# marionmari/pyGPs

Hardware: AMD Instinct MI355X
Metric: GP fits/sec (nlZ+grad, RBF, N=8192 d=16) (higher is better)
Workload: dtype f64; 1 GPU; GPR+RBF, N=8192 d=16 fp64 synthetic (SURVEY 8d recipe, seed 0), infExact nlZ + dnlZ (BASELINE configs[1]); x,y resident in HBM, hyp changes every step; outputs nlZ, dnlZ(4), alpha(N) to host per step; fits_per_rank=313, fit_streams_per_gpu=2, sched=1

## Files before the change

pygps_amd/_lib.py:

```python
import ctypes as C
import os
import threading

import numpy as np

_HERE = os.path.dirname(os.path.abspath(__file__))
LIB_PATH = os.environ.get("PYGPS_AMD_LIB") or os.path.join(_HERE, "libpygps_amd.so")

COV_RBF, COV_RBFARD, COV_MATERN, COV_RBFUNIT, COV_RQ, COV_PIECEPOLY = 0, 1, 2, 3, 4, 5
COV_RQARD, COV_GABOR, COV_PERIODIC, COV_NOISE, COV_CONST, COV_SM = 6, 7, 8, 9, 10, 11
COV_PRE = 12
COV_COMPOSITE = 100
PROG_LEAF, PROG_SUM, PROG_PRODUCT, PROG_SCALE = 1, 2, 3, 4
PROG_MAX_ARD_DIM = 64
PROG_MAX = 8
MODE_TRAIN, MODE_CROSS, MODE_SELF_TEST = 0, 1, 2
LIK_ERF, LIK_GAUSS, LIK_LAPLACE = 0, 1, 2
ERR_LAPLACE_WNEG = -90
FLAG_MATERN_REFERENCE_DER = 1
STAGES = ("assemble", "potrf", "solve", "trtri", "lauum", "grad", "total")

_dp = C.POINTER(C.c_double)
_vp = C.c_void_p
_i64 = C.c_int64

SIGNATURES = {
    "pgp_init": (C.c_int, [C.c_int, C.POINTER(_vp)]),
    "pgp_destroy": (None, [_vp]),
    "pgp_strerror": (C.c_char_p, [C.c_int]),
    "pgp_version": (C.c_char_p, []),
    "pgp_device_count": (C.c_int, []),
    "pgp_device_info": (C.c_int, [_vp, C.POINTER(C.c_int), C.POINTER(C.c_int), _dp, C.c_char_p, C.c_int]),
    "pgp_cov": (C.c_int, [_vp, C.c_int, C.c_int, C.c_int, _dp, _i64, _dp, _i64, _i64, _dp, C.c_int, C.c_int,
                          C.c_int, _dp]),
    "pgp_set_composite": (C.c_int, [_vp, C.POINTER(C.c_int32), C.c_int]),
    "pgp_set_pre": (C.c_int, [_vp, _dp, _i64, _dp, _i64]),
    "pgp_node_kernel": (C.c_int, [_vp, C.c_int, _dp, _i64, C.c_double, C.c_double, _dp]),
    "pgp_knn_graph": (C.c_int, [_vp, _dp, _i64, _i64, C.c_int, _dp]),
    "pgp_set_data": (C.c_int, [_vp, _dp, _i64, _i64, _dp]),
    "pgp_exact_fit": (C.c_int, [_vp, C.c_int, _dp, C.c_int, C.c_int, C.c_int, C.c_double, _dp, _dp, C.c_int,
                                C.c_int, _dp, _dp, _dp, C.POINTER(_vp)]),
    "pgp_factor_to_host": (C.c_int, [_vp, _vp, _dp]),
    "pgp_factor_n": (_i64, [_vp]),
    "pgp_factor_free": (None, [_vp, _vp]),
    "pgp_predict": (C.c_int, [_vp, _vp, _dp, _i64, _dp, _dp, _dp]),
    "pgp_exact_fit_dense": (C.c_int, [_vp, _dp, _i64, _dp, C.c_double, C.c_int, _dp, _dp, _dp, C.POINTER(_vp)]),
    "pgp_dense_grad_term": (C.c_int, [_vp, _dp, _i64, C.c_double, _dp]),
    "pgp_predict_dense": (C.c_int, [_vp, _vp, _dp, _i64, _dp, _dp, _dp, _dp]),
    "pgp_ep_fit": (C.c_int, [_vp, C.c_int, _dp, C.c_int, C.c_int, C.c_int, _dp, _dp, C.c_int, C.c_int, C.c_int,
                             _dp, _dp, _dp, _dp, _dp, _dp, C.POINTER(C.c_int), C.POINTER(_vp)]),
    "pgp_ep_fit_dense": (C.c_int, [_vp, _dp, _dp, _dp, C.c_int, C.c_int, C.c_int, _dp, _dp, _dp, _dp, _dp, _dp,
                                   C.POINTER(C.c_int), C.POINTER(_vp)]),
    "pgp_ep_fit_lik": (C.c_int, [_vp, C.c_int, _dp, C.c_int, C.c_int, C.c_int, C.c_int, _dp, C.c_int, C.c_int, _dp, _dp,
                                 C.c_int, C.c_int, C.c_int, _dp, _dp, _dp, _dp, _dp, _dp, C.POINTER(C.c_int), C.POINTER(_vp)]),
    "pgp_ep_fit_dense_lik": (C.c_int, [_vp, _dp, C.c_int, _dp, C.c_int, C.c_int, _dp, _dp, C.c_int, C.c_int, C.c_int, _dp, _dp,
                                       _dp, _dp, _dp, _dp, C.POINTER(C.c_int), C.POINTER(_vp)]),
    "pgp_laplace_fit": (C.c_int, [_vp, C.c_int, _dp, C.c_int, C.c_int, C.c_int, C.c_int, _dp, C.c_int, _dp, _dp, C.c_int,
                                  C.c_int, C.c_int, _dp, _dp, _dp, _dp, C.POINTER(C.c_int), _dp, C.POINTER(_vp)]),
    "pgp_laplace_fit_dense": (C.c_int, [_vp, _dp, C.c_int, _dp, C.c_int, _dp, _dp, C.c_int, C.c_int, C.c_int, _dp, _dp,
                                        _dp, _dp, C.POINTER(C.c_int), _dp, C.POINTER(_vp)]),
    "pgp_gpmc_fit_predict": (C.c_int, [_vp, C.c_int, _dp, C.c_int, C.c_int, C.c_int, C.c_int, C.POINTER(C.c_int32), C.c_int, _dp, _dp,
                                       _i64, _dp, _dp, _dp, C.POINTER(C.c_int32), C.POINTER(C.c_int32)]),
    "pgp_fitc_fit": (C.c_int, [_vp, C.c_int, _dp, C.c_int, C.c_int, C.c_int, C.c_double, _dp, _i64, _dp, _dp, C.c_int,
                               C.c_int, _dp, _dp, _dp, _dp, C.POINTER(_vp)]),
    "pgp_fitc_predict": (C.c_int, [_vp, _vp, _dp, _i64, _dp, _dp, _dp]),
    "pgp_fitc_free": (None, [_vp, _vp]),
    "pgp_fitc_ep_fit": (C.c_int, [_vp, C.c_int, _dp, C.c_int, C.c_int, C.c_int, _dp, _i64, _dp, _dp, C.c_int, C.c_int,
                                  C.c_int, _dp, _dp, _dp, _dp, _dp, _dp, C.POINTER(C.c_int), C.POINTER(_vp)]),
    "pgp_fitc_ep_fit_lik": (C.c_int, [_vp, C.c_int, _dp, C.c_int, C.c_int, C.c_int, C.c_int, _dp, C.c_int, C.c_int, _dp, _i64,
                                      _dp, _dp, C.c_int, C.c_int, C.c_int, _dp, _dp, _dp, _dp, _dp, _dp, C.POINTER(C.c_int),
                                      C.POINTER(_vp)]),
    "pgp_potrf": (C.c_int, [_vp, _dp, _i64, _dp]),
    "pgp_potrs": (C.c_int, [_vp, _dp, _i64, _dp, _i64, _dp]),
    "pgp_last_timings": (C.c_int, [_vp, _dp]),
    "pgp_set_profiling": (C.c_int, [_vp, C.c_int]),
    "pgp_profile_classes": (C.c_int, []),
    "pgp_profile_class_name": (C.c_char_p, [C.c_int]),
    "pgp_profile_read": (C.c_int, [_vp, C.c_int, C.POINTER(_i64), _dp, _dp, _dp]),
    "pgp_profile_reset": (C.c_int, [_vp]),
    "pgp_set_option": (C.c_int, [_vp, C.c_char_p, C.c_int]),
    "pgp_comm_unique_id": (C.c_int, [C.c_char_p, C.c_char_p]),
    "pgp_comm_init_rccl": (C.c_int, [_vp, C.c_int, C.c_int, C.c_char_p, C.c_char_p, C.POINTER(_vp)]),
    "pgp_comm_init_host": (C.c_int, [_vp, C.c_int, C.c_int, _vp, _vp, _vp, C.POINTER(_vp)]),
    "pgp_comm_free": (None, [_vp]),
    "pgp_comm_world": (C.c_int, [_vp]),
    "pgp_comm_rank": (C.c_int, [_vp]),
    "pgp_comm_bcast_host": (C.c_int, [_vp, _dp, _i64, C.c_int]),
    "pgp_comm_allreduce_host": (C.c_int, [_vp, _dp, _i64, C.c_int]),
    "pgp_comm_allgather_host": (C.c_int, [_vp, _dp, _i64, _dp]),
    "pgp_sharded_exact_fit": (C.c_int, [_vp, _vp, C.c_int, _dp, C.c_int, C.c_int, C.c_int, C.c_double, _dp, _dp, C.c_int,
                                        C.c_int, _dp, _dp, _dp, _dp, _dp, C.POINTER(_vp)]),
    "pgp_sharded_predict": (C.c_int, [_vp, _vp, _vp, _dp, _i64, _dp, _dp, _dp]),
    "pgp_sfactor_free": (None, [_vp, _vp]),
    "pgp_sfactor_bytes": (_i64, [_vp]),
}

TEST_SIGNATURES = {
    "pgp_test_gemm": (C.c_int, [_vp, C.c_int, C.c_int, C.c_int, C.c_int, C.c_int, C.c_int, C.c_int, C.c_double,
                                C.c_double, _dp, _i64, _dp, _i64, _dp, _i64, C.c_int, C.c_int, C.c_int, C.c_int,
                                _dp]),
    "pgp_test_gemm_shrink": (C.c_int, [_vp, _dp, _i64, C.c_int, C.c_int, C.c_int, C.c_int, C.c_int, C.c_int, _dp, _i64,
                                       _i64]),
    "pgp_test_gemm_zskip": (C.c_int, [_vp] + [C.c_int] * 5 + [C.c_double, C.c_double, _dp, _i64, _dp, _i64, _dp, _dp, _i64,
                                      C.c_int, C.c_int, C.c_int]),
    "pgp_test_gemm_skip_wait": (C.c_int, [_vp, C.c_int, _dp, _dp, _dp, C.c_int, C.c_int, C.c_int, C.c_int, C.c_int,
                                          C.POINTER(C.c_int)]),
    "pgp_test_probit_hazard": (C.c_int, [_vp, _dp, _dp, C.c_int]),
    "pgp_test_laplace_lik": (C.c_int, [_vp, C.c_int, C.c_double, _dp, _dp, C.c_int, _dp]),
    "pgp_test_laplace_ep_lik": (C.c_int, [_vp, _dp, _dp, _dp, _dp, C.c_int, _dp]),
    "pgp_test_valu_peak": (C.c_int, [_vp, C.c_int, C.c_int, _dp]),
    "pgp_test_mfma_peak": (C.c_int, [_vp, C.c_int, _dp]),
    "pgp_test_mfma_cycles": (C.c_int, [_vp, C.c_int, C.c_int, C.c_int, _dp]),
    "pgp_test_leaf_ticks": (C.c_int, [_vp, _dp]),
    "pgp_test_assemble": (C.c_int, [_vp, C.c_int, C.c_int, _i64, _i64, C.c_int, _dp]),
    "pgp_test_gemm_trace": (C.c_int, [_vp, C.c_int, C.c_int, C.c_int, C.c_int, C.c_int, C.POINTER(C.c_longlong), _i64, C.POINTER(_i64)]),
    "pgp_test_read_gemm_trace": (C.c_int, [_vp, C.POINTER(C.c_longlong), _i64, C.POINTER(_i64)]),
    "pgp_test_store_roof": (C.c_int, [_vp, _i64, C.c_int, C.c_int, _dp]),
    "pgp_test_cumask_gemm": (C.c_int, [_vp, C.c_int, C.c_int, C.c_int, C.c_int, C.c_int, _dp]),
    "pgp_test_wave_costs": (C.c_int, [_vp, _dp]),
    "pgp_test_stream_concurrency": (C.c_int, [_vp, C.c_int, _dp]),
    "pgp_test_slot_probe": (C.c_int, [_vp, C.c_int, C.c_int, C.c_int, C.c_int, C.c_int, C.c_int, _dp]),
    "pgp_test_hadamard": (C.c_int, [_vp, C.c_int, _dp, C.c_int, C.c_int, C.c_int, _dp, _dp, _dp, C.c_double, _dp]),
    "pgp_test_gather_sym": (C.c_int, [_vp, _dp, _i64, C.POINTER(C.c_int32), _i64, _i64, _dp, _dp, _dp, _dp]),
    "pgp_test_vote": (C.c_int, [_vp, _dp, _dp, _i64, C.c_int, C.c_int, C.c_int, _dp, _dp]),
    "pgp_test_yield_table": (C.c_int, [_vp, C.POINTER(C.c_uint32)]),
}

_lock = threading.RLock()
_dll = None
_ctx = {}


def _torch_first():
    import sys
    if os.environ.get("PYGPS_AMD_NO_TORCH"):
        return
    if "torch" in sys.modules or os.environ.get("PYGPS_AMD_TORCH_FIRST") == "1":
        try:
            import torch
        except Exception:
            pass


def want_torch():
    import sys
    if "torch" not in sys.modules and _dll is not None:
        import logging
        logging.getLogger(__name__).warning(
            "pygps_amd: torch is imported AFTER libpygps_amd.so (HIP runtime in use: %s); on some nodes one of the two then "
            "sees no GPU -- import torch first or set PYGPS_AMD_TORCH_FIRST=1", hip_runtime_path())
    import torch
    return torch


def hip_runtime_path():
    try:
        with open("/proc/self/maps") as f:
            for line in f:
                if "libamdhip64" in line:
                    return line.split()[-1]
    except OSError:
        pass
    return None


def load():
    global _dll
    if _dll is not None:
        return _dll
    with _lock:
        if _dll is None:
            _torch_first()
            if not os.path.exists(LIB_PATH):
                raise RuntimeError(
                    "pygps_amd: %s not found -- build it with `python -c 'import __graft_entry__ as g; g.build()'` "
                    "(hipcc --offload-arch=gfx950).  There is no CPU fallback." % LIB_PATH)
            dll = C.CDLL(LIB_PATH)
            for table in (SIGNATURES, TEST_SIGNATURES):
                for name, (res, args) in table.items():
                    fn = getattr(dll, name)
                    fn.restype = res
                    fn.argtypes = args
            _dll = dll
    return _dll


def strerror(rc):
    return load().pgp_strerror(rc).decode()


def check(rc, what="pygps_amd", arg_messages=None):
    if rc == 0:
        return
    if rc > 0:
        raise np.linalg.LinAlgError("kernel matrix not positive definite, even with jitter. (first bad pivot %d)" % rc)
    if rc <= -100:
        raise RuntimeError("%s: %s" % (what, strerror(rc)))
    if arg_messages and rc in arg_messages:
        raise Exception(arg_messages[rc])
    raise Exception("%s: bad argument (code %d)" % (what, rc))


def ptr(a):
    return None if a is None else a.ctypes.data_as(_dp)


def f64(a):
    return np.ascontiguousarray(a, dtype=np.float64)


def default_device():
    return int(os.environ.get("LOCAL_RANK", os.environ.get("PYGPS_AMD_DEVICE", "0")))


_tls = threading.local()


def current_slot():
    return getattr(_tls, "slot", 0)


class fit_stream(object):

    def __init__(self, k):
        self.k = int(k)

    def __enter__(self):
        self.prev = current_slot()
        _tls.slot = self.k
        return self

    def __exit__(self, *exc):
        _tls.slot = self.prev
        return False


class concurrent_fit_streams(object):

    def __enter__(self):
        self.prev = getattr(_tls, "concurrent", None)
        self.used = {}
        _tls.concurrent = self
        return self

    def _use(self, key, h):
        if key not in self.used:
            load().pgp_set_option(h, b"concurrent_streams", 1)
            self.used[key] = h

    def __exit__(self, *exc):
        _tls.concurrent = self.prev
        for key, h in self.used.items():
            if self.prev is not None and key in self.prev.used:
                continue
            load().pgp_set_option(h, b"concurrent_streams", 0)
        self.used = {}
        return False


def ctx(device=None, slot=None):
    if device is None:
        device = default_device()
    if slot is None:
        slot = current_slot()
    h = _ctx.get((device, slot))
    scope = getattr(_tls, "concurrent", None)
    if h is not None:
        if scope is not None:
            scope._use((device, slot), h)
        return h
    dll = load()
    with _lock:
        h = _ctx.get((device, slot))
        if h is None:
            out = _vp()
            rc = dll.pgp_init(device, C.byref(out))
            if rc != 0:
                raise RuntimeError("pygps_amd: cannot initialise HIP device %d: %s (no CPU fallback)"
                                   % (device, dll.pgp_strerror(rc).decode()))
            h = out
            _ctx[(device, slot)] = h
    if scope is not None:
        scope._use((device, slot), h)
    return h


def device_info(device=None):
    dll = load()
    ncu, clk, gib = C.c_int(), C.c_int(), C.c_double()
    name = C.create_string_buffer(256)
    check(dll.pgp_device_info(ctx(device), C.byref(ncu), C.byref(clk), C.byref(gib), name, 256))
    return dict(name=name.value.decode(), n_cu=ncu.value, sclk_mhz=clk.value, hbm_gib=gib.value)


_devmem = {}


def device_memory_bytes(device=None):
    if device is None:
        device = default_device()
    if device not in _devmem:
        _devmem[device] = device_info(device)["hbm_gib"] * 2.0 ** 30
    return _devmem[device]


def last_timings(device=None):
    out = np.zeros(len(STAGES))
    check(load().pgp_last_timings(ctx(device), ptr(out)))
    return dict(zip(STAGES, out.tolist()))


def profile(device=None):
    dll = load()
    res = {}
    for i in range(dll.pgp_profile_classes()):
        n, ms, fl, by = _i64(), C.c_double(), C.c_double(), C.c_double()
        check(dll.pgp_profile_read(ctx(device), i, C.byref(n), C.byref(ms), C.byref(fl), C.byref(by)))
        res[dll.pgp_profile_class_name(i).decode()] = dict(launches=n.value, ms=ms.value, flops=fl.value,
                                                           bytes=by.value)
    return res
```

pygps_amd/csrc/capi.hip:

```cpp
#include <algorithm>
#include <atomic>
#include <cmath>
#include <cstdio>
#include <cstdlib>
#include <cstring>
#include <map>
#include <string>
#include <mutex>
#include <vector>

#include "ctx.h"

static thread_local char g_err[512] = "";
void pgp_set_last_hip_error(hipError_t e, const char* what, const char* file, int line) {
    snprintf(g_err, sizeof(g_err), "HIP error %d (%s) in %s at %s:%d", (int)e, hipGetErrorString(e), what, file, line);
    (void)hipGetLastError();
}

static void ctx_register(pgp_ctx* c);
static void ctx_unregister(pgp_ctx* c);

void prof_collect(pgp_ctx* c) {
    if (c->recs.empty()) return;
    (void)hipStreamSynchronize(c->st);
    for (auto& r : c->recs) {
        float ms = 0.f;
        (void)hipEventElapsedTime(&ms, r.e0, r.e1);
        c->pc_ms[r.cls] += ms; c->pc_flops[r.cls] += r.flops; c->pc_bytes[r.cls] += r.bytes; c->pc_launch[r.cls]++;
        if (r.shadow >= 0) { c->pc_ms[r.shadow] += ms; c->pc_flops[r.shadow] += r.flops; c->pc_launch[r.shadow]++; }
        if (getenv("PGP_PROF_DUMP"))
            fprintf(stderr, "prof %-34s %8.4f ms %10.3f GF %7.2f TF\n", kProfNames[r.cls], ms, r.flops * 1e-9,
                    ms > 0 ? r.flops / (ms * 1e-3) * 1e-12 : 0.0);
        c->ev_pool.push_back(r.e0); c->ev_pool.push_back(r.e1);
    }
    c->recs.clear();
}

DeviceGate& device_gate(int device) {
    static DeviceGate gates[64];
    return gates[(unsigned)device % 64u];
}
int& device_gate_depth(int device) {
    static thread_local int depth[64] = {0};
    return depth[(unsigned)device % 64u];
}

extern "C" {

const char* pgp_version(void) { return "pygps_amd 0.1 (gfx950)"; }
int pgp_device_count(void) {
    int n = 0;
    if (hipGetDeviceCount(&n) != hipSuccess) { (void)hipGetLastError(); return 0; }
    return n;
}

const char* pgp_strerror(int status) {
    if (status == 0) return "ok";
    if (status > 0) return "kernel matrix not positive definite";
    if (status <= PGP_ERR_HIP) return g_err[0] ? g_err : "HIP runtime failure";
    return "bad argument";
}

__global__ void pgp_noop_kernel() {}
static int alloc_result_buffer(pgp_ctx* c, long np);

static unsigned* yield_table(int device) {
    static std::mutex mu;
    static unsigned* tab[64] = {nullptr};
    std::lock_guard<std::mutex> lk(mu);
    if (device < 0 || device >= 64) return nullptr;
    if (!tab[device]) {
        if (hipMalloc((void**)&tab[device], 4096 * sizeof(unsigned)) != hipSuccess) { (void)hipGetLastError(); tab[device] = nullptr; return nullptr; }
        (void)hipMemset(tab[device], 0, 4096 * sizeof(unsigned));
    }
    return tab[device];
}

int pgp_init(int device, pgp_ctx** ctx_out) { GateShared device_gate_hold(device);
    if (!ctx_out) return -2;
    HIP_TRY(hipSetDevice(device));
    {
        static std::mutex mu;
        static bool primed[64] = {false};
        std::lock_guard<std::mutex> lk(mu);
        if (device >= 0 && device < 64 && !primed[device]) {
            hipLaunchKernelGGL(pgp_noop_kernel, dim3(1), dim3(64), 0, 0);
            HIP_TRY(hipDeviceSynchronize());
            primed[device] = true;
        }
    }
    pgp_ctx* c = new pgp_ctx();
    c->device = device;
    if (const char* e = getenv("PYGPS_AMD_PREDICT_INVERSE")) { const int v = atoi(e); if (v >= 0 && v <= 2) c->predict_inverse = v; }
    if (const char* e = getenv("PYGPS_AMD_KEEP_INVERSE")) c->keep_inverse = atoi(e) != 0;
    HIP_TRY(hipGetDeviceProperties(&c->prop, device));
    HIP_TRY(hipStreamCreateWithFlags(&c->st, hipStreamNonBlocking));
    {
        int lo = 0, hi = 0;
        (void)hipDeviceGetStreamPriorityRange(&lo, &hi);
        HIP_TRY(hipStreamCreateWithPriority(&c->st2, hipStreamNonBlocking, hi));
        if (lo == hi) c->ep_block = 0;
    }
    for (auto& e : c->ev) HIP_TRY(hipEventCreate(&e));
    memset(c->last_ms, 0, sizeof(c->last_ms));
    memset(c->pc_ms, 0, sizeof(c->pc_ms)); memset(c->pc_flops, 0, sizeof(c->pc_flops));
    memset(c->pc_bytes, 0, sizeof(c->pc_bytes)); memset(c->pc_launch, 0, sizeof(c->pc_launch));
    CHK(alloc_result_buffer(c, 0));
    c->yield_flags = yield_table(device);
    HIP_TRY(hipMalloc((void**)&c->Dk, (size_t)2048 * 1024 * sizeof(double)));
    HIP_TRY(hipMalloc((void**)&c->dpack, (size_t)8 * PACK_DOUBLES * sizeof(double)));
    HIP_TRY(hipMemset(c->Dk, 0, (size_t)2048 * 1024 * sizeof(double)));
    ctx_register(c);
    *ctx_out = c;
    return PGP_OK;
}

constexpr long RES_HEAD = 272, RES_INFO = 264;
static int alloc_result_buffer(pgp_ctx* c, long np) {
    const size_t bytes = (size_t)(RES_HEAD + np) * sizeof(double);
    if (c->res_dev) (void)hipFree(c->res_dev);
    if (c->res_host) (void)hipHostFree(c->res_host);
    c->res_dev = c->res_host = c->res_host_dev = nullptr; c->scal = c->alpha_dev = nullptr; c->info_dev = nullptr; c->res_cap = 0;
    HIP_TRY(hipMalloc((void**)&c->res_dev, bytes));
    HIP_TRY(hipMemset(c->res_dev, 0, bytes));
    HIP_TRY(hipHostMalloc((void**)&c->res_host, bytes, hipHostMallocMapped | hipHostMallocCoherent));
    c->res_host_dev = nullptr;
    if (hipHostGetDevicePointer((void**)&c->res_host_dev, c->res_host, 0) != hipSuccess) { (void)hipGetLastError(); c->res_host_dev = nullptr; }
    c->scal = c->res_dev; c->info_dev = (int*)(c->res_dev + RES_INFO); c->alpha_dev = c->res_dev + RES_HEAD;
    c->res_cap = bytes;
    return PGP_OK;
}

void pgp_destroy(pgp_ctx* c) { if (!c) return; GateShared device_gate_hold(c);
    if (!c) return;
    ctx_unregister(c);
    (void)hipSetDevice(c->device);
    (void)hipStreamSynchronize(c->st);
    if (c->st2) (void)hipStreamSynchronize(c->st2);
    for (auto& kv : c->pool) (void)hipFree(kv.second);
    for (auto& kv : c->spool) (void)hipFree(kv.second);
    for (auto& kv : c->orders) (void)hipFree(kv.second.first);
    void* bufs[] = {c->x_dev, c->y_dev, c->XsT, c->scale_dev, c->W, c->T, c->Binv, c->inv16, c->m_dev,
                    c->rvec, c->zvec, c->partial, c->Dk, c->dpack, c->Xs, c->res_dev, c->prep, c->pre2, c->pre1t, c->pre1s};
    for (void* b : bufs) if (b) (void)hipFree(b);
    if (c->res_host) (void)hipHostFree(c->res_host);
    if (c->in_host) (void)hipHostFree(c->in_host);
    if (c->pred_host) (void)hipHostFree(c->pred_host);
    if (c->gemm_trace) (void)hipFree(c->gemm_trace);
    for (auto& e : c->ev) (void)hipEventDestroy(e);
    for (auto& e : c->ev_pool) (void)hipEventDestroy(e);
    for (auto& r : c->recs) { (void)hipEventDestroy(r.e0); (void)hipEventDestroy(r.e1); }
    for (auto& e : c->la_ev) (void)hipEventDestroy(e);
    for (auto& e : c->tm_ev) (void)hipEventDestroy(e);
    for (auto& e : c->fill_ev) (void)hipEventDestroy(e);
    for (auto& e : c->ep_ev) (void)hipEventDestroy(e);
    (void)hipStreamDestroy(c->st);
    if (c->st2) (void)hipStreamDestroy(c->st2);
    delete c;
}

int pgp_device_info(pgp_ctx* c, int* n_cu, int* sclk_mhz, double* hbm_gib, char* name, int name_len) {
    if (!c) return -1;
    if (n_cu) *n_cu = c->prop.multiProcessorCount;
    if (sclk_mhz) *sclk_mhz = c->prop.clockRate / 1000;
    if (hbm_gib) *hbm_gib = (double)c->prop.totalGlobalMem / (1024.0 * 1024.0 * 1024.0);
    if (name && name_len > 0) { strncpy(name, c->prop.name, name_len - 1); name[name_len - 1] = 0; }
    return PGP_OK;
}

int pgp_set_option(pgp_ctx* c, const char* name, int value) {
    if (!c || !name) return -1;
    if (!strcmp(name, "nb_outer")) { if (value < 0) return -3; c->nb_outer = value; return PGP_OK; }
    if (!strcmp(name, "small_tile_below")) { c->small_tile_below = value; return PGP_OK; }
    if (!strcmp(name, "trtri_small_tile_below")) { c->trtri_small_tile_below = value; return PGP_OK; }
    if (!strcmp(name, "xcd_order")) { c->xcd_order = value; return PGP_OK; }
    if (!strcmp(name, "gemm_dbg")) { if (value & ~(64 | 256 | 512)) return -2; c->gemm_dbg = value; return PGP_OK; }
    if (!strcmp(name, "lookahead")) { c->lookahead = value; return PGP_OK; }
    if (!strcmp(name, "leaf_first")) { c->leaf_first = value; return PGP_OK; }
    if (!strcmp(name, "leaf_pivot")) { if (value < 0 || value > 2) return -2; c->leaf_pivot = value; return PGP_OK; }
    if (!strcmp(name, "sched")) { if (value < -1 || value > 2) return -2; c->sched = value < 0 ? PGP_SCHED_DEFAULT : value; c->sched_explicit = value >= 0; return PGP_OK; }
    if (!strcmp(name, "concurrent_streams")) { c->concurrent_streams = value != 0; return PGP_OK; }
    if (!strcmp(name, "tud_tile")) { if (value != 64 && value != 128) return -2; c->tud_tile = value; return PGP_OK; }
    if (!strcmp(name, "tur_tile")) { if (value != 0 && value != 64 && value != 128 && value != 1264) return -2; c->tur_tile = value; return PGP_OK; }
    if (!strcmp(name, "s_pan")) { if (value < -1 || value > 2) return -2; c->s_pan = value; return PGP_OK; }
    if (!strcmp(name, "s_pan_direct")) { c->s_pan_direct = value != 0; return PGP_OK; }
    if (!strcmp(name, "s_pan_out")) { c->s_pan_out = value != 0; return PGP_OK; }
    if (!strcmp(name, "skip_zeros")) { c->skip_zeros = value != 0; return PGP_OK; }
    if (!strcmp(name, "tud_mark")) { c->tud_mark = value != 0; return PGP_OK; }
    if (!strcmp(name, "sched2_wide")) { c->sched2_wide = value != 0; return PGP_OK; }
    if (!strcmp(name, "gram_assembly")) { if (value < 0 || value > 2) return -2; c->gram_assembly = value; return PGP_OK; }
    if (!strcmp(name, "yield")) { c->yield = value; return PGP_OK; }
    if (!strcmp(name, "ep_fused")) { c->ep_fused = value; return PGP_OK; }
    if (!strcmp(name, "ep_tol_exp")) { if (value < 1 || value > 16) return -3; c->ep_tol_exp = value; return PGP_OK; }
    if (!strcmp(name, "ep_max_sweep")) { if (value < 2 || value > 1000) return -3; c->ep_max_sweep = value; return PGP_OK; }
    if (!strcmp(name, "laplace_tol_exp")) { if (value < 1 || value > 16) return -3; c->laplace_tol_exp = value; return PGP_OK; }
    if (!strcmp(name, "ep_r_direct")) { c->ep_r_direct = value; return PGP_OK; }
    if (!strcmp(name, "ep_alpha_direct")) { c->ep_alpha_direct = value; return PGP_OK; }
    if (!strcmp(name, "ep_sym")) { c->ep_sym = value; return PGP_OK; }
    if (!strcmp(name, "ep_wait_kernel")) { c->ep_wait_kernel = value; return PGP_OK; }
    if (!strcmp(name, "ep_sigma_under")) { c->ep_sigma_under = value; return PGP_OK; }
    if (!strcmp(name, "ep_recompute")) { c->ep_recompute = value; return PGP_OK; }
    if (!strcmp(name, "ep_final_rebuild")) { c->ep_final_rebuild = value; return PGP_OK; }
    if (!strcmp(name, "ep_block")) { c->ep_block = value; return PGP_OK; }
    if (!strcmp(name, "xcd_max_k")) { c->xcd_max_k = value; return PGP_OK; }
    if (!strcmp(name, "xcd_min_tiles")) { c->xcd_min_tiles = value; return PGP_OK; }
    if (!strcmp(name, "xcd_super")) { c->xcd_super = value; return PGP_OK; }
    if (!strcmp(name, "solve_outer")) { if (value < 1) return -2; c->solve_outer = value; return PGP_OK; }
    if (!strcmp(name, "keep_inverse")) { c->keep_inverse = value != 0; return PGP_OK; }
    if (!strcmp(name, "predict_inverse")) { if (value < 0 || value > 2) return -2; c->predict_inverse = value; return PGP_OK; }
    if (!strcmp(name, "predict_batch")) { if (value < 128 || value % 128) return -2; c->predict_batch = value; return PGP_OK; }
    if (!strcmp(name, "s_tile")) { if (value != 0 && value != 64 && value != 128) return -2; c->s_tile = value; return PGP_OK; }
    if (!strcmp(name, "eet_overlap")) { if (value != 0 && value != 2 && value != 3) return -2; c->eet_overlap = value; return PGP_OK; }
    if (!strcmp(name, "eet_max_panels")) { c->eet_max_panels = value; return PGP_OK; }
    if (!strcmp(name, "eet_first")) { if (value < -1) return -2; c->eet_first = value; return PGP_OK; }
    if (!strcmp(name, "eet_tile")) { if (value != 64 && value != 128) return -2; c->eet_tile = value; return PGP_OK; }
    if (!strcmp(name, "fused_inverse")) { c->fused_inverse = value; return PGP_OK; }
    if (!strcmp(name, "trsm_lean")) { if (value < 0 || value > 2) return -2; c->trsm_lean = value; return PGP_OK; }
    if (!strcmp(name, "ep_merge12")) { c->ep_merge12 = value != 0; return PGP_OK; }
    if (!strcmp(name, "publish")) { c->publish = value != 0; return PGP_OK; }
    if (!strcmp(name, "fused_value_max_np")) { c->fused_value_max_np = value; return PGP_OK; }
    if (!strcmp(name, "asm_grid")) { c->asm_grid = value; return PGP_OK; }
    if (!strcmp(name, "gram_fast")) { if (value < 0 || value > 2) return -2; c->gram_fast = value; return PGP_OK; }
    if (!strcmp(name, "gram_grid")) { if (value < 0) return -2; c->gram_grid = value; return PGP_OK; }
    if (!strcmp(name, "asm_nt")) { c->asm_nt = value; return PGP_OK; }
    if (!strcmp(name, "pair_launch")) { c->pair_launch = value != 0; return PGP_OK; }
    if (!strcmp(name, "gemm_trace")) {
        GateShared device_gate_hold(c);
        HIP_TRY(hipSetDevice(c->device));
        HIP_TRY(hipDeviceSynchronize());
        if (c->gemm_trace) { (void)hipFree(c->gemm_trace); c->gemm_trace = nullptr; }
        c->gemm_trace_cap = 0; c->gemm_trace_pos = 0;
        if (value > 0) {
            const long cap = (long)value * 1024;
            HIP_TRY(hipMalloc((void**)&c->gemm_trace, (size_t)cap * 64));
            HIP_TRY(hipMemset(c->gemm_trace, 0, (size_t)cap * 64));
            c->gemm_trace_cap = cap;
        }
        return PGP_OK;
    }
    if (!strcmp(name, "ard_grad_form")) { if (value < 0 || value > 2) return -3; c->ard_grad_form = value; return PGP_OK; }
    return -2;
}

int pgp_last_timings(pgp_ctx* c, double* ms_out) {
    if (!c || !ms_out) return -1;
    memcpy(ms_out, c->last_ms, sizeof(c->last_ms));
    return PGP_OK;
}
int pgp_set_profiling(pgp_ctx* c, int on) { if (!c) return -1; c->prof = on != 0; return PGP_OK; }
int pgp_profile_classes(void) { return PC_COUNT; }
const char* pgp_profile_class_name(int cls) { return (cls >= 0 && cls < PC_COUNT) ? kProfNames[cls] : "?"; }
int pgp_profile_read(pgp_ctx* c, int cls, int64_t* launches, double* ms, double* flops, double* bytes) {
    if (!c || cls < 0 || cls >= PC_COUNT) return -1;
    prof_collect(c);
    if (launches) *launches = c->pc_launch[cls];
    if (ms) *ms = c->pc_ms[cls];
    if (flops) *flops = c->pc_flops[cls];
    if (bytes) *bytes = c->pc_bytes[cls];
    return PGP_OK;
}
int pgp_profile_reset(pgp_ctx* c) {
    if (!c) return -1;
    prof_collect(c);
    memset(c->pc_ms, 0, sizeof(c->pc_ms)); memset(c->pc_flops, 0, sizeof(c->pc_flops));
    memset(c->pc_bytes, 0, sizeof(c->pc_bytes)); memset(c->pc_launch, 0, sizeof(c->pc_launch));
    return PGP_OK;
}

}


static int matern_d(int para) { return (para == 1 || para == 3 || para == 5 || para == 7) ? para : 3; }

static int leaf_nhyp(int kind, long d) {
    switch (kind) {
        case PGP_COV_RBF: case PGP_COV_MATERN: case PGP_COV_PIECEPOLY: case PGP_COV_GABOR: return 2;
        case PGP_COV_RBFARD: return (int)d + 1;
        case PGP_COV_RQARD: return (int)d + 2;
        case PGP_COV_RBFUNIT: case PGP_COV_NOISE: case PGP_COV_CONST: return 1;
        case PGP_COV_RQ: case PGP_COV_PERIODIC: return 3;
        case PGP_COV_PRE: return 0;
        default: return -1;
    }
}

static int make_leaf(int kind, const double* hyp, int nhyp, int para, int flags, long d, CovParams& cp, double& iso) {
    const int want = leaf_nhyp(kind, d);
    if (want < 0) return -2;
    if (nhyp != want) return -11;
    cp = CovParams{};
    cp.kind = kind; cp.der = -1; cp.md = matern_d(para); cp.D = (int)d; cp.train = 1;
    cp.ref_der = (flags & PGP_FLAG_MATERN_REFERENCE_DER) ? 1 : 0;
    cp.sf2 = 1.0; cp.alpha = 1.0; cp.ppv = 0; cp.ppj = 1.0; cp.ga = 0.0; cp.gb = 0.0;
    iso = 1.0;
    switch (kind) {
        case PGP_COV_RBF: iso = 1.0 / exp(hyp[0]); cp.sf2 = exp(2.0 * hyp[1]); break;
        case PGP_COV_RBFARD: cp.sf2 = exp(2.0 * hyp[d]); break;
        case PGP_COV_MATERN: iso = sqrt((double)cp.md) / exp(hyp[0]); cp.sf2 = exp(2.0 * hyp[1]); break;
        case PGP_COV_RBFUNIT: iso = 1.0 / exp(hyp[0]); break;
        case PGP_COV_RQ: iso = 1.0 / exp(hyp[0]); cp.sf2 = exp(2.0 * hyp[1]); cp.alpha = exp(hyp[2]); break;
        case PGP_COV_PIECEPOLY:
            if (para < 0 || para > 3) return -12;
            iso = 1.0 / exp(hyp[0]); cp.sf2 = exp(2.0 * hyp[1]);
            cp.ppv = para; cp.ppj = floor(0.5 * (double)d) + para + 1.0;
            break;
        case PGP_COV_RQARD: cp.sf2 = exp(2.0 * hyp[d]); cp.alpha = exp(hyp[d + 1]); cp.gb = 1.0; break;
        case PGP_COV_GABOR: {
            const double ell = exp(hyp[0]), p = exp(2.0 * hyp[1]);
            iso = 1.0 / ell; cp.ga = 2.0 * M_PI * ell / p;
            break;
        }
        case PGP_COV_PERIODIC:
            if (d != 1) return -12;
            cp.gb = 1.0 / exp(hyp[0]); cp.ga = M_PI / exp(hyp[1]); cp.sf2 = exp(2.0 * hyp[2]);
            break;
        case PGP_COV_NOISE: cp.sf2 = exp(2.0 * hyp[0]); break;
        case PGP_COV_CONST: cp.sf2 = exp(hyp[0]); break;
    }
    return PGP_OK;
}

static int bind_pre(pgp_ctx* c, CovSpec& cs) {
    if (cs.pg.pre_leaf < 0) return PGP_OK;
    if (!c || !c->pre2 || c->pre_n != c->n || c->n <= 0) return -14;
    cs.pre_train = c->pre2; cs.pre_ld = c->pre_ld; cs.pre_rows = c->pre_ld;
    return PGP_OK;
}

int make_spec(pgp_ctx* c, int kind, const double* hyp, int nhyp, int para, int flags, int der, long d, CovSpec& cs) {
    cs = CovSpec{};
    if (c) { cs.asm_grid = c->asm_grid; cs.asm_nt = c->asm_nt; cs.gram_fast = c->gram_fast; cs.gram_grid = c->gram_grid; }
    if (!hyp && nhyp > 0) return -10;
    if (kind == PGP_COV_SM) {
        const long Q = para;
        if (Q < 1) return -12;
        if (d > SM_MAXD || Q * (1 + 2 * d) > SM_MAXHYP) return -13;
        if ((long)nhyp != Q * (1 + 2 * d)) return -11;
        if (der >= nhyp) return -4;
        CovSM& P = cs.smp;
        P = CovSM{};
        P.Q = (int)Q; P.D = (int)d; P.dt = -1; P.dj = -1; P.dq = 0;
        const long double pi = 3.14159265358979323846264338327950288L;
        long double sw = 0.0L;
        for (long q = 0; q < Q; ++q) { P.h[q] = (double)expl((long double)hyp[q]); sw += expl((long double)hyp[q]); }
        for (long i = 0; i < d * Q; ++i) {
            P.h[Q + i] = (double)(2.0L * pi * expl((long double)hyp[Q + i]));
            P.h[Q + d * Q + i] = (double)(2.0L * pi * pi * expl(2.0L * (long double)hyp[Q + d * Q + i]));
        }
        cs.sm = true; cs.scale.assign(d, 1.0); cs.ncov = nhyp; cs.nder = nhyp;
        cs.cp = CovParams{};
        cs.cp.kind = kind; cs.cp.der = der; cs.cp.D = (int)d; cs.cp.train = 1; cs.cp.sf2 = (double)sw;
        return PGP_OK;
    }
    if (kind >= PGP_COV_GABOR && kind < PGP_COV_NKIND) {
        CovProgram& P = cs.pg;
        P = CovProgram{};
        double iso;
        CHK(make_leaf(kind, hyp, nhyp, para, flags, d, P.leaf[0], iso));
        if (der >= nhyp) return -4;
        P.nleaf = 1; P.nterm = 1; P.nscale = 0; P.is2[0] = iso * iso; P.hyp0[0] = 0; P.nh[0] = nhyp; P.ard_leaf = -1; P.ard_leaf2 = -1;
        P.pre_leaf = kind == PGP_COV_PRE ? 0 : -1;
        P.coef[0] = 1.0; P.tl[0] = 1u; P.ts[0] = 0u;
        P.der = der; P.der_leaf = der >= 0 ? 0 : -1; P.der_j = der; P.der_scale = -1;
        cs.prog = true; cs.scale.assign(d, 1.0); cs.ncov = nhyp; cs.nder = nhyp;
        return bind_pre(c, cs);
    }
    if (kind != PGP_COV_COMPOSITE) {
        double iso;
        CHK(make_leaf(kind, hyp, nhyp, para, flags, d, cs.cp, iso));
        cs.scale.assign(d, iso);
        if (kind == PGP_COV_RBFARD || kind == PGP_COV_RQARD) {
            for (long k = 0; k < d; ++k) cs.scale[k] = 1.0 / exp(hyp[k]);
            double bound = 0.0;
            if (c && (long)c->xdev2.size() == d)
                for (long k = 0; k < d; ++k) bound += cs.scale[k] * cs.scale[k] * c->xdev2[k];
            cs.ard_grad_diff = !(bound <= ARD_GRAM_GRAD_BOUND) || (c && c->ard_grad_form == 2);
            if (c && c->ard_grad_form == 1) cs.ard_grad_diff = false;
        }
        cs.ncov = nhyp;
        cs.nder = (kind == PGP_COV_MATERN || kind == PGP_COV_PIECEPOLY) ? 3 : nhyp;
        if (der >= cs.nder) return -4;
        cs.cp.der = der;
        cs.ell4 = (kind == PGP_COV_RQARD && cs.cp.ref_der && der >= 0 && der < d) ? exp(4.0 * hyp[der]) : 1.0;
        return PGP_OK;
    }
    const std::vector<int>& tok = c->composite;
    if (tok.empty()) return -2;
    struct Term { unsigned leaves, scales; };
    std::vector<std::vector<Term>> stack;
    CovProgram& P = cs.pg;
    P = CovProgram{};
    P.der = der; P.der_leaf = P.der_j = P.der_scale = -1;
    P.ard_leaf = -1; P.ard_leaf2 = -1; P.pre_leaf = -1;
    int used = 0;
    for (size_t i = 0; i < tok.size();) {
        const int op = tok[i];
        if (op == PGP_PROG_LEAF) {
            if (i + 5 > tok.size()) return -2;
            const int lk = tok[i + 1], lpara = tok[i + 2], lflags = tok[i + 3], h0 = tok[i + 4];
            i += 5;
            const bool ard = lk == PGP_COV_RBFARD || lk == PGP_COV_RQARD;
            if (ard && (P.ard_leaf2 >= 0 || d > CP_MAXARD)) return -13;
            const int nh = leaf_nhyp(lk, d);
            if (nh < 0) return -2;
            if (h0 < 0 || h0 + nh > nhyp) return -11;
            if (P.nleaf >= CP_MAXLEAF) return -13;
            if (lk == PGP_COV_PRE) {
                if (P.pre_leaf >= 0) return -13;
                P.pre_leaf = P.nleaf;
            }
            double iso;
            CHK(make_leaf(lk, hyp + h0, nh, lpara, lflags, d, P.leaf[P.nleaf], iso));
            P.is2[P.nleaf] = iso * iso; P.hyp0[P.nleaf] = h0; P.nh[P.nleaf] = nh;
            if (ard) {
                double* aw = P.ard_leaf < 0 ? P.ardw : P.ardw2;
                (P.ard_leaf < 0 ? P.ard_leaf : P.ard_leaf2) = P.nleaf;
                for (long k = 0; k < d; ++k) aw[k] = exp(-2.0 * hyp[h0 + k]);
                if (lk == PGP_COV_RQARD && P.leaf[P.nleaf].ref_der && der >= h0 && der < h0 + d) cs.ell4 = exp(4.0 * hyp[der]);
            }
            if (der >= h0 && der < h0 + nh) { P.der_leaf = P.nleaf; P.der_j = der - h0; }
            stack.push_back({Term{1u << P.nleaf, 0u}});
            ++P.nleaf; used += nh;
        } else if (op == PGP_PROG_SUM || op == PGP_PROG_PRODUCT) {
            ++i;
            if (stack.size() < 2) return -2;
            std::vector<Term> b = stack.back(); stack.pop_back();
            std::vector<Term> a = stack.back(); stack.pop_back();
            std::vector<Term> r;
            if (op == PGP_PROG_SUM) { r = a; r.insert(r.end(), b.begin(), b.end()); }
            else for (const Term& x : a) for (const Term& y : b) r.push_back(Term{x.leaves | y.leaves, x.scales | y.scales});
            if (r.size() > (size_t)CP_MAXTERM) return -13;
            stack.push_back(r);
        } else if (op == PGP_PROG_SCALE) {
            if (i + 1 >= tok.size()) return -2;
            const int h = tok[i + 1];
            i += 2;
            if (stack.empty()) return -2;
            if (h < 0 || h >= nhyp) return -11;
            if (P.nscale >= CP_MAXSCALE) return -13;
            for (Term& t : stack.back()) t.scales |= 1u << P.nscale;
            P.shyp[P.nscale] = h;
            if (der == h) P.der_scale = P.nscale;
            ++P.nscale; ++used;
        } else {
            return -2;
        }
    }
    if (stack.size() != 1 || used != nhyp) return -11;
    P.nterm = (int)stack[0].size();
    for (int t = 0; t < P.nterm; ++t) {
        P.tl[t] = stack[0][t].leaves; P.ts[t] = stack[0][t].scales;
        double cf = 1.0;
        for (int k = 0; k < P.nscale; ++k)
            if ((P.ts[t] >> k) & 1u) cf *= exp(hyp[P.shyp[k]]);
        P.coef[t] = cf;
    }
    if (der >= nhyp) return -4;
    cs.prog = true;
    cs.scale.assign(d, 1.0);
    cs.ncov = nhyp; cs.nder = nhyp;
    cs.cp = CovParams{};
    if (P.ard_leaf >= 0 && c && (long)c->xdev2.size() == d) {
        double b1 = 0.0, b2 = 0.0;
        for (long k = 0; k < d && k < CP_MAXARD; ++k) { b1 += P.ardw[k] * c->xdev2[k]; if (P.ard_leaf2 >= 0) b2 += P.ardw2[k] * c->xdev2[k]; }
        cs.ard_grad_diff = !(std::max(b1, b2) <= ARD_GRAM_GRAD_BOUND);
    }
    if (c && P.ard_leaf >= 0 && c->ard_grad_form) cs.ard_grad_diff = c->ard_grad_form == 2;
    return bind_pre(c, cs);
}

int cov_point_value(pgp_ctx* c, const CovSpec& cs, int train, double* out) {
    if (cs.has_pre()) { *out = 0.0; return PGP_OK; }
    if (!cs.prog && cs.cp.der < 0) {
        (void)train;
        *out = cs.cp.sf2;
        return PGP_OK;
    }
    double* dv = c->scal + 6;
    CHK(cov_self_launch(cs, train, dv, c->st));
    HIP_TRY(hipMemcpyAsync(out, dv, sizeof(double), hipMemcpyDeviceToHost, c->st));
    HIP_TRY(hipStreamSynchronize(c->st));
    return PGP_OK;
}

int upload_scaled(pgp_ctx* c, const double* x_dev, long n, long d, const std::vector<double>& sc, double* XsT,
                         long ldp, int dpad, double* scale_dev) {
    HIP_TRY(hipMemcpyAsync(scale_dev, sc.data(), d * sizeof(double), hipMemcpyHostToDevice, c->st));
    return scale_transpose_launch(x_dev, n, (int)d, scale_dev, XsT, ldp, dpad, c->st);
}

static int tile_order(pgp_ctx* c, int mt, int nt, int tri, int off_tiles, const int** out, int* n) {
    std::vector<int> key = {mt, nt, tri ? 1 : 0, off_tiles, c->xcd_super};
    auto it = c->orders.find(key);
    if (it != c->orders.end()) { *out = it->second.first; *n = it->second.second; return PGP_OK; }
    const int S = c->xcd_super > 0 ? c->xcd_super : 8;
    std::vector<std::vector<int>> sts;
    for (int SI = 0; SI * S < mt; ++SI)
        for (int SJ = 0; SJ * S < nt; ++SJ) {
            std::vector<int> st;
            for (int ti = SI * S; ti < std::min(mt, SI * S + S); ++ti)
                for (int tj = SJ * S; tj < std::min(nt, SJ * S + S); ++tj)
                    if (!tri || ti + off_tiles >= tj) { st.push_back(ti); st.push_back(tj); }
            if (!st.empty()) sts.push_back(std::move(st));
        }
    std::stable_sort(sts.begin(), sts.end(), [](const std::vector<int>& a, const std::vector<int>& b) { return a.size() > b.size(); });
    std::vector<std::vector<int>> seq(8);
    for (auto& st : sts) {
        int best = 0;
        for (int x = 1; x < 8; ++x) if (seq[x].size() < seq[best].size()) best = x;
        seq[best].insert(seq[best].end(), st.begin(), st.end());
    }
    for (;;) {
        int lo = 0, hi = 0;
        for (int x = 1; x < 8; ++x) { if (seq[x].size() < seq[lo].size()) lo = x; if (seq[x].size() > seq[hi].size()) hi = x; }
        if (seq[hi].size() < seq[lo].size() + 4) break;
        const int tj = seq[hi].back(); seq[hi].pop_back();
        const int ti = seq[hi].back(); seq[hi].pop_back();
        seq[lo].push_back(ti); seq[lo].push_back(tj);
    }
    size_t maxlen = 0;
    for (auto& q : seq) maxlen = std::max(maxlen, q.size() / 2);
    const int nb = (int)maxlen * 8;
    std::vector<int> ord(2 * (size_t)nb, -1);
    for (int b = 0; b < nb; ++b) {
        const int x = b % 8, idx = b / 8;
        if ((size_t)idx < seq[x].size() / 2) { ord[2 * b] = seq[x][2 * idx]; ord[2 * b + 1] = seq[x][2 * idx + 1]; }
    }
    int* dev = nullptr;
    HIP_TRY(hipMalloc((void**)&dev, ord.size() * sizeof(int)));
    HIP_TRY(hipMemcpyAsync(dev, ord.data(), ord.size() * sizeof(int), hipMemcpyHostToDevice, c->st));
    HIP_TRY(hipStreamSynchronize(c->st));
    c->orders[key] = {dev, nb};
    *out = dev; *n = nb;
    return PGP_OK;
}

static int tri_tile_list(pgp_ctx* c, int mt, int nt, int off_tiles, const int** out, int* n) {
    std::vector<int> key = {mt, nt, 2, off_tiles};
    auto it = c->orders.find(key);
    if (it != c->orders.end()) { *out = it->second.first; *n = it->second.second; return PGP_OK; }
    std::vector<int> ord;
    for (int tj = 0; tj < nt; ++tj)
        for (int ti = 0; ti < mt; ++ti)
            if (ti + off_tiles >= tj) { ord.push_back(ti); ord.push_back(tj); }
    int* dev = nullptr;
    HIP_TRY(hipMalloc((void**)&dev, ord.size() * sizeof(int)));
    HIP_TRY(hipMemcpyAsync(dev, ord.data(), ord.size() * sizeof(int), hipMemcpyHostToDevice, c->st));
    HIP_TRY(hipStreamSynchronize(c->st));
    c->orders[key] = {dev, (int)ord.size() / 2};
    *out = dev; *n = (int)ord.size() / 2;
    return PGP_OK;
}

int batch_tile_list(pgp_ctx* c, int mt0, int nt, int nb, int dmt, const int** out, int* n) {
    std::vector<int> key = {mt0, nt, nb, dmt, 7777};
    auto it = c->orders.find(key);
    if (it != c->orders.end()) { *out = it->second.first; *n = it->second.second; return PGP_OK; }
    std::vector<int> ord;
    for (int z = 0; z < nb; ++z)
        for (int tj = 0; tj < nt; ++tj)
            for (int ti = tj; ti < mt0 - z * dmt; ++ti) { ord.push_back(ti | (z << 16)); ord.push_back(tj); }
    if (ord.empty()) { ord.push_back(-1); ord.push_back(-1); }
    int* dev = nullptr;
    HIP_TRY(hipMalloc((void**)&dev, ord.size() * sizeof(int)));
    HIP_TRY(hipMemcpyAsync(dev, ord.data(), ord.size() * sizeof(int), hipMemcpyHostToDevice, c->st));
    HIP_TRY(hipStreamSynchronize(c->st));
    c->orders[key] = {dev, (int)ord.size() / 2};
    *out = dev; *n = (int)ord.size() / 2;
    return PGP_OK;
}

bool gram_assembly_applies(pgp_ctx* c, const CovSpec& cs) {
    if (!c->gram_assembly || !cov_gram_applies(cs, c->dpad) || (long)c->xdev2.size() != c->d || (long)cs.scale.size() < c->d) return false;
    if (c->gram_assembly == 2) return true;
    double bound = 0.0;
    for (long k = 0; k < c->d; ++k) bound += cs.scale[k] * cs.scale[k] * c->xdev2[k];
    return bound <= 64.0;
}

static int gemm_prepare(pgp_ctx* c, GemmArgs& g) {
    if (g.batch < 1) g.batch = 1;
    g.dbg |= c->gemm_dbg;
    bool xcd = false;
    if (c->xcd_order && !g.order && g.tile != 64 && g.tile != 1264 && g.batch == 1 && g.K <= c->xcd_max_k) {
        const long mt = g.M / 128, nt = g.N / 128;
        const long tiles = g.tri == 2 ? mt * (mt + 1) / 2 : (g.tri == 1 ? mt * nt - nt * (nt - 1) / 2 : mt * nt);
        xcd = tiles >= c->xcd_min_tiles;
    }
    if (g.tri == 1 && !g.order && !xcd) {
        const int T = g.tile == 64 ? 64 : 128;
        CHK(tri_tile_list(c, g.M / T, g.N / T, g.tri_off / T, &g.order, &g.norder));
    }
    if (xcd) CHK(tile_order(c, g.M / 128, g.N / 128, g.tri, g.tri ? g.tri_off / 128 : 0, &g.order, &g.norder));
    if (c->yield && c->yield_flags) {
        g.yield_flags = c->yield_flags;
        if (g.yield_role != 2) g.yield_role = gemm_f64_uses_dma(g) ? 1 : 0;
    } else g.yield_role = 0;
    if (c->gemm_trace && gemm_f64_uses_dma128(g) && g.batch == 1) {
        const long mt = g.M / 128, nt = g.N / 128;
        const long nb = g.order ? g.norder : (g.tri == 2 ? mt * (mt + 1) / 2 : mt * nt);
        if (c->gemm_trace_pos + nb <= c->gemm_trace_cap) { g.trace = c->gemm_trace + 8 * c->gemm_trace_pos; c->gemm_trace_pos += nb; }
    }
    return PGP_OK;
}

int gemm_prof(pgp_ctx* c, int cls, GemmArgs g, hipStream_t st) {
    if (!st) st = c->st;
    CHK(gemm_prepare(c, g));
    ProfScope ps(c, cls, g.flops, 0.0, st, gemm_f64_uses_dma128(g) ? PC_KERNEL_DMA128 : -1);
    return gemm_f64_launch(g, st);
}

int gemm_prof_pair(pgp_ctx* c, int cls_a, GemmArgs a, int cls_b, GemmArgs b, hipStream_t st) {
    if (!st) st = c->st;
    CHK(gemm_prepare(c, a));
    CHK(gemm_prepare(c, b));
    if (c->pair_launch && gemm_f64_pair_ok(a, b)) {
        ProfScope ps(c, cls_a, a.flops + b.flops, 0.0, st, PC_KERNEL_DMA128);
        return gemm_f64_launch_pair(a, b, st);
    }
    { ProfScope ps(c, cls_a, a.flops, 0.0, st, gemm_f64_uses_dma128(a) ? PC_KERNEL_DMA128 : -1);
      CHK(gemm_f64_launch(a, st)); }
    ProfScope ps(c, cls_b, b.flops, 0.0, st, gemm_f64_uses_dma128(b) ? PC_KERNEL_DMA128 : -1);
    return gemm_f64_launch(b, st);
}

struct TriNode { int lo, mid, hi, depth; };
static void tri_nodes(int lo, int hi, int depth, std::vector<TriNode>& out) {
    if (hi - lo <= 1) return;
    int half = 1;
    while (half * 2 < hi - lo) half *= 2;
    const int mid = lo + half;
    out.push_back({lo, mid, hi, depth});
    tri_nodes(lo, mid, depth + 1, out);
    tri_nodes(mid, hi, depth + 1, out);
}

int trtri_lower(pgp_ctx* c, const double* L, long ldl, double* W, long ldw, double* T, long np) {
    const int nblk = (int)(np / 128);
    {
        ProfScope ps(c, PC_LEAFINV, (double)nblk * 128.0 * 128.0 * 128.0 / 3.0, 0.0);
        CHK(leaf_inv_launch(L, ldl, W, ldw, 128L * (1 + ldw), nblk, c->st));
    }
    std::vector<TriNode> nodes;
    tri_nodes(0, nblk, 0, nodes);
    int maxd = -1;
    for (auto& nd : nodes) maxd = std::max(maxd, nd.depth);
    for (int dep = maxd; dep >= 0; --dep) {
        std::vector<TriNode> lv;
        for (auto& nd : nodes) if (nd.depth == dep) lv.push_back(nd);
        if (lv.empty()) continue;
        std::sort(lv.begin(), lv.end(), [](const TriNode& a, const TriNode& b) { return a.lo < b.lo; });
        bool uniform = true;
        const int h1 = lv[0].mid - lv[0].lo, h2 = lv[0].hi - lv[0].mid;
        const int step = lv.size() > 1 ? lv[1].lo - lv[0].lo : 0;
        for (size_t i = 0; i < lv.size(); ++i)
            if (lv[i].mid - lv[i].lo != h1 || lv[i].hi - lv[i].mid != h2 || lv[i].lo != lv[0].lo + (int)i * step)
                uniform = false;
        const size_t ngroups = uniform ? 1 : lv.size();
        for (size_t gi = 0; gi < ngroups; ++gi) {
            const TriNode& nd = lv[gi];
            const int a1 = (nd.mid - nd.lo) * 128, a2 = (nd.hi - nd.mid) * 128;
            const long o1 = (long)nd.lo * 128, o2 = (long)nd.mid * 128;
            const int batch = uniform ? (int)lv.size() : 1;
            const long bstep = (long)step * 128;
            const long t128 = (long)(a2 / 128) * (a1 / 128) * batch;
            GemmArgs g{};
            g.A = L + o2 + o1 * ldl; g.lda = ldl; g.a_kc = 0;
            g.B = W + o1 + o1 * ldw; g.ldb = ldw; g.b_kc = 1;
            g.C = T; g.ldc = a2;
            g.M = a2; g.N = a1; g.K = a1; g.alpha = 1.0; g.beta = 0.0;
            g.kmode = KM_GE_J; g.koff = 0;
            g.batch = batch; g.sA = bstep * (1 + ldl); g.sB = bstep * (1 + ldw); g.sC = (long)a1 * a2;
            g.tile = t128 < c->trtri_small_tile_below ? 64 : 128;
            g.flops = (double)batch * (double)a2 * a1 * a1;
            CHK(gemm_prof(c, PC_GEMM_TRTRI, g));
            GemmArgs h{};
            h.A = W + o2 + o2 * ldw; h.lda = ldw; h.a_kc = 0;
            h.B = T; h.ldb = a2; h.b_kc = 1;
            h.C = W + o2 + o1 * ldw; h.ldc = ldw;
            h.M = a2; h.N = a1; h.K = a2; h.alpha = -1.0; h.beta = 0.0;
            h.kmode = KM_LT_I; h.koff = 0;
            h.batch = batch; h.sA = bstep * (1 + ldw); h.sB = (long)a1 * a2; h.sC = bstep * (1 + ldw);
            h.tile = g.tile;
            h.flops = (double)batch * (double)a2 * a2 * a1;
            CHK(gemm_prof(c, PC_GEMM_TRTRI, h));
        }
    }
    return PGP_OK;
}

int lauum_lower(pgp_ctx* c, const double* W, long ldw, double* Binv, long ldb, long np) {
    GemmArgs g{};
    g.A = W; g.lda = ldw; g.a_kc = 1;
    g.B = W; g.ldb = ldw; g.b_kc = 1;
    g.C = Binv; g.ldc = ldb;
    g.M = (int)np; g.N = (int)np; g.K = (int)np; g.alpha = 1.0; g.beta = 0.0;
    g.tri = 2; g.mask_diag = 1; g.kmode = KM_GE_I; g.koff = 0;
    const long t128 = (np / 128) * (np / 128 + 1) / 2;
    g.tile = t128 < c->small_tile_below ? 64 : 128;
    g.flops = (double)np * np * np / 3.0;
    return gemm_prof(c, PC_GEMM_LAUUM, g);
}

int eet_lower(pgp_ctx* c, const double* E, long lde, double* Binv, long ldb, long np) {
    GemmArgs g{};
    g.A = E; g.lda = lde; g.a_kc = 0;
    g.B = E; g.ldb = lde; g.b_kc = 0;
    g.C = Binv; g.ldc = ldb;
    g.M = (int)np; g.N = (int)np; g.K = (int)np; g.alpha = 1.0; g.beta = 0.0;
    g.tri = 2; g.mask_diag = 1; g.kmode = KM_GE_I; g.koff = 0;
    const long t128 = (np / 128) * (np / 128 + 1) / 2;
    g.tile = t128 < c->small_tile_below ? 64 : 128;
    g.flops = (double)np * np * np / 3.0;
    return gemm_prof(c, PC_GEMM_LAUUM, g);
}

int ensure_workspace(pgp_ctx* c, long np) {
    if (c->ws_np == np) return PGP_OK;
    (void)hipStreamSynchronize(c->st);
    void* olds[] = {c->W, c->T, c->Binv, c->inv16, c->m_dev, c->rvec, c->zvec, c->prep};
    for (void* b : olds) if (b) (void)hipFree(b);
    c->W = c->T = c->Binv = c->inv16 = c->m_dev = c->rvec = c->zvec = c->prep = nullptr;
    if (c->in_host) { (void)hipHostFree(c->in_host); c->in_host = nullptr; c->in_cap = 0; }
    c->ws_np = 0;
    c->dense_ready = false;
    const size_t nn = (size_t)np * np * sizeof(double);
    HIP_TRY(hipMalloc((void**)&c->W, nn));
    HIP_TRY(hipMemsetAsync(c->W, 0, nn, c->st));
    HIP_TRY(hipMalloc((void**)&c->Binv, nn));
    HIP_TRY(hipMemsetAsync(c->Binv, 0, nn, c->st));
    HIP_TRY(hipMalloc((void**)&c->T, std::max<size_t>(nn / 4, 128 * 128 * sizeof(double))));
    HIP_TRY(hipMalloc((void**)&c->inv16, (size_t)(np / 128) * PACK_DOUBLES * sizeof(double)));
    CHK(alloc_result_buffer(c, np));
    HIP_TRY(hipMalloc((void**)&c->m_dev, np * sizeof(double)));
    HIP_TRY(hipMalloc((void**)&c->rvec, np * sizeof(double)));
    HIP_TRY(hipMalloc((void**)&c->zvec, np * sizeof(double)));
    HIP_TRY(hipMalloc((void**)&c->prep, (size_t)hadamard_prep_count(np) * sizeof(double)));
    HIP_TRY(hipMemsetAsync(c->rvec, 0, np * sizeof(double), c->st));
    c->in_cap = (size_t)(np + 1024) * sizeof(double);
    HIP_TRY(hipHostMalloc((void**)&c->in_host, c->in_cap, hipHostMallocDefault));
    c->ws_np = np;
    return PGP_OK;
}

int alloc_factor_buffer(pgp_ctx* c, long np, long ldf, double** F) {
    const size_t bytes = (size_t)ldf * np * sizeof(double);
    bool fresh = false;
    CHK(pool_alloc(c, bytes, (void**)F, &fresh));
    if (fresh) HIP_TRY(hipMemsetAsync(*F, 0, bytes, c->st));
    return PGP_OK;
}

static std::mutex g_ctx_mu;
static std::vector<pgp_ctx*> g_ctxs;
int pgp_ctx_count_on_device(int device) {
    std::lock_guard<std::mutex> lk(g_ctx_mu);
    int n = 0;
    for (pgp_ctx* c : g_ctxs) n += c->device == device;
    return n;
}
void pgp_drop_idle_pools(int device) { GateShared device_gate_hold(device);
    std::lock_guard<std::mutex> lk(g_ctx_mu);
    for (pgp_ctx* c : g_ctxs) {
        if (c->device != device) continue;
        std::lock_guard<std::mutex> lp(c->pool_mu);
        for (auto& kv : c->pool) (void)hipFree(kv.second);
        for (auto& kv : c->spool) (void)hipFree(kv.second);
        c->pool.clear(); c->pool_bytes = 0;
        c->spool.clear(); c->spool_bytes = 0;
    }
}
static void ctx_register(pgp_ctx* c) { std::lock_guard<std::mutex> lk(g_ctx_mu); g_ctxs.push_back(c); }
static void ctx_unregister(pgp_ctx* c) {
    std::lock_guard<std::mutex> lk(g_ctx_mu);
    g_ctxs.erase(std::remove(g_ctxs.begin(), g_ctxs.end(), c), g_ctxs.end());
}

extern "C" {

int pgp_set_composite(pgp_ctx* c, const int32_t* prog, int nprog) { if (!c) return -1; GateShared device_gate_hold(c);
    if (!c) return -1;
    if (nprog < 0 || (nprog > 0 && !prog)) return -2;
    c->composite.assign(prog, prog + nprog);
    return PGP_OK;
}

int pgp_set_pre(pgp_ctx* c, const double* M2, int64_t n, const double* M1, int64_t ns) { if (!c) return -1; GateShared device_gate_hold(c);
    if (!c) return -1;
    if (n <= 0) return -3;
    if (M1 && ns <= 0) return -5;
    HIP_TRY(hipSetDevice(c->device));
    (void)hipStreamSynchronize(c->st);
    const long np = round_up(n, 128);
    if (M2) {
        if (c->pre2) (void)hipFree(c->pre2);
        c->pre2 = nullptr; c->pre_n = 0;
        if (c->pre1t) (void)hipFree(c->pre1t);
        if (c->pre1s) (void)hipFree(c->pre1s);
        c->pre1t = c->pre1s = nullptr; c->pre_ns = 0;
        HIP_TRY(hipMalloc((void**)&c->pre2, (size_t)np * np * sizeof(double)));
        HIP_TRY(hipMemsetAsync(c->pre2, 0, (size_t)np * np * sizeof(double), c->st));
        HIP_TRY(hipMemcpy2DAsync(c->pre2, np * sizeof(double), M2, n * sizeof(double), n * sizeof(double), n, hipMemcpyHostToDevice, c->st));
        HIP_TRY(hipStreamSynchronize(c->st));
        c->pre_n = n; c->pre_ld = np;
    }
    if (M1) {
        if (!c->pre2 || c->pre_n != n) return -2;
        if (c->pre1t) (void)hipFree(c->pre1t);
        if (c->pre1s) (void)hipFree(c->pre1s);
        c->pre1t = c->pre1s = nullptr; c->pre_ns = 0;
        const long nsp = round_up(ns, 128);
        HIP_TRY(hipMalloc((void**)&c->pre1t, (size_t)nsp * np * sizeof(double)));
        HIP_TRY(hipMalloc((void**)&c->pre1s, (size_t)nsp * sizeof(double)));
        HIP_TRY(hipMemsetAsync(c->pre1t, 0, (size_t)nsp * np * sizeof(double), c->st));
        HIP_TRY(hipMemsetAsync(c->pre1s, 0, (size_t)nsp * sizeof(double), c->st));
        std::vector<double> blk;
        for (int64_t a = 0; a < ns; a += 1024) {
            const int64_t nb = std::min<int64_t>(1024, ns - a);
            blk.resize((size_t)nb * n);
            for (int64_t i = 0; i < n; ++i)
                for (int64_t j = 0; j < nb; ++j) blk[(size_t)j * n + i] = M1[(size_t)i * ns + a + j];
            HIP_TRY(hipMemcpy2DAsync(c->pre1t + a * np, np * sizeof(double), blk.data(), n * sizeof(double), n * sizeof(double), nb,
                                     hipMemcpyHostToDevice, c->st));
            HIP_TRY(hipStreamSynchronize(c->st));
        }
        HIP_TRY(hipMemcpyAsync(c->pre1s, M1 + (size_t)n * ns, ns * sizeof(double), hipMemcpyHostToDevice, c->st));
        HIP_TRY(hipStreamSynchronize(c->st));
        c->pre_ns = ns; c->pre_nsp = nsp;
    }
    return PGP_OK;
}

int pgp_set_data(pgp_ctx* c, const double* x, int64_t n, int64_t d, const double* y) { if (!c) return -1; GateShared device_gate_hold(c);
    if (!c) return -1;
    if (!x) return -2;
    if (n <= 0) return -3;
    if (d <= 0) return -4;
    HIP_TRY(hipSetDevice(c->device));
    (void)hipStreamSynchronize(c->st);
    void* olds[] = {c->x_dev, c->y_dev, c->XsT, c->scale_dev};
    for (void* b : olds) if (b) (void)hipFree(b);
    c->x_dev = c->y_dev = c->XsT = c->scale_dev = nullptr;
    c->n = 0;
    const long np = round_up(n, 128);
    const int dpad = (int)round_up(d, SKC);
    HIP_TRY(hipMalloc((void**)&c->x_dev, n * d * sizeof(double)));
    HIP_TRY(hipMalloc((void**)&c->y_dev, np * sizeof(double)));
    HIP_TRY(hipMalloc((void**)&c->XsT, (size_t)dpad * np * sizeof(double)));
    HIP_TRY(hipMalloc((void**)&c->scale_dev, dpad * sizeof(double)));
    HIP_TRY(hipMemcpyAsync(c->x_dev, x, n * d * sizeof(double), hipMemcpyHostToDevice, c->st));
    HIP_TRY(hipMemsetAsync(c->y_dev, 0, np * sizeof(double), c->st));
    if (y) HIP_TRY(hipMemcpyAsync(c->y_dev, y, n * sizeof(double), hipMemcpyHostToDevice, c->st));
    HIP_TRY(hipStreamSynchronize(c->st));
    {
        std::vector<double> mean((size_t)d, 0.0);
        for (int64_t p = 0; p < n; ++p) for (int64_t k = 0; k < d; ++k) mean[k] += x[p * d + k];
        for (int64_t k = 0; k < d; ++k) mean[k] /= (double)n;
        c->xdev2.assign((size_t)d, 0.0);
        for (int64_t p = 0; p < n; ++p)
            for (int64_t k = 0; k < d; ++k) { const double v = x[p * d + k] - mean[k]; if (v * v > c->xdev2[k]) c->xdev2[k] = v * v; }
    }
    c->n = n; c->d = d; c->np = np; c->ldf = np + 128;
    c->dpad = dpad;
    return PGP_OK;
}

int pgp_exact_fit(pgp_ctx* c, int kind, const double* covhyp, int ncov, int para, int flags, double log_sn,
                  const double* mvec, const double* dm, int nmean, int want, double* alpha_out, double* nlZ_out,
                  double* dnlZ_out, pgp_factor** factor_out) {
    if (!c) return -1;
    GateShared device_gate_hold(c);
    if (!c) return -1;
    if (c->n <= 0) return -1;
    if (!covhyp) return -3;
    if (want < 1 || want > 3) return -11;
    if (ncov < 0 || 8 + ncov + 1 > RES_INFO) return -4;
    HIP_TRY(hipSetDevice(c->device));
    c->dense_ready = false;
    const long n = c->n, d = c->d, np = c->np;
    bool fused = c->fused_inverse != 0;
    if (want < 3 && fused && c->fused_value_max_np >= 0 && np > c->fused_value_max_np) fused = false;
    const long ldf = c->ldf;
    CovSpec cp;
    { const int rc = make_spec(c, kind, covhyp, ncov, para, flags, -1, d, cp); if (rc != PGP_OK) return rc == -11 ? -10 : rc; }
    const std::vector<double>& sc = cp.scale;
    CHK(ensure_workspace(c, np));
    double kss = 0.0;
    if (factor_out) CHK(cov_point_value(c, cp, 2, &kss));
    const long need = std::max(hadamard_partial_count(np, ncov), 32L * np);
    if ((want >= 3 || fused) && c->partial_cap < need) {
        if (c->partial) (void)hipFree(c->partial);
        c->partial = nullptr; c->partial_cap = 0;
        HIP_TRY(hipMalloc((void**)&c->partial, need * sizeof(double)));
        c->partial_cap = need;
    }
    const double sn2 = exp(2.0 * log_sn);
    double* F = nullptr;
    CHK(alloc_factor_buffer(c, np, ldf, &F));
    FactorGuard fguard(c, F, (size_t)ldf * np * sizeof(double), true);
// ... 258 lines not shown
```

pygps_amd/csrc/common.h:

```cpp
#pragma once
#include <hip/hip_runtime.h>
#include <cstdint>
#include <cstdio>

#define PGP_OK 0
#define PGP_ERR_HIP (-100)
#define PGP_ERR_ARG (-1)

#define HIP_TRY(expr)                                                                       \
    do {                                                                                    \
        hipError_t e__ = (expr);                                                            \
        if (e__ != hipSuccess) {                                                            \
            pgp_set_last_hip_error(e__, #expr, __FILE__, __LINE__);                         \
            return PGP_ERR_HIP;                                                             \
        }                                                                                   \
    } while (0)

void pgp_set_last_hip_error(hipError_t e, const char* what, const char* file, int line);

enum GemmKMode {
    KM_FULL = 0,
    KM_GE_I = 1,
    KM_GE_J = 2,
    KM_LT_I = 3,
    KM_LT_J = 4,
};

struct GemmArgs {
    const double* A; long lda; int a_kc;
    const double* B; long ldb; int b_kc;
    double* C; long ldc;
    int M, N, K;
    double alpha, beta;
    int tri;
    int tri_off;
    int mask_diag;
    int kmode; int koff;
    int batch; long sA, sB, sC;
    int tile;
    const int* order;
    int norder;
    int order_z;
    int dbg;
    double flops;
    const double* A2; long lda2; int a_split;
    double* C2; long ldc2; int c_split;
    const double* Cin; long ldcin; const double* Cin2; long ldcin2;
    int rev_cols;
    int rev_rows;
    int fold_rows;
    int zero_from;
    int zf_upper;
    int batch_dm;
    int batch_dk;
    int batch_dldc; long batch_sC2;
    unsigned* yield_flags; int yield_role;
    int skip_lo, skip_hi;
    unsigned* wait_flag; unsigned wait_target; unsigned* wait_err;
    long long* trace;
};

__device__ __forceinline__ unsigned pgp_cu_key() {
    const unsigned hw = __builtin_amdgcn_s_getreg((4 << 0) | (0 << 6) | (31 << 11));
    const unsigned xcc = __builtin_amdgcn_s_getreg((20 << 0) | (0 << 6) | (3 << 11)) & 15u;
    return (xcc << 8) | ((hw >> 8) & 0xffu);
}
__device__ __forceinline__ void pgp_yield_mark(unsigned* flags, int delta) {
    if (flags && threadIdx.x == 0) {
        if (delta > 0) __hip_atomic_fetch_add(flags + pgp_cu_key(), 1u, __ATOMIC_RELAXED, __HIP_MEMORY_SCOPE_AGENT);
        else __hip_atomic_fetch_sub(flags + pgp_cu_key(), 1u, __ATOMIC_RELAXED, __HIP_MEMORY_SCOPE_AGENT);
    }
}

int gemm_f64_launch(const GemmArgs& g, hipStream_t st);
bool gemm_f64_pair_ok(const GemmArgs& a, const GemmArgs& b);
int gemm_f64_launch_pair(const GemmArgs& a, const GemmArgs& b, hipStream_t st);
bool gemm_f64_uses_dma(const GemmArgs& g);
bool gemm_f64_uses_dma128(const GemmArgs& g);

void func_max_dynamic_lds(const void* fn, size_t bytes);
```

pygps_amd/csrc/ctx.h:

```cpp
#pragma once
#include <algorithm>
#include <chrono>
#include <condition_variable>
#include <cstdio>
#include <cstdlib>
#include <map>
#include <mutex>
#include <vector>

#include "../../include/pygps_amd.h"
#include "kernels.h"
#include "sqdist_tile.h"

enum ProfClass { PC_ASSEMBLE = 0, PC_GEMM_TRAIL, PC_GEMM_INNER, PC_LEAF, PC_TRSM, PC_LEAFINV, PC_GEMM_TRTRI,
                 PC_GEMM_LAUUM, PC_HADAMARD, PC_SMALL, PC_GEMM_SOLVE, PC_DIAG, PC_KERNEL_DMA128, PC_COUNT };
static const char* const kProfNames[PC_COUNT] = {
    "cov_tile_kernel(assemble)", "gemm_f64(potrf trailing syrk)", "gemm_f64(potrf inner update)",
    "leaf_potrf_kernel", "trsm_rows_kernel", "leaf_inv_kernel", "gemm_f64(trtri)", "gemm_f64(lauum W^T W)",
    "hadamard_reduce_kernel", "small/O(N) kernels", "gemm_f64(panel solve X E_D)", "diag_in/out staging",
    "kernel gemm_f64_kernel<128,128,false,false,true,*> + gemm_f64_pair_kernel (LDS-DMA 128-tile)"};

struct ProfRec { int cls; hipEvent_t e0, e1; double flops, bytes; int shadow; };

struct pgp_factor {
    long n, np, ldf;
    double* F;
    double* alpha;
    double* XsT;
    double* Wd;
    double* Linv = nullptr;
    double* Eraw = nullptr;
    size_t Eraw_bytes = 0;
    int dpad, d;
    CovSpec cs;
    double kss = 0.0;
    double sn2;
    double sw;
    double* sWv = nullptr;
};

constexpr int PGP_SCHED_DEFAULT = 2;

struct pgp_ctx {
    int device = 0;
    std::vector<int> composite;
    hipStream_t st = nullptr;
    hipStream_t st2 = nullptr;
    std::vector<hipEvent_t> fill_ev;
    std::vector<hipEvent_t> ep_ev;
    int eet_tile = 128;
    int eet_first = -1;
    int eet_overlap = 3;
    int eet_max_panels = 32;
    std::vector<hipEvent_t> la_ev;
    std::vector<hipEvent_t> tm_ev;
    int lookahead = 1;
    bool sched_explicit = false;
    bool concurrent_streams = false;
    int sched = PGP_SCHED_DEFAULT;
    int tur_tile = 0;
    int tud_tile = 64;
    int sched2_wide = 0;
    int s_pan = -1;
    int s_pan_direct = 1;
    int s_pan_out = 1;
    int skip_zeros = 1;
    int tud_mark = 1;
    int leaf_pivot = 2;
    int leaf_first = 0;
    int yield = 1;
    long long* gemm_trace = nullptr;
    long gemm_trace_cap = 0;
    long gemm_trace_pos = 0;
    unsigned* yield_flags = nullptr;
    int ep_fused = 2;
    int ep_r_direct = 1;
    int ep_alpha_direct = 1;
    int ep_recompute = 0;
    int ep_final_rebuild = 0;
    int ep_tol_exp = 4;
    int ep_max_sweep = 10;
    int laplace_tol_exp = 6;
    int ep_sigma_under = 1;
    int ep_wait_kernel = 1;
    int ep_sym = 1;
    int ep_block = 1;
    int fused_value_max_np = 12288;
    int fused_inverse = 1;
    hipDeviceProp_t prop;
    std::mutex pool_mu;
    std::multimap<size_t, void*> pool;
    size_t pool_bytes = 0;
    std::multimap<size_t, void*> spool;
    size_t spool_bytes = 0;
    long n = 0, d = 0, np = 0, ldf = 0;
    int dpad = 0;
    double *x_dev = nullptr, *y_dev = nullptr, *XsT = nullptr, *scale_dev = nullptr;
    double *pre2 = nullptr, *pre1t = nullptr, *pre1s = nullptr;
    long pre_n = 0, pre_ld = 0, pre_ns = 0, pre_nsp = 0;
    long ws_np = 0;
    double *W = nullptr, *T = nullptr, *Binv = nullptr, *inv16 = nullptr, *alpha_dev = nullptr, *m_dev = nullptr,
           *rvec = nullptr, *zvec = nullptr, *partial = nullptr, *scal = nullptr;
    long partial_cap = 0;
    double* prep = nullptr;
    int pair_launch = 1;
    int ard_grad_form = 0;
    std::vector<double> xdev2;
    int gram_assembly = 1;
    bool dense_ready = false;
    long dense_n = 0;
    int* info_dev = nullptr;
    double* res_dev = nullptr;
    double* res_host = nullptr;
    double* res_host_dev = nullptr;
    int ep_merge12 = 1;
    int trsm_lean = 0;
    int publish = 1;
    double* in_host = nullptr;
    double* pred_host = nullptr;
    size_t pred_cap = 0;
    size_t res_cap = 0, in_cap = 0;
    double *Dk = nullptr, *dpack = nullptr, *Xs = nullptr;
    int xcd_max_k = 512;
    int xcd_min_tiles = 256;
    int xcd_super = 8;
    int solve_outer = 8;
    int keep_inverse = 1;
    int predict_inverse = 1;
    int predict_batch = 65536;
    int s_tile = 0;
    int gram_fast = 2, gram_grid = 32768;
    int asm_grid = 4096, asm_nt = 0;
    size_t Xs_bytes = 0;
    hipEvent_t ev[PGP_NSTAGE + 2];
    double last_ms[PGP_NSTAGE];
    bool prof = false;
    std::vector<ProfRec> recs;
    std::vector<hipEvent_t> ev_pool;
    double pc_ms[PC_COUNT], pc_flops[PC_COUNT], pc_bytes[PC_COUNT];
    int64_t pc_launch[PC_COUNT];
    std::map<std::vector<int>, std::pair<int*, int>> orders;
    int gemm_dbg = 64 | 256 | 512;
    int xcd_order = 0;
    int nb_outer = 0;
    int trtri_small_tile_below = 2049;
    int small_tile_below = 200;
};

#define CHK(x)                      \
    do {                            \
        int rc__ = (x);             \
        if (rc__ != PGP_OK) return rc__; \
    } while (0)

int pgp_ctx_count_on_device(int device);
void pgp_drop_idle_pools(int device);

static inline bool pool_trace_on() { static const bool on = getenv("PGP_POOL_TRACE") != nullptr; return on; }
static inline hipError_t pool_hip_malloc(void** out, size_t bytes, const char* who) {
    if (!pool_trace_on()) return hipMalloc(out, bytes);
    const auto t0 = std::chrono::steady_clock::now();
    const hipError_t e = hipMalloc(out, bytes);
    fprintf(stderr, "[pool] hipMalloc %8.1f MiB  %8.3f ms  (%s)%s\n", bytes / 1048576.0,
            std::chrono::duration<double, std::milli>(std::chrono::steady_clock::now() - t0).count(), who, e == hipSuccess ? "" : " FAILED");
    return e;
}
static inline void pool_hip_free(void* p, size_t bytes, const char* who) {
    if (!pool_trace_on()) { (void)hipFree(p); return; }
    const auto t0 = std::chrono::steady_clock::now();
    (void)hipFree(p);
    fprintf(stderr, "[pool] hipFree   %8.1f MiB  %8.3f ms  (%s)\n", bytes / 1048576.0,
            std::chrono::duration<double, std::milli>(std::chrono::steady_clock::now() - t0).count(), who);
}

static inline size_t pool_idle_cap(pgp_ctx* c) {
    return (size_t)c->prop.totalGlobalMem / 3 / (size_t)std::max(1, pgp_ctx_count_on_device(c->device));
}

static inline int pool_alloc(pgp_ctx* c, size_t bytes, void** out, bool* fresh = nullptr) {
    if (fresh) *fresh = false;
    {
        std::lock_guard<std::mutex> lk(c->pool_mu);
        auto it = c->pool.find(bytes);
        if (it != c->pool.end()) {
            *out = it->second;
            c->pool.erase(it);
            c->pool_bytes -= bytes;
            return PGP_OK;
        }
    }
    if (fresh) *fresh = true;
    if (pool_hip_malloc(out, bytes, "factor pool") != hipSuccess) {
        (void)hipGetLastError();
        pgp_drop_idle_pools(c->device);
        HIP_TRY(pool_hip_malloc(out, bytes, "factor pool, retry"));
    }
    return PGP_OK;
}
static inline void pool_free(pgp_ctx* c, size_t bytes, void* p) {
    if (!p) return;
    const size_t cap = pool_idle_cap(c);
    std::lock_guard<std::mutex> lk(c->pool_mu);
    if (c->pool_bytes + bytes > cap) { pool_hip_free(p, bytes, "factor pool over its cap"); return; }
    c->pool.insert({bytes, p});
    c->pool_bytes += bytes;
}

static inline int spool_take(pgp_ctx* c, size_t bytes, void** out) {
    {
        std::lock_guard<std::mutex> lk(c->pool_mu);
        auto it = c->spool.find(bytes);
        if (it != c->spool.end()) {
            *out = it->second;
            c->spool.erase(it);
            c->spool_bytes -= bytes;
            return PGP_OK;
        }
    }
    hipError_t e = pool_hip_malloc(out, bytes ? bytes : 8, "handle buffer");
    if (e != hipSuccess) { pgp_set_last_hip_error(e, "hipMalloc(handle buffer)", __FILE__, __LINE__); return PGP_ERR_HIP; }
    return PGP_OK;
}
static inline void spool_give(pgp_ctx* c, size_t bytes, void* p) {
    if (!p) return;
    if (!c) { (void)hipFree(p); return; }
    const size_t cap = pool_idle_cap(c);
    std::lock_guard<std::mutex> lk(c->pool_mu);
    if (c->spool_bytes + bytes > cap) { pool_hip_free(p, bytes, "scratch pool over its cap (handle buffer)"); return; }
    c->spool.insert({bytes, p});
    c->spool_bytes += bytes;
}

struct ProfScope {
    pgp_ctx* c; int cls; double flops, bytes; hipEvent_t e0 = nullptr, e1 = nullptr; hipStream_t s; int shadow;
    ProfScope(pgp_ctx* c_, int cls_, double f, double b, hipStream_t s_ = nullptr, int shadow_ = -1)
        : c(c_), cls(cls_), flops(f), bytes(b), s(s_ ? s_ : c_->st), shadow(shadow_) {
        if (!c->prof) return;
        auto get = [&]() {
            hipEvent_t e;
            if (!c->ev_pool.empty()) { e = c->ev_pool.back(); c->ev_pool.pop_back(); }
            else (void)hipEventCreate(&e);
            return e;
        };
        e0 = get(); e1 = get();
        (void)hipEventRecord(e0, s);
    }
    ~ProfScope() {
        if (!c->prof) return;
        (void)hipEventRecord(e1, s);
        c->recs.push_back({cls, e0, e1, flops, bytes, shadow});
    }
};


struct DevScratch {
    std::vector<void*> ptrs;
    ~DevScratch() { for (void* p : ptrs) if (p) (void)hipFree(p); }
    template <typename T>
    int alloc(T** out, size_t bytes) {
        void* p = nullptr;
        hipError_t e = hipMalloc(&p, bytes ? bytes : 8);
        if (e != hipSuccess) { pgp_set_last_hip_error(e, "hipMalloc(scratch)", __FILE__, __LINE__); return PGP_ERR_HIP; }
        ptrs.push_back(p);
        *out = (T*)p;
        return PGP_OK;
    }
};

struct PoolScratch {
    pgp_ctx* c;
    std::vector<std::pair<size_t, void*>> held;
    explicit PoolScratch(pgp_ctx* c_) : c(c_) {}
    ~PoolScratch() {
        const size_t cap = pool_idle_cap(c);
        std::lock_guard<std::mutex> lk(c->pool_mu);
        for (auto& h : held) {
            if (c->spool_bytes + h.first > cap) { pool_hip_free(h.second, h.first, "scratch pool over its cap"); continue; }
            c->spool.insert({h.first, h.second});
            c->spool_bytes += h.first;
        }
    }
    template <typename T>
    int alloc(T** out, size_t bytes) {
        void* p = nullptr;
        if (!bytes) bytes = 8;
        {
            std::lock_guard<std::mutex> lk(c->pool_mu);
            auto it = c->spool.find(bytes);
            if (it != c->spool.end()) { p = it->second; c->spool.erase(it); c->spool_bytes -= bytes; }
        }
        if (!p && pool_hip_malloc(&p, bytes, "scratch pool") != hipSuccess) {
            (void)hipGetLastError();
            pgp_drop_idle_pools(c->device);
            hipError_t e = pool_hip_malloc(&p, bytes, "scratch pool, retry");
            if (e != hipSuccess) { pgp_set_last_hip_error(e, "hipMalloc(pool scratch)", __FILE__, __LINE__); return PGP_ERR_HIP; }
        }
        held.push_back({bytes, p});
        *out = (T*)p;
        return PGP_OK;
    }
    size_t release(void* p) {
        for (size_t i = 0; i < held.size(); ++i)
            if (held[i].second == p) { const size_t b = held[i].first; held.erase(held.begin() + (long)i); return b; }
        return 0;
    }
};

struct FactorGuard {
    pgp_ctx* c; double* F; size_t bytes; bool scrub;
    FactorGuard(pgp_ctx* c_, double* F_, size_t b, bool scrub_ = false) : c(c_), F(F_), bytes(b), scrub(scrub_) {}
    ~FactorGuard() {
        if (!F) return;
        if (scrub) { (void)hipMemsetAsync(F, 0, bytes, c->st); (void)hipStreamSynchronize(c->st); }
        pool_free(c, bytes, F);
    }
    double* release() { double* p = F; F = nullptr; return p; }
};

struct FactorHandleGuard {
    pgp_ctx* c; pgp_factor* f;
    FactorHandleGuard(pgp_ctx* c_, pgp_factor* f_) : c(c_), f(f_) {}
    ~FactorHandleGuard() { if (f) pgp_factor_free(c, f); }
    pgp_factor* release() { pgp_factor* p = f; f = nullptr; return p; }
};

void prof_collect(pgp_ctx* c);
static inline long round_up(long v, long m) { return (v + m - 1) / m * m; }
int make_spec(pgp_ctx* c, int kind, const double* hyp, int nhyp, int para, int flags, int der, long d, CovSpec& cs);
int cov_point_value(pgp_ctx* c, const CovSpec& cs, int train, double* out);
struct SweepJob {
    double* F; long ldf, np, mrows;
    bool inverse = false;
    double* E = nullptr; long lde = 0;
    double* R = nullptr; long ldr = 0, nrhs2 = 0;
    double* eet_out = nullptr; long eet_ld = 0;
    double* rhs_C = nullptr;  long rhs_ld = 0;
    hipEvent_t join = nullptr;
};
int potrf_blocked(pgp_ctx* c, SweepJob& job);
static inline int ensure_events(std::vector<hipEvent_t>& ev, size_t n) {
    for (hipEvent_t e; ev.size() < n; ev.push_back(e)) HIP_TRY(hipEventCreateWithFlags(&e, hipEventDisableTiming));
    return PGP_OK;
}
int gemm_prof(pgp_ctx* c, int cls, GemmArgs g, hipStream_t st = nullptr);
int gemm_prof_pair(pgp_ctx* c, int cls_a, GemmArgs a, int cls_b, GemmArgs b, hipStream_t st = nullptr);
int batch_tile_list(pgp_ctx* c, int mt0, int nt, int nb, int dmt, const int** out, int* n);
inline long predict_batch_points(int option, long ns, long np) {
    const long cap = std::max<long>(16384, ((long)1 << 34) / (8 * std::max<long>(np, 1)) / 128 * 128);
    const long want = std::min<long>(option, (ns + 127) / 128 * 128);
    return std::max<long>(128, std::min<long>(want, cap));
}
struct DeviceGate {
    std::mutex m;
    std::condition_variable cv;
    int readers = 0, writers_waiting = 0;
    bool writer = false;
    void lock_shared() { std::unique_lock<std::mutex> l(m); cv.wait(l, [&] { return !writer && writers_waiting == 0; }); ++readers; }
    void unlock_shared() { std::lock_guard<std::mutex> l(m); if (--readers == 0) cv.notify_all(); }
    void lock() { std::unique_lock<std::mutex> l(m); ++writers_waiting; cv.wait(l, [&] { return !writer && readers == 0; }); --writers_waiting; writer = true; }
    void unlock() { std::lock_guard<std::mutex> l(m); writer = false; cv.notify_all(); }
};
DeviceGate& device_gate(int device);
int& device_gate_depth(int device);
struct GateShared {
    DeviceGate& g; int& depth; int state = 1;
    explicit GateShared(pgp_ctx* c) : GateShared(c ? c->device : 0) {}
    explicit GateShared(int device) : g(device_gate(device)), depth(device_gate_depth(device)) {
        if (depth++ > 0) state = 0; else g.lock_shared();
    }
    void exclusive() { if (state == 1) { g.unlock_shared(); g.lock(); state = 2; } }
    void shared_again() { if (state == 2) { g.unlock(); g.lock_shared(); state = 1; } }
    ~GateShared() { --depth; if (state == 1) g.unlock_shared(); else if (state == 2) g.unlock(); }
    GateShared(const GateShared&) = delete;
    GateShared& operator=(const GateShared&) = delete;
};
constexpr double ARD_GRAM_GRAD_BOUND = 1.0e6;
bool gram_assembly_applies(pgp_ctx* c, const CovSpec& cs);
int diag_block_factor(pgp_ctx* c, const double* src, long lds, int w, double* Fd, long ldf, double* Ed, long lde,
                      int info_base, hipStream_t st, hipEvent_t staged = nullptr);
int trtri_lower(pgp_ctx* c, const double* L, long ldl, double* W, long ldw, double* T, long np);
int lauum_lower(pgp_ctx* c, const double* W, long ldw, double* Binv, long ldb, long np);
int upload_scaled(pgp_ctx* c, const double* x_dev, long n, long d, const std::vector<double>& sc, double* XsT, long ldp,
                  int dpad, double* scale_dev);
int alloc_factor_buffer(pgp_ctx* c, long np, long ldf, double** F);
int ensure_workspace(pgp_ctx* c, long np);
int solve_lower_multi(pgp_ctx* c, const double* L, long ldl, const double* Wd, double* Y, long ldy, long np, int nrhs,
                      bool trans);
int eet_lower(pgp_ctx* c, const double* E, long lde, double* Binv, long ldb, long np);

struct GatherSrc {
    long n = 0;
    long n_pos = 0;
    const double* K_all = nullptr;
    long ld = 0;
    const int* idx = nullptr;
    const double* m_all = nullptr;
    double* y = nullptr;
    double* m = nullptr;
};
int gather_sym_launch(const GatherSrc& g, double* Kd, long np, hipStream_t st);
int ep_fit_gathered(pgp_ctx* c, const GatherSrc& g, double* nlZ_out, int* sweeps_out, pgp_factor** factor_out);
int laplace_fit_gathered(pgp_ctx* c, const GatherSrc& g, double* nlZ_out, int* steps_out, pgp_factor** factor_out);
int predict_dense_block(pgp_ctx* c, pgp_factor* f, double* Ks, long nb, int nrhs, const double* msd, double* o1, double* o2);
```

pygps_amd/csrc/gemm_f64.hip:

```cpp
#include <algorithm>
#include <atomic>

#include "gemm_tile.h"

void func_max_dynamic_lds(const void* fn, size_t bytes) {
    constexpr int MAXF = 64, MAXD = 16;
    static std::atomic<const void*> fns[MAXF];
    static std::atomic<size_t> done[MAXF][MAXD];
    int dev = 0;
    if (hipGetDevice(&dev) != hipSuccess || dev < 0 || dev >= MAXD) { (void)hipFuncSetAttribute(fn, hipFuncAttributeMaxDynamicSharedMemorySize, (int)bytes); return; }
    int slot = -1;
    for (int i = 0; i < MAXF; ++i) {
        const void* cur = fns[i].load(std::memory_order_acquire);
        if (cur == fn) { slot = i; break; }
        if (cur == nullptr) {
            const void* expect = nullptr;
            if (fns[i].compare_exchange_strong(expect, fn, std::memory_order_acq_rel) || expect == fn) { slot = i; break; }
        }
    }
    if (slot < 0) { (void)hipFuncSetAttribute(fn, hipFuncAttributeMaxDynamicSharedMemorySize, (int)bytes); return; }
    if (done[slot][dev].load(std::memory_order_acquire) >= bytes) return;
    (void)hipFuncSetAttribute(fn, hipFuncAttributeMaxDynamicSharedMemorySize, (int)bytes);
    size_t prev = done[slot][dev].load(std::memory_order_relaxed);
    while (prev < bytes && !done[slot][dev].compare_exchange_weak(prev, bytes, std::memory_order_release)) {}
}


namespace {

using gemm_tile_ns::BK;

__device__ __forceinline__ bool decode_tile(const GemmArgs& g, int b, int T, int TNc, int& ti, int& tj) {
    if (g.order) {
        ti = g.order[2 * b];
        tj = g.order[2 * b + 1];
        return ti >= 0;
    }
    if (g.tri == 2) {
        int r = (int)((sqrt(8.0 * (double)b + 1.0) - 1.0) * 0.5);
        while ((long)(r + 1) * (r + 2) / 2 <= b) ++r;
        while ((long)r * (r + 1) / 2 > b) --r;
        ti = r;
        tj = b - r * (r + 1) / 2;
        return true;
    }
    const int mt = g.M / T;
    ti = b % mt;
    tj = b / mt;
    if (g.rev_cols) tj = g.N / TNc - 1 - tj;
    if (g.rev_rows) ti = mt - 1 - ti;
    return true;
}

template <int TM, int TN, bool AKC, bool BKC, bool DMA = false, bool YIELD = false>
__global__ __launch_bounds__(256, 2) void gemm_f64_kernel(GemmArgs g) {
    extern __shared__ __attribute__((aligned(16))) double smem[];
    if (g.trace) {
        long long* tr0 = g.trace + 8L * (blockIdx.x + (long)gridDim.x * blockIdx.z);
        tr0[0] = (long long)wall_clock64();
        tr0[6] = (long long)__builtin_readcyclecounter();
    }
    int ti, tj;
    if (!decode_tile(g, (int)blockIdx.x, TM, TN, ti, tj)) return;
    long bz = blockIdx.z;
    if (g.order_z) { bz = ti >> 16; ti &= 0xffff; }
    if (g.wait_flag) {
        if (threadIdx.x == 0) {
            for (unsigned it = 0; (int)(__hip_atomic_load(g.wait_flag, __ATOMIC_ACQUIRE, __HIP_MEMORY_SCOPE_AGENT) - g.wait_target) < 0; ++it) {
                if (it > (1u << 22) || ((it & 1023u) == 1023u && __hip_atomic_load(g.wait_err, __ATOMIC_RELAXED, __HIP_MEMORY_SCOPE_AGENT))) {
                    __hip_atomic_store(g.wait_err, 1u, __ATOMIC_RELAXED, __HIP_MEMORY_SCOPE_AGENT);
                    break;
                }
                __builtin_amdgcn_s_sleep(8);
            }
        }
        __syncthreads();
    }
    if (!YIELD && g.yield_role == 2) {
        pgp_yield_mark(g.yield_flags, +1);
        gemm_tile_ns::gemm_tile<TM, TN, AKC, BKC, DMA, false>(g, ti, tj, bz, smem, (int)(blockIdx.x + gridDim.x * blockIdx.z));
        __syncthreads();
        pgp_yield_mark(g.yield_flags, -1);
        return;
    }
    gemm_tile_ns::gemm_tile<TM, TN, AKC, BKC, DMA, YIELD>(g, ti, tj, bz, smem, (int)(blockIdx.x + gridDim.x * blockIdx.z));
}

template <bool YIELD>
__global__ __launch_bounds__(256, 2) void gemm_f64_pair_kernel(GemmArgs a, GemmArgs b, int na) {
    extern __shared__ __attribute__((aligned(16))) double smem[];
    auto run = [&](const GemmArgs& g, int bid) {
        if (g.trace) {
            long long* tr0 = g.trace + 8L * bid;
            tr0[0] = (long long)wall_clock64();
            tr0[6] = (long long)__builtin_readcyclecounter();
        }
        int ti, tj;
        if (!decode_tile(g, bid, 128, 128, ti, tj)) return;
        gemm_tile_ns::gemm_tile<128, 128, false, false, true, YIELD>(g, ti, tj, 0, smem, bid);
    };
    if ((int)blockIdx.x < na) run(a, (int)blockIdx.x);
    else run(b, (int)blockIdx.x - na);
}

template <bool YIELD>
__global__ __launch_bounds__(256, 2) void gemm_f64_fold_kernel(GemmArgs g) {
    extern __shared__ __attribute__((aligned(16))) double smem[];
    const int mt = g.M / 128, half = (mt + 1) / 2;
    const int r = (int)blockIdx.x % half, tj = (int)blockIdx.x / half;
    const int hi = mt - 1 - r;
    const long bz = blockIdx.z;
    gemm_tile_ns::gemm_tile<128, 128, false, false, true, YIELD>(g, hi, tj, bz, smem, 0);
    if (hi != r) {
        __syncthreads();
        gemm_tile_ns::gemm_tile<128, 128, false, false, true, YIELD>(g, r, tj, bz, smem, 0);
    }
}

template <int T, bool AKC, bool BKC, bool DMA = false, bool YIELD = false>
int launch_t(const GemmArgs& g, hipStream_t st) {
    constexpr int SK = BK + 2;
    constexpr int ASZ = AKC ? T * SK : BK * (T + 16);
    constexpr int BSZ = BKC ? T * SK : BK * (T + 16);
    const size_t shm = 2 * (ASZ + BSZ) * sizeof(double);
    const int mt = g.M / T, nt = g.N / T;
    unsigned nblk = (g.tri == 2) ? (unsigned)((long)mt * (mt + 1) / 2) : (unsigned)(mt * nt);
    if (g.order) nblk = (unsigned)g.norder;
    dim3 grid(nblk, 1, (g.batch > 0 && !g.order_z) ? g.batch : 1);
    func_max_dynamic_lds((const void*)gemm_f64_kernel<T, T, AKC, BKC, DMA, YIELD>, shm);
    hipLaunchKernelGGL((gemm_f64_kernel<T, T, AKC, BKC, DMA, YIELD>), grid, dim3(256), shm, st, g);
    return hipGetLastError() == hipSuccess ? PGP_OK : PGP_ERR_HIP;
}

static bool dma_ok(const GemmArgs& g);
static bool dma1264_ok(const GemmArgs& g) {
    return g.tile == 1264 && dma_ok(g) && !g.tri && !g.order && g.batch <= 1 && !g.order_z && (g.N % 64) == 0 && (g.M % 128) == 0 && g.kmode == KM_FULL;
}
template <bool YIELD>
int launch_1264(const GemmArgs& g, hipStream_t st) {
    constexpr int SA_ = 128 + 16;
    const size_t shm = 2 * (BK * SA_ + (BK / 2) * SA_) * sizeof(double);
    dim3 grid((unsigned)((g.M / 128) * (g.N / 64)), 1, 1);
    func_max_dynamic_lds((const void*)gemm_f64_kernel<128, 64, false, false, true, YIELD>, shm);
    hipLaunchKernelGGL((gemm_f64_kernel<128, 64, false, false, true, YIELD>), grid, dim3(256), shm, st, g);
    return hipGetLastError() == hipSuccess ? PGP_OK : PGP_ERR_HIP;
}

static bool dma_ok(const GemmArgs& g) {
    return g.tile != 64 && (g.dbg & 64) && !g.a_kc && !g.b_kc && (g.K % 16) == 0 && (g.koff % 16) == 0 && (g.batch_dk % 16) == 0;
}

template <int T>
int launch_l(const GemmArgs& g, hipStream_t st) {
    if (!g.a_kc && !g.b_kc) return launch_t<T, false, false>(g, st);
    if (!g.a_kc && g.b_kc) return launch_t<T, false, true>(g, st);
    if (g.a_kc && !g.b_kc) return launch_t<T, true, false>(g, st);
    return launch_t<T, true, true>(g, st);
}

}

bool gemm_f64_uses_dma128(const GemmArgs& g) { return dma_ok(g) && !dma1264_ok(g); }
bool gemm_f64_uses_dma(const GemmArgs& g) { return dma_ok(g); }

static unsigned launch_blocks(const GemmArgs& g) {
    const int mt = g.M / 128, nt = g.N / 128;
    if (g.order) return (unsigned)g.norder;
    return (g.tri == 2) ? (unsigned)((long)mt * (mt + 1) / 2) : (unsigned)(mt * nt);
}
bool gemm_f64_pair_ok(const GemmArgs& a, const GemmArgs& b) {
    auto plain = [](const GemmArgs& g) {
        return g.M > 0 && g.N > 0 && g.tile != 64 && dma_ok(g) && g.batch <= 1 && !g.order_z && !g.wait_flag && g.yield_role != 2;
    };
    return plain(a) && plain(b) && (a.yield_role == 1 && a.yield_flags) == (b.yield_role == 1 && b.yield_flags);
}
int gemm_f64_launch_pair(const GemmArgs& a, const GemmArgs& b, hipStream_t st) {
    if (!gemm_f64_pair_ok(a, b)) return -2;
    constexpr int SA_ = 128 + 16;
    const size_t shm = 2 * (2 * BK * SA_) * sizeof(double);
    const unsigned na = launch_blocks(a), nb = launch_blocks(b);
    const bool yield = a.yield_role == 1 && a.yield_flags;
    func_max_dynamic_lds((const void*)(yield ? gemm_f64_pair_kernel<true> : gemm_f64_pair_kernel<false>), shm);
    if (yield) hipLaunchKernelGGL(gemm_f64_pair_kernel<true>, dim3(na + nb), dim3(256), shm, st, a, b, (int)na);
    else hipLaunchKernelGGL(gemm_f64_pair_kernel<false>, dim3(na + nb), dim3(256), shm, st, a, b, (int)na);
    return hipGetLastError() == hipSuccess ? PGP_OK : PGP_ERR_HIP;
}

static int launch_fold(const GemmArgs& g, hipStream_t st) {
    constexpr int SA_ = 128 + 16;
    const size_t shm = 2 * (2 * BK * SA_) * sizeof(double);
    const int mt = g.M / 128, nt = g.N / 128;
    dim3 grid((unsigned)(((mt + 1) / 2) * nt), 1, g.batch > 0 ? g.batch : 1);
    const bool yield = g.yield_role == 1 && g.yield_flags;
    func_max_dynamic_lds((const void*)(yield ? gemm_f64_fold_kernel<true> : gemm_f64_fold_kernel<false>), shm);
    if (yield) hipLaunchKernelGGL(gemm_f64_fold_kernel<true>, grid, dim3(256), shm, st, g);
    else hipLaunchKernelGGL(gemm_f64_fold_kernel<false>, grid, dim3(256), shm, st, g);
    return hipGetLastError() == hipSuccess ? PGP_OK : PGP_ERR_HIP;
}

int gemm_f64_launch(const GemmArgs& g, hipStream_t st) {
    if (g.M <= 0 || g.N <= 0) return PGP_OK;
    if (g.tile == 64) return launch_l<64>(g, st);
    if (g.fold_rows && g.tile == 128 && dma_ok(g) && !g.tri && !g.order && !g.order_z && !g.wait_flag && g.yield_role != 2 && !g.trace)
        return launch_fold(g, st);
    if (dma1264_ok(g)) return (g.yield_role == 1 && g.yield_flags) ? launch_1264<true>(g, st) : launch_1264<false>(g, st);
    if (dma_ok(g)) return (g.yield_role == 1 && g.yield_flags) ? launch_t<128, false, false, true, true>(g, st)
                                                               : launch_t<128, false, false, true>(g, st);
    return launch_l<128>(g, st);
}
```

pygps_amd/csrc/gemm_tile.h:

```cpp
#pragma once
#include "common.h"

typedef double double4_t __attribute__((ext_vector_type(4)));
typedef double double2_t __attribute__((ext_vector_type(2)));

namespace gemm_tile_ns {

constexpr int BK = 16;

template <int LDS_OFF>
__device__ __forceinline__ void lds_dma_1k_s(unsigned voff, const double* sbase, unsigned lds_wave_base) {
    asm volatile("s_add_u32 m0, %2, %3\n\ts_nop 0\n\tglobal_load_lds_dwordx4 %0, %1"
                 :: "v"(voff), "s"(sbase), "s"(lds_wave_base), "n"(LDS_OFF) : "memory", "scc");
}
__device__ __forceinline__ const double* uniform_ptr(const double* p) {
    const unsigned long a = (unsigned long)p;
    const unsigned lo = __builtin_amdgcn_readfirstlane((unsigned)a), hi = __builtin_amdgcn_readfirstlane((unsigned)(a >> 32));
    return (const double*)(((unsigned long)hi << 32) | lo);
}
template <int V> struct IC { static constexpr int value = V; };

__device__ __forceinline__ double swap_adjacent(double v) {
    const int lo = __builtin_amdgcn_update_dpp(0, __double2loint(v), 0xB1, 0xF, 0xF, false);
    const int hi = __builtin_amdgcn_update_dpp(0, __double2hiint(v), 0xB1, 0xF, 0xF, false);
    return __hiloint2double(hi, lo);
}

__device__ __noinline__ void gemm_yield_wait(const unsigned* yf) {
    for (int i = 0; i < 400; ++i) {
        __builtin_amdgcn_s_sleep(32);
        if (__hip_atomic_load(yf, __ATOMIC_RELAXED, __HIP_MEMORY_SCOPE_AGENT) == 0u) break;
    }
}

template <int TM, int TN, bool AKC, bool BKC, bool DMA = false, bool YIELD = false>
__device__ __forceinline__ void gemm_tile(const GemmArgs& g, int ti, int tj, long bz, double* __restrict__ smem, int wg = 0) {
    static_assert(!DMA || (!AKC && !BKC && TM == 128 && (TN == 128 || TN == 64)), "LDS-DMA staging: M-contiguous operands, 128 x 128 or 128 x 64 tiles");
    constexpr bool BH = DMA && TN == 64;
    constexpr int SA = TM + 16, SB = BH ? TM + 16 : TN + 16, SK = BK + 2;
    constexpr int ASZ = AKC ? TM * SK : BK * SA;
    constexpr int BSZ = BKC ? TN * SK : (BH ? (BK / 2) * SB : BK * SB);
    constexpr int STAGE = ASZ + BSZ;
    constexpr int FM = TM / 32, FN = TN / 32;
    constexpr int AV = TM * BK / 2 / 256;
    constexpr int BV = TN * BK / 2 / 256;

    const int i0 = ti * TM, j0 = tj * TN;
    if (g.batch_dm && i0 >= g.M - (int)bz * g.batch_dm) return;
    const int zero_from = g.zero_from > 0 ? g.zero_from - (int)bz * g.batch_dm : 0;
    if (i0 < g.skip_hi && j0 < g.skip_hi && i0 >= g.skip_lo && j0 >= g.skip_lo) return;
    bool diag = false;
    if (g.tri) {
        if (i0 + g.tri_off < j0) return;
        diag = g.mask_diag && (i0 + g.tri_off == j0);
    }
    int k0 = 0, k1 = g.K;
    const int koff = g.koff + (int)bz * g.batch_dk;
    if (g.kmode == KM_GE_I) k0 = i0 + koff;
    else if (g.kmode == KM_GE_J) k0 = j0 + koff;
    else if (g.kmode == KM_LT_I) k1 = i0 + TM + koff;
    else if (g.kmode == KM_LT_J) k1 = j0 + TN + koff;
    if (g.zf_upper && zero_from > 0 && i0 >= zero_from && i0 - zero_from > k0) k0 = i0 - zero_from;
    if (k0 < 0) k0 = 0;
    if (k1 > g.K) k1 = g.K;
    k0 &= ~(BK - 1);

    const bool a_hi = g.a_split && i0 >= g.a_split;
    const bool c_hi = g.c_split && i0 >= g.c_split;
    const double* __restrict__ A = (a_hi ? g.A2 - g.a_split : g.A) + bz * g.sA;
    const long lda = a_hi ? g.lda2 : g.lda;
    const double* __restrict__ B = g.B + bz * g.sB;
    double* __restrict__ C = (c_hi ? g.C2 - g.c_split : g.C) + bz * g.sC - (bz * (bz - 1) / 2) * g.batch_sC2;
    const long ldc = (c_hi ? g.ldc2 : g.ldc) - bz * g.batch_dldc;
    const double* __restrict__ Cin = g.Cin ? (c_hi ? g.Cin2 - g.c_split : g.Cin) : C;
    const long ldcin = g.Cin ? (c_hi ? g.ldcin2 : g.ldcin) : ldc;

    const int t = threadIdx.x;
    const int lane = t & 63, wave = t >> 6;
    const int wm = (wave & 1) * (TM / 2), wn = (wave >> 1) * (TN / 2);
    const int l15 = lane & 15, l4 = lane >> 4;

    double4_t acc[FM][FN];
    const double ab = g.beta / g.alpha;
    const bool wantc = g.beta != 0.0 && !(zero_from > 0 && i0 >= zero_from);
    constexpr int LZ = 16;
    const bool lazyc = DMA && wantc && (g.dbg & 256) && (k1 - k0) >= (LZ + 2) * BK;
    const bool preload = wantc && !lazyc;
#pragma unroll
    for (int im = 0; im < FM; ++im)
#pragma unroll
        for (int in = 0; in < FN; ++in) {
            if (preload) {
                const double* cp = Cin + (long)(i0 + wm + im * 16 + l15) + (long)(j0 + wn + in * 16 + l4) * ldcin;
#pragma unroll
                for (int r = 0; r < 4; ++r) acc[im][in][r] = ab * cp[(long)(4 * r) * ldcin];
            } else {
#pragma unroll
                for (int r = 0; r < 4; ++r) acc[im][in][r] = 0.0;
            }
        }

    double2_t ra[AV], rb[BV];
    const double* pa[AV];
    const double* pb[BV];
    long astep, bstep;
    if (!AKC) {
        constexpr int VPR = TM / 2, RPP = 256 / VPR;
#pragma unroll
        for (int p = 0; p < AV; ++p) pa[p] = A + (long)(i0 + 2 * (t % VPR)) + (long)(k0 + t / VPR + p * RPP) * lda;
        astep = (long)BK * lda;
    } else {
#pragma unroll
        for (int p = 0; p < AV; ++p) pa[p] = A + (long)(k0 + 2 * (t & 7)) + (long)(i0 + (t >> 3) + p * 32) * lda;
        astep = BK;
    }
    if (!BKC) {
        constexpr int VPR = TN / 2, RPP = 256 / VPR;
#pragma unroll
        for (int p = 0; p < BV; ++p) pb[p] = B + (long)(j0 + 2 * (t % VPR)) + (long)(k0 + t / VPR + p * RPP) * g.ldb;
        bstep = (long)BK * g.ldb;
    } else {
#pragma unroll
        for (int p = 0; p < BV; ++p) pb[p] = B + (long)(k0 + 2 * (t & 7)) + (long)(j0 + (t >> 3) + p * 32) * g.ldb;
        bstep = BK;
    }
    const double* da[4];
    const double* db[4];
    unsigned lds_w = 0;
    const unsigned dvoff = (unsigned)lane * 16u;
    unsigned dvoff_b = dvoff;
    if constexpr (BH) dvoff_b = (unsigned)(lane & 31) * 16u + (unsigned)(lane >> 5) * (unsigned)(4L * g.ldb * 8L);
    const unsigned smem_lds = (unsigned)(unsigned long)(__attribute__((address_space(3))) void*)smem;
    if constexpr (DMA) {
        static_assert(SA == SB, "one LDS row stride for both operands");
#pragma unroll
        for (int p = 0; p < 4; ++p) {
            da[p] = uniform_ptr(A + (long)i0 + (long)(k0 + wave + 4 * p) * lda);
            db[p] = uniform_ptr(B + (long)j0 + (long)(k0 + wave + (BH ? 8 * (p & 1) : 4 * p)) * g.ldb);
        }
        lds_w = __builtin_amdgcn_readfirstlane(smem_lds + (unsigned)wave * (unsigned)(SA * 8));
    }
    const long dstep_a = (long)BK * lda, dstep_b = (long)BK * g.ldb;
    auto dma_stage = [&](auto bufc) {
        constexpr int O = decltype(bufc)::value * STAGE * 8;
        if constexpr (DMA && BH) {
            lds_dma_1k_s<O + 0 * SA * 8>(dvoff, da[0], lds_w);
            lds_dma_1k_s<O + ASZ * 8 + 0 * SB * 8>(dvoff_b, db[0], lds_w);
            lds_dma_1k_s<O + 4 * SA * 8>(dvoff, da[1], lds_w);
            lds_dma_1k_s<O + 8 * SA * 8>(dvoff, da[2], lds_w);
            lds_dma_1k_s<O + ASZ * 8 + 4 * SB * 8>(dvoff_b, db[1], lds_w);
            lds_dma_1k_s<O + 12 * SA * 8>(dvoff, da[3], lds_w);
#pragma unroll
            for (int p = 0; p < 4; ++p) da[p] += dstep_a;
            db[0] += dstep_b; db[1] += dstep_b;
        } else if constexpr (DMA) {
            lds_dma_1k_s<O + 0 * SA * 8>(dvoff, da[0], lds_w);
            lds_dma_1k_s<O + ASZ * 8 + 0 * SB * 8>(dvoff, db[0], lds_w);
            lds_dma_1k_s<O + 4 * SA * 8>(dvoff, da[1], lds_w);
            lds_dma_1k_s<O + ASZ * 8 + 4 * SB * 8>(dvoff, db[1], lds_w);
            lds_dma_1k_s<O + 8 * SA * 8>(dvoff, da[2], lds_w);
            lds_dma_1k_s<O + ASZ * 8 + 8 * SB * 8>(dvoff, db[2], lds_w);
            lds_dma_1k_s<O + 12 * SA * 8>(dvoff, da[3], lds_w);
            lds_dma_1k_s<O + ASZ * 8 + 12 * SB * 8>(dvoff, db[3], lds_w);
#pragma unroll
            for (int p = 0; p < 4; ++p) { da[p] += dstep_a; db[p] += dstep_b; }
        }
    };
    auto gload = [&](int) {
#pragma unroll
        for (int p = 0; p < AV; ++p) { ra[p] = *(const double2_t*)pa[p]; pa[p] += astep; }
#pragma unroll
        for (int p = 0; p < BV; ++p) { rb[p] = *(const double2_t*)pb[p]; pb[p] += bstep; }
    };
    auto sstore = [&](int buf) {
        double* sa = smem + buf * STAGE;
        double* sb = sa + ASZ;
        if (!AKC) {
            constexpr int VPR = TM / 2;
            constexpr int RPP = 256 / VPR;
#pragma unroll
            for (int p = 0; p < AV; ++p) {
                const int mv = t % VPR, kr = t / VPR + p * RPP;
                *(double2_t*)(sa + kr * SA + 2 * mv) = ra[p];
            }
        } else {
#pragma unroll
            for (int p = 0; p < AV; ++p) {
                const int kp = t & 7, m = (t >> 3) + p * 32;
                *(double2_t*)(sa + m * SK + 2 * kp) = ra[p];
            }
        }
        if (!BKC) {
            constexpr int VPR = TN / 2;
            constexpr int RPP = 256 / VPR;
#pragma unroll
            for (int p = 0; p < BV; ++p) {
                const int nv = t % VPR, kr = t / VPR + p * RPP;
                *(double2_t*)(sb + kr * SB + 2 * nv) = rb[p];
            }
        } else {
#pragma unroll
            for (int p = 0; p < BV; ++p) {
                const int kp = t & 7, n = (t >> 3) + p * 32;
                *(double2_t*)(sb + n * SK + 2 * kp) = rb[p];
            }
        }
    };

    if (k0 < k1) {
        if constexpr (DMA) {
            dma_stage(IC<0>{});
            asm volatile("s_waitcnt vmcnt(0)" ::: "memory");
        } else {
            gload(k0);
            sstore(0);
        }
        __syncthreads();
        double fa[2][FM], fb[2][FN];
        auto ldfrag = [&](int b, int ks, int slot) {
            const double* sa = smem + b * STAGE;
            const double* sb = sa + ASZ;
            const int k = ks * 4 + l4;
#pragma unroll
            for (int im = 0; im < FM; ++im) {
                const int m = wm + im * 16 + l15;
                fa[slot][im] = AKC ? sa[m * SK + k] : sa[k * SA + m];
            }
#pragma unroll
            for (int in = 0; in < FN; ++in) {
                const int n = wn + in * 16 + l15;
                if constexpr (BH) fb[slot][in] = sb[(l4 + 4 * (ks >> 1)) * SB + (ks & 1) * 64 + n];
                else fb[slot][in] = BKC ? sb[n * SK + k] : sb[k * SB + n];
            }
        };
        auto mfmas = [&](int slot) {
#pragma unroll
            for (int in = 0; in < FN; ++in)
#pragma unroll
                for (int im = 0; im < FM; ++im)
                    acc[im][in] = __builtin_amdgcn_mfma_f64_16x16x4f64(fb[slot][in], fa[slot][im], acc[im][in], 0, 0, 0);
        };
        constexpr int NS = BK / 4;
        ldfrag(0, 0, 0);
        const unsigned* yf = nullptr;
        if constexpr (YIELD) yf = g.yield_flags + pgp_cu_key();
        auto kstep = [&](int kt, auto bufc, auto pollc) {
            constexpr int buf = decltype(bufc)::value;
            constexpr bool POLL = YIELD && decltype(pollc)::value != 0;
            const bool more = kt + BK < k1;
            if constexpr (DMA) { if (more) dma_stage(IC<(buf ^ 1)>{}); }
            else if (more) gload(kt + BK);
            unsigned yv = 0u;
            if constexpr (POLL) yv = __hip_atomic_load(yf, __ATOMIC_RELAXED, __HIP_MEMORY_SCOPE_AGENT);
#pragma unroll
            for (int ks = 0; ks + 1 < NS; ++ks) {
                ldfrag(buf, ks + 1, (ks + 1) & 1);
                mfmas(ks & 1);
            }
            if constexpr (DMA) asm volatile("s_waitcnt vmcnt(0)" ::: "memory");
            else if (more) sstore(buf ^ 1);
            __syncthreads();
            if constexpr (POLL) { if (__builtin_amdgcn_readfirstlane(yv) != 0u) gemm_yield_wait(yf); }
            if (more) ldfrag(buf ^ 1, 0, NS & 1);
            __builtin_amdgcn_sched_barrier(0);
            mfmas((NS - 1) & 1);
        };
        int kt = k0;
        if constexpr (DMA) {
            if (lazyc) {
                double4_t creg[2];
                static_assert(FM == 4 && (FN == 4 || FN == 2), "lazy C: 64-row wave tiles, 64 or 32 columns");
                const int my_half = __builtin_amdgcn_readfirstlane(wave >> 1);
#pragma unroll
                for (int st = 0; st < LZ; ++st) {
                    const int chunk = (BH ? (st & 7) : st) >> 1, in = chunk / (FM / 2), hf = chunk % (FM / 2);
                    const bool act = !BH || my_half == (st >> 3);
                    if (!(st & 1)) {
                        if (act) {
#pragma unroll
                        for (int q = 0; q < 2; ++q) {
                            const double* cp = Cin + (long)(i0 + wm + (2 * hf + q) * 16 + l15) + (long)(j0 + wn + in * 16 + l4) * ldcin;
#pragma unroll
                            for (int r = 0; r < 4; ++r) creg[q][r] = cp[(long)(4 * r) * ldcin];
                        }
                        }
                    } else if (act) {
#pragma unroll
                        for (int q = 0; q < 2; ++q)
#pragma unroll
                            for (int r = 0; r < 4; ++r) acc[2 * hf + q][in][r] = fma(ab, creg[q][r], acc[2 * hf + q][in][r]);
                    }
                    if (st & 1) kstep(kt, IC<1>{}, IC<0>{});
                    else if ((st & 3) == 0) kstep(kt, IC<0>{}, IC<1>{});
                    else kstep(kt, IC<0>{}, IC<0>{});
                    kt += BK;
                }
            }
        }
        while (kt < k1) {
            kstep(kt, IC<0>{}, IC<1>{});
            kt += BK;
            if (kt >= k1) break;
            kstep(kt, IC<1>{}, IC<0>{});
            kt += BK;
            if constexpr (YIELD) {
                if (kt >= k1) break;
                kstep(kt, IC<0>{}, IC<0>{});
                kt += BK;
                if (kt >= k1) break;
                kstep(kt, IC<1>{}, IC<0>{});
                kt += BK;
            }
        }
    }

    long long* const trc = g.trace ? g.trace + 8L * wg : nullptr;
    if (trc) trc[2] = (long long)wall_clock64();
    if (!diag && (g.dbg & 512) && !(ldc & 1) && !((unsigned long)C & 15ul)) {
        const bool odd = l15 & 1;
#pragma unroll
        for (int im = 0; im < FM; ++im)
#pragma unroll
            for (int in = 0; in < FN; ++in) {
                const int m = wm + im * 16 + l15;
                const int nb = wn + in * 16 + l4;
#pragma unroll
                for (int r = 0; r < 4; r += 2) {
                    const double x = g.alpha * acc[im][in][r], yv = g.alpha * acc[im][in][r + 1];
                    const double nx = swap_adjacent(x), ny = swap_adjacent(yv);
                    const double2_t val = odd ? double2_t{ny, yv} : double2_t{x, nx};
                    double* cp = C + (long)(i0 + (odd ? m - 1 : m)) + (long)(j0 + nb + 4 * (odd ? r + 1 : r)) * ldc;
                    *(double2_t*)cp = val;
                }
            }
    } else {
#pragma unroll
    for (int im = 0; im < FM; ++im)
#pragma unroll
        for (int in = 0; in < FN; ++in) {
            const int m = wm + im * 16 + l15;
            const int nb = wn + in * 16 + l4;
            double* cp = C + (long)(i0 + m) + (long)(j0 + nb) * ldc;
#pragma unroll
            for (int r = 0; r < 4; ++r) {
                const int n = nb + 4 * r;
                if (!diag || m >= n) cp[(long)(4 * r) * ldc] = g.alpha * acc[im][in][r];
            }
        }
    }
    if (trc) {
        trc[3] = (long long)wall_clock64();
        asm volatile("s_waitcnt vmcnt(0)" ::: "memory");
        __syncthreads();
        trc[4] = (long long)wall_clock64(); trc[5] = (long long)pgp_cu_key(); trc[7] = (long long)__builtin_readcyclecounter();
    }
}

}
```

pygps_amd/csrc/testhooks.h:

```cpp
#pragma once
#include <stdint.h>

#include "../../include/pygps_amd.h"
#ifdef __cplusplus
extern "C" {
#endif
int pgp_test_gemm(pgp_ctx* ctx, int tile, int a_kc, int b_kc, int tri, int mask_diag, int kmode, int koff,
                  double alpha, double beta, const double* A, int64_t lda, const double* B, int64_t ldb,
                  double* C, int64_t ldc, int M, int N, int K, int iters, double* ms_out);
int pgp_test_gemm_shrink(pgp_ctx* ctx, const double* Y, int64_t ldy, int M, int K, int w, int nb, int dm, int zero_from,
                         double* C, int64_t ldc, int64_t sC);
int pgp_test_gemm_zskip(pgp_ctx* ctx, int tile, int tri, int mask_diag, int zero_from, int zf_upper, double alpha, double beta,
                        const double* A, int64_t lda, const double* B, int64_t ldb, const double* Cin, double* C, int64_t ldc,
                        int M, int N, int K);
int pgp_test_gemm_skip_wait(pgp_ctx* ctx, int tile, const double* A, const double* B, double* C, int n, int K, int skip_lo,
                            int skip_hi, int wait_ms, int* timed_out);
int pgp_test_probit_hazard(pgp_ctx* ctx, const double* z, double* out, int n);
int pgp_test_laplace_lik(pgp_ctx* ctx, int lik, double log_sn, const double* y, const double* f, int n, double* out);
int pgp_test_laplace_ep_lik(pgp_ctx* ctx, const double* y, const double* mu, const double* s2, const double* sn, int n, double* out);
int pgp_test_valu_peak(pgp_ctx* ctx, int iters, int waves_per_simd, double* out2);
int pgp_test_mfma_peak(pgp_ctx* ctx, int iters, double* tflops_out);
int pgp_test_mfma_cycles(pgp_ctx* ctx, int iters, int nacc, int waves_per_simd, double* out3);
int pgp_test_leaf_ticks(pgp_ctx* ctx, double* ticks_out );
int pgp_test_wave_costs(pgp_ctx* ctx, double* out16);
int pgp_test_slot_probe(pgp_ctx* ctx, int nwg, int lds_kb, int hold_us, int reserve, int probe_lds_kb, int delay_us, double* out4);
int pgp_test_cumask_gemm(pgp_ctx* ctx, int M, int K, int reserve_per_xcd, int stride, int iters, double* out2);
int pgp_test_assemble(pgp_ctx* ctx, int kind, int mode, int64_t n, int64_t d, int iters, double* ms_out);
int pgp_test_gemm_trace(pgp_ctx* ctx, int M, int K, int tri, int warm, int conc, long long* out, int64_t out_words, int64_t* nblk_out);
int pgp_test_read_gemm_trace(pgp_ctx* ctx, long long* out, int64_t words, int64_t* nwg);
int pgp_test_store_roof(pgp_ctx* ctx, int64_t n, int grid, int iters, double* out3);
int pgp_test_hadamard(pgp_ctx* ctx, int kind, const double* hyp, int ncov, int para, int flags, const double* Binv,
                      const double* alpha, const double* wv, double sn2, double* out);
int pgp_test_stream_concurrency(pgp_ctx* ctx, int wait_us, double* out2);
int pgp_test_gather_sym(pgp_ctx* ctx, const double* K, int64_t n, const int32_t* idx, int64_t n_idx, int64_t n_pos,
                        const double* m_all, double* Kd_out, double* y_out, double* m_out);
int pgp_test_vote(pgp_ctx* ctx, const double* fmu, const double* fs2, int64_t ns, int n_class, int ci, int cj, double* votes_out,
                  double* norm_out);
int pgp_test_yield_table(pgp_ctx* ctx, uint32_t* out4096);
#ifdef __cplusplus
}
#endif
```

pygps_amd/csrc/testhooks.hip:

```cpp
#include <time.h>
#include <cstdlib>
#include <cmath>
#include <vector>

#include "ctx.h"
#include <chrono>
#include <thread>

#include "testhooks.h"
#include "erf_lik.h"
#include "laplace_lik.h"

typedef double double4_t __attribute__((ext_vector_type(4)));

namespace {
__global__ __launch_bounds__(256) void mfma_peak_kernel(double* out, int iters, double a0, double b0) {
    double4_t acc[8];
#pragma unroll
    for (int i = 0; i < 8; ++i) acc[i] = double4_t{0.0, 0.0, 0.0, 0.0};
    double a = a0 + threadIdx.x * 1e-9, b = b0;
    for (int it = 0; it < iters; ++it) {
#pragma unroll
        for (int i = 0; i < 8; ++i) acc[i] = __builtin_amdgcn_mfma_f64_16x16x4f64(a, b, acc[i], 0, 0, 0);
    }
// ... 52 lines not shown
    long long h[2];
    HIP_TRY(hipMemcpy(h, d, 16, hipMemcpyDeviceToHost));
    out3[0] = (double)h[0]; out3[1] = (double)h[1]; out3[2] = ms;
    (void)hipEventDestroy(e0); (void)hipEventDestroy(e1); (void)hipFree(d);
    return PGP_OK;
}

__global__ __launch_bounds__(256) void valu_peak_kernel(double* out, int iters, double a0, double b0) {
    double s[16], a[4], b[4];
    for (int i = 0; i < 16; ++i) s[i] = 0.0;
    for (int i = 0; i < 4; ++i) { a[i] = a0 + threadIdx.x * 1e-3 + i; b[i] = b0 + i * 0.5; }
    for (int it = 0; it < iters; ++it) {
#pragma unroll
        for (int i = 0; i < 4; ++i)
#pragma unroll
            for (int j = 0; j < 4; ++j) {
                const double d = a[i] - b[j];
                s[4 * i + j] = fma(d, d, s[4 * i + j]);
            }
#pragma unroll
        for (int i = 0; i < 4; ++i) { a[i] += 1e-9; }
    }
    double t = 0.0;
    for (int i = 0; i < 16; ++i) t += s[i];
    if (t == 12345.678) out[0] = t;
}

int pgp_test_valu_peak(pgp_ctx* c, int iters, int waves_per_simd, double* out2) {
    if (!c || !out2) return -1;
    HIP_TRY(hipSetDevice(c->device));
    double* out = nullptr;
    HIP_TRY(hipMalloc((void**)&out, 8));
    hipEvent_t e0, e1;
    HIP_TRY(hipEventCreate(&e0)); HIP_TRY(hipEventCreate(&e1));
    const int blocks = c->prop.multiProcessorCount * waves_per_simd;
    hipLaunchKernelGGL(valu_peak_kernel, dim3(blocks), dim3(256), 0, c->st, out, 64, 1.0, 1.0);
    HIP_TRY(hipEventRecord(e0, c->st));
    hipLaunchKernelGGL(valu_peak_kernel, dim3(blocks), dim3(256), 0, c->st, out, iters, 1.0, 1.0);
    HIP_TRY(hipEventRecord(e1, c->st));
    HIP_TRY(hipStreamSynchronize(c->st));
    float ms = 0.f;
    HIP_TRY(hipEventElapsedTime(&ms, e0, e1));
    const double winstr = (double)blocks * 4.0 * (double)iters * 36.0;
    const double per_simd = (double)waves_per_simd * (double)iters * 36.0;
    out2[0] = winstr / (ms * 1e6);
    out2[1] = (ms * 1e-3) * 2.4e9 / per_simd;
    (void)hipEventDestroy(e0); (void)hipEventDestroy(e1); (void)hipFree(out);
    return PGP_OK;
}

int pgp_test_mfma_peak(pgp_ctx* ctx, int iters, double* tflops_out) {
    if (!ctx || !tflops_out) return -1;
    pgp_ctx* c = ctx;
    HIP_TRY(hipSetDevice(c->device));
    hipDeviceProp_t prop;
    HIP_TRY(hipGetDeviceProperties(&prop, c->device));
    double* out = nullptr;
    HIP_TRY(hipMalloc((void**)&out, 8));
    hipEvent_t e0, e1;
    HIP_TRY(hipEventCreate(&e0)); HIP_TRY(hipEventCreate(&e1));
    const int blocks = prop.multiProcessorCount * 2;
    hipLaunchKernelGGL(mfma_peak_kernel, dim3(blocks), dim3(256), 0, c->st, out, 16, 1.0, 1.0);
    HIP_TRY(hipEventRecord(e0, c->st));
    hipLaunchKernelGGL(mfma_peak_kernel, dim3(blocks), dim3(256), 0, c->st, out, iters, 1.0, 1.0);
    HIP_TRY(hipEventRecord(e1, c->st));
    HIP_TRY(hipStreamSynchronize(c->st));
    float ms = 0.f;
    HIP_TRY(hipEventElapsedTime(&ms, e0, e1));
    const double flops = (double)blocks * 4.0 * (double)iters * 8.0 * 2048.0;
    *tflops_out = flops / (ms * 1e-3) / 1e12;
    (void)hipEventDestroy(e0); (void)hipEventDestroy(e1); (void)hipFree(out);
    return PGP_OK;
}

int pgp_test_leaf_ticks(pgp_ctx* c, double* ticks_out) {
    if (!c || !ticks_out) return -1;
    HIP_TRY(hipSetDevice(c->device));
    std::vector<double> A(128 * 128, 0.0);
    for (int i = 0; i < 128; ++i)
        for (int j = 0; j < 128; ++j) A[i + j * 128] = (i == j ? 3.0 : 0.0) + 1.0 / (1.0 + (i > j ? i - j : j - i));
    double *Ad, *pk; int* info; long long* tk;
    HIP_TRY(hipMalloc((void**)&Ad, A.size() * 8)); HIP_TRY(hipMalloc((void**)&pk, PACK_DOUBLES * 8));
    HIP_TRY(hipMalloc((void**)&info, 4)); HIP_TRY(hipMalloc((void**)&tk, 24 * 8));
    HIP_TRY(hipMemset(info, 0, 4)); HIP_TRY(hipMemset(tk, 0, 24 * 8));
    for (int rep = 0; rep < 3; ++rep) {
        HIP_TRY(hipMemcpy(Ad, A.data(), A.size() * 8, hipMemcpyHostToDevice));
        int rc = leaf_potrf_launch(Ad, 128, pk, info, 0, c->st, tk, nullptr, c->leaf_pivot);
        if (rc) return rc;
        HIP_TRY(hipStreamSynchronize(c->st));
    }
    long long h[24];
    HIP_TRY(hipMemcpy(h, tk, sizeof(h), hipMemcpyDeviceToHost));
    for (int i = 0; i < 24; ++i) ticks_out[i] = (double)h[i];
    (void)hipFree(Ad); (void)hipFree(pk); (void)hipFree(info); (void)hipFree(tk);
    return PGP_OK;
}

namespace {
__global__ __launch_bounds__(256) void wave_costs_kernel(double* __restrict__ out, double seed) {
    __shared__ double lds[512];
    __shared__ int nxt[256];
    const int t = threadIdx.x;
    lds[t] = seed + t; lds[t + 256] = seed - t; nxt[t] = (t * 7 + 1) & 255;
    __syncthreads();
    long long a, b, ra, rb;
    double x = seed, acc = 0.0;
    a = __builtin_amdgcn_s_memtime(); ra = __builtin_amdgcn_s_memrealtime();
#pragma unroll 16
    for (int i = 0; i < 2048; ++i) x = fma(x, 0.999999, 1e-9);
    acc += x;
    asm volatile("" :: "v"(x));
    b = __builtin_amdgcn_s_memtime(); rb = __builtin_amdgcn_s_memrealtime();
    if (t == 0) { out[0] = (double)(b - a) / 2048.0; out[1] = (double)(rb - ra); out[9] = (double)(b - a); }
    double y[8];
#pragma unroll
    for (int q = 0; q < 8; ++q) y[q] = seed + q;
    a = __builtin_amdgcn_s_memtime();
    for (int i = 0; i < 256; ++i) {
#pragma unroll
        for (int q = 0; q < 8; ++q) y[q] = fma(y[q], 0.999999, 1e-9);
    }
#pragma unroll
    for (int q = 0; q < 8; ++q) acc += y[q];
    asm volatile("" :: "v"(acc));
    b = __builtin_amdgcn_s_memtime();
    if (t == 0) out[2] = (double)(b - a) / 2048.0;
    int idx = t;
    a = __builtin_amdgcn_s_memtime();
    for (int i = 0; i < 512; ++i) idx = nxt[idx];
    asm volatile("" :: "v"(idx));
    b = __builtin_amdgcn_s_memtime();
    if (t == 0) out[3] = (double)(b - a) / 512.0;
    acc += idx;
    a = __builtin_amdgcn_s_memtime();
    for (int i = 0; i < 512; ++i) {
        double sum = 0.0;
        const int o = (i & 1) * 256;
#pragma unroll
        for (int q = 0; q < 20; ++q) sum += lds[o + ((t >> 4) + 16 * q) % 256];
        acc = fma(sum, 1e-9, acc);
        asm volatile("" :: "v"(acc));
    }
    b = __builtin_amdgcn_s_memtime();
    if (t == 0) out[4] = (double)(b - a) / 512.0;
    a = __builtin_amdgcn_s_memtime();
    for (int i = 0; i < 512; ++i) __syncthreads();
    b = __builtin_amdgcn_s_memtime();
    if (t == 0) out[5] = (double)(b - a) / 512.0;
    a = __builtin_amdgcn_s_memtime();
    for (int i = 0; i < 512; ++i) {
        if ((t & 15) == (i & 15)) lds[(i & 1) * 256 + (t >> 4)] = acc + i;
        __syncthreads();
        acc += lds[(i & 1) * 256 + (i & 15)];
        asm volatile("" :: "v"(acc));
    }
    b = __builtin_amdgcn_s_memtime();
    if (t == 0) out[6] = (double)(b - a) / 512.0;
    x = seed + 2.0;
    a = __builtin_amdgcn_s_memtime();
#pragma unroll 16
    for (int i = 0; i < 512; ++i) x = __builtin_amdgcn_rcp(x) + 1.5;
    asm volatile("" :: "v"(x));
    b = __builtin_amdgcn_s_memtime();
    if (t == 0) out[7] = (double)(b - a) / 512.0;
    acc += x;
    x = seed + 2.0;
    a = __builtin_amdgcn_s_memtime();
#pragma unroll 16
    for (int i = 0; i < 512; ++i) x = __builtin_amdgcn_rsq(x) + 1.5;
    asm volatile("" :: "v"(x));
    b = __builtin_amdgcn_s_memtime();
    if (t == 0) out[8] = (double)(b - a) / 512.0;
    acc += x;
    if (acc == 12345.678 && t == 0) out[15] = acc;
}
}
int pgp_test_wave_costs(pgp_ctx* c, double* out16) {
    if (!c || !out16) return -1;
    HIP_TRY(hipSetDevice(c->device));
    double* od;
    HIP_TRY(hipMalloc((void**)&od, 16 * 8));
    HIP_TRY(hipMemset(od, 0, 16 * 8));
    for (int rep = 0; rep < 3; ++rep) hipLaunchKernelGGL(wave_costs_kernel, dim3(1), dim3(256), 0, c->st, od, 1.0 + 1e-3 * rep);
    HIP_TRY(hipStreamSynchronize(c->st));
    HIP_TRY(hipMemcpy(out16, od, 16 * 8, hipMemcpyDeviceToHost));
    (void)hipFree(od);
    return PGP_OK;
}

int pgp_test_assemble(pgp_ctx* c, int kind, int mode, int64_t n, int64_t d, int iters, double* ms_out) {
    if (!c || !ms_out) return -1;
    HIP_TRY(hipSetDevice(c->device));
    const long np = round_up(n, 128);
    const int dpad = (int)round_up(d, SKC);
    std::vector<double> x((size_t)n * d);
    unsigned long long s = 88172645463325252ULL;
    for (auto& v : x) { s ^= s << 13; s ^= s >> 7; s ^= s << 17; v = ((double)(s >> 11) / 9007199254740992.0 - 0.5) * 3.4; }
    std::vector<double> hyp(kind == PGP_COV_RBFARD ? d + 1 : 2, 0.0);
    for (size_t i = 0; i + 1 < hyp.size(); ++i) hyp[i] = 0.5 * log((double)d);
    CovSpec cp;
    CHK(make_spec(c, kind, hyp.data(), (int)hyp.size(), 3, 0, -1, d, cp));
    const std::vector<double>& sc = cp.scale;
    double *xd, *XT, *scd, *out;
    const long ldo = mode == 2 ? np + 128 : n;
    HIP_TRY(hipMalloc((void**)&xd, x.size() * 8)); HIP_TRY(hipMalloc((void**)&XT, (size_t)dpad * np * 8));
    HIP_TRY(hipMalloc((void**)&scd, dpad * 8)); HIP_TRY(hipMalloc((void**)&out, (size_t)ldo * np * 8));
    HIP_TRY(hipMemcpy(xd, x.data(), x.size() * 8, hipMemcpyHostToDevice));
    HIP_TRY(hipMemcpy(scd, sc.data(), d * 8, hipMemcpyHostToDevice));
    CHK(scale_transpose_launch(xd, n, (int)d, scd, XT, np, dpad, c->st));
    const bool gram = c->gram_assembly && cov_gram_applies(cp, dpad);
    double* prep = nullptr;
    if (gram) HIP_TRY(hipMalloc((void**)&prep, (size_t)hadamard_prep_count(np) * 8));
    hipEvent_t e0, e1;
    HIP_TRY(hipEventCreate(&e0)); HIP_TRY(hipEventCreate(&e1));
    int rc = PGP_OK;
    for (int it = -std::max(100, iters); it < iters && rc == PGP_OK; ++it) {
        if (it == 0) HIP_TRY(hipEventRecord(e0, c->st));
        if (gram) {
            rc = hadamard_prepare_launch(XT, np, n, np, dpad, cp, prep, c->st, true);
            if (rc == PGP_OK) rc = mode == 2 ? cov_factor_gram_launch(XT, np, n, np, dpad, cp, 100.0, out, ldo, prep, c->st)
                                             : cov_sym_gram_launch(XT, np, n, dpad, cp, out, 0, prep, c->st);
        } else
        rc = mode == 2 ? cov_factor_launch(XT, np, n, np, dpad, cp, 100.0, out, ldo, c->st)
                       : cov_sym_launch(XT, np, n, dpad, cp, out, c->st, 0);
    }
    HIP_TRY(hipEventRecord(e1, c->st));
    HIP_TRY(hipStreamSynchronize(c->st));
    float ms = 0.f;
    HIP_TRY(hipEventElapsedTime(&ms, e0, e1));
    *ms_out = ms / iters;
    (void)hipEventDestroy(e0); (void)hipEventDestroy(e1);
    (void)hipFree(xd); (void)hipFree(XT); (void)hipFree(scd); (void)hipFree(out);
    if (prep) (void)hipFree(prep);
    return rc;
}

namespace {
__global__ __launch_bounds__(256) void store_only_sym_kernel(double* out, long n, const int2* tab, long ntiles, double v) {
    const int t = threadIdx.x;
    for (long ti = blockIdx.x; ti < ntiles; ti += gridDim.x) {
        const int2 ij = tab[ti];
        double* base = out + (long)ij.x * 64 * n + (long)ij.y * 64;
        double* mir = out + (long)ij.y * 64 * n + (long)ij.x * 64;
#pragma unroll
        for (int p = 0; p < 8; ++p) {
            const int e = t + 256 * p, r = e >> 5, cpair = e & 31;
            *(double2_t*)(base + (long)r * n + 2 * cpair) = double2_t{v, v + 1.0};
        }
        if (ij.x != ij.y) {
#pragma unroll
            for (int p = 0; p < 8; ++p) {
                const int e = t + 256 * p, r = e >> 5, cpair = e & 31;
                *(double2_t*)(mir + (long)r * n + 2 * cpair) = double2_t{v, v + 1.0};
            }
        }
    }
}
__global__ __launch_bounds__(256) void store_only_linear_kernel(double* out, long n2, double v) {
    const long i = ((long)blockIdx.x * 256 + threadIdx.x) * 2;
    if (i + 1 < n2) *(double2_t*)(out + i) = double2_t{v, v + 1.0};
}
}

int pgp_test_store_roof(pgp_ctx* c, int64_t n, int grid, int iters, double* out3) {
    if (!c || !out3 || n <= 0 || n % 64 || iters <= 0) return -1;
    HIP_TRY(hipSetDevice(c->device));
    const long nt = n / 64, S = 8, nst = (nt + S - 1) / S;
    std::vector<int2> h;
    for (long SI = 0; SI < nst; ++SI)
        for (long SJ = SI; SJ < nst; ++SJ)
            for (long i = SI * S; i < std::min(nt, SI * S + S); ++i)
                for (long j = std::max(i, SJ * S); j < std::min(nt, SJ * S + S); ++j) h.push_back(make_int2((int)i, (int)j));
    int2* tab; double* out;
    HIP_TRY(hipMalloc((void**)&tab, h.size() * sizeof(int2)));
    HIP_TRY(hipMalloc((void**)&out, (size_t)n * n * 8));
    HIP_TRY(hipMemcpy(tab, h.data(), h.size() * sizeof(int2), hipMemcpyHostToDevice));
    hipEvent_t e0, e1;
    HIP_TRY(hipEventCreate(&e0)); HIP_TRY(hipEventCreate(&e1));
    const long ntl = (long)h.size(), n2 = (long)n * n;
    const unsigned g = (unsigned)std::min<long>(ntl, grid > 0 ? grid : 4096);
    for (int which = 0; which < 3; ++which) {
        for (int it = -std::max(50, iters / 2); it < iters; ++it) {
            if (it == 0) HIP_TRY(hipEventRecord(e0, c->st));
            if (which == 0) hipLaunchKernelGGL(store_only_sym_kernel, dim3(g), dim3(256), 0, c->st, out, (long)n, tab, ntl, 1.0);
            else if (which == 1) HIP_TRY(hipMemsetAsync(out, 0, (size_t)n2 * 8, c->st));
            else hipLaunchKernelGGL(store_only_linear_kernel, dim3((unsigned)((n2 / 2 + 255) / 256)), dim3(256), 0, c->st, out, n2, 1.0);
        }
        HIP_TRY(hipEventRecord(e1, c->st));
        HIP_TRY(hipStreamSynchronize(c->st));
        float ms = 0.f;
        HIP_TRY(hipEventElapsedTime(&ms, e0, e1));
        out3[which] = ms / iters;
    }
    (void)hipEventDestroy(e0); (void)hipEventDestroy(e1);
    (void)hipFree(tab); (void)hipFree(out);
    return hipGetLastError() == hipSuccess ? PGP_OK : PGP_ERR_HIP;
}

int pgp_test_gemm(pgp_ctx* ctx, int tile, int a_kc, int b_kc, int tri, int mask_diag, int kmode, int koff,
                  double alpha, double beta, const double* A, int64_t lda, const double* B, int64_t ldb, double* C,
                  int64_t ldc, int M, int N, int K, int iters, double* ms_out) {
    if (!ctx) return -1;
    pgp_ctx* c = ctx;
    HIP_TRY(hipSetDevice(c->device));
    const size_t an = (size_t)lda * (a_kc ? M : K), bn = (size_t)ldb * (b_kc ? N : K), cn = (size_t)ldc * N;
    double *Ad, *Bd, *Cd;
    HIP_TRY(hipMalloc((void**)&Ad, an * 8)); HIP_TRY(hipMalloc((void**)&Bd, bn * 8)); HIP_TRY(hipMalloc((void**)&Cd, cn * 8));
    HIP_TRY(hipMemcpy(Ad, A, an * 8, hipMemcpyHostToDevice));
    HIP_TRY(hipMemcpy(Bd, B, bn * 8, hipMemcpyHostToDevice));
    HIP_TRY(hipMemcpy(Cd, C, cn * 8, hipMemcpyHostToDevice));
    GemmArgs g{};
    g.A = Ad; g.lda = lda; g.a_kc = a_kc; g.B = Bd; g.ldb = ldb; g.b_kc = b_kc; g.C = Cd; g.ldc = ldc;
    g.M = M; g.N = N; g.K = K; g.alpha = alpha; g.beta = beta; g.tri = tri; g.tri_off = 0; g.mask_diag = mask_diag;
    g.kmode = kmode; g.koff = koff; g.batch = 1; g.tile = tile; g.dbg = c->gemm_dbg;
    if (getenv("PGP_TEST_GEMM_FOLD")) g.fold_rows = 1;
    hipStream_t ts = c->st;
    int rc = gemm_f64_launch(g, ts);
    HIP_TRY(hipStreamSynchronize(ts));
    if (rc == PGP_OK) HIP_TRY(hipMemcpy(C, Cd, cn * 8, hipMemcpyDeviceToHost));
    if (rc == PGP_OK && iters > 0 && ms_out) {
        hipEvent_t e0, e1;
        HIP_TRY(hipEventCreate(&e0)); HIP_TRY(hipEventCreate(&e1));
        {
            HIP_TRY(hipEventRecord(e0, ts));
            rc = gemm_f64_launch(g, ts);
            HIP_TRY(hipEventRecord(e1, ts));
            HIP_TRY(hipStreamSynchronize(ts));
            float m1 = 0.f;
            HIP_TRY(hipEventElapsedTime(&m1, e0, e1));
            const int nwarm = (int)std::min(4000.0, std::max(1.0, 80.0 / std::max(1e-3, (double)m1)));
            for (int i = 0; i < nwarm && rc == PGP_OK; ++i) rc = gemm_f64_launch(g, ts);
        }
        HIP_TRY(hipEventRecord(e0, ts));
        for (int i = 0; i < iters; ++i) rc = gemm_f64_launch(g, ts);
        HIP_TRY(hipEventRecord(e1, ts));
        HIP_TRY(hipStreamSynchronize(ts));
        float ms = 0.f;
        HIP_TRY(hipEventElapsedTime(&ms, e0, e1));
        *ms_out = ms / iters;
        (void)hipEventDestroy(e0); (void)hipEventDestroy(e1);
    }
    (void)hipFree(Ad); (void)hipFree(Bd); (void)hipFree(Cd);
    return rc;
}

int pgp_test_gemm_trace(pgp_ctx* c, int M, int K, int tri, int warm, int conc, long long* out, int64_t out_words, int64_t* nblk_out) {
    if (!c || !out || !nblk_out || M % 128 || K % 16) return -1;
    HIP_TRY(hipSetDevice(c->device));
    const long mt = M / 128;
    const long nblk = tri ? mt * (mt + 1) / 2 : mt * mt;
    if (out_words < 8 * nblk) return -2;
    double *A, *Cd, *C2; long long* tr;
    HIP_TRY(hipMalloc((void**)&A, (size_t)M * K * 8)); HIP_TRY(hipMalloc((void**)&Cd, (size_t)M * M * 8));
    HIP_TRY(hipMalloc((void**)&C2, (size_t)M * M * 8)); HIP_TRY(hipMalloc((void**)&tr, (size_t)nblk * 64));
    HIP_TRY(hipMemset(tr, 0, (size_t)nblk * 64));
    std::vector<double> h((size_t)M * K);
    unsigned long long s = 88172645463325252ULL;
    for (auto& v : h) { s ^= s << 13; s ^= s >> 7; s ^= s << 17; v = ((double)(s >> 11) / 9007199254740992.0 - 0.5) * 0.01; }
    HIP_TRY(hipMemcpy(A, h.data(), h.size() * 8, hipMemcpyHostToDevice));
    HIP_TRY(hipMemset(Cd, 0, (size_t)M * M * 8)); HIP_TRY(hipMemset(C2, 0, (size_t)M * M * 8));
    GemmArgs g{};
    g.A = A; g.lda = M; g.B = A; g.ldb = M; g.C = Cd; g.ldc = M; g.M = M; g.N = M; g.K = K; g.alpha = -1.0; g.beta = 1.0;
    g.tri = tri ? 2 : 0; g.mask_diag = tri ? 1 : 0; g.batch = 1; g.tile = 128; g.dbg = c->gemm_dbg;
    int rc = PGP_OK;
    for (int i = 0; i < warm && rc == PGP_OK; ++i) rc = gemm_f64_launch(g, c->st);
    HIP_TRY(hipStreamSynchronize(c->st));
    GemmArgs g2 = g; g2.C = C2;
    if (conc > 0 && rc == PGP_OK) rc = gemm_f64_launch(g2, c->st2);
    g.trace = tr;
    if (rc == PGP_OK) rc = gemm_f64_launch(g, c->st);
    HIP_TRY(hipStreamSynchronize(c->st)); HIP_TRY(hipStreamSynchronize(c->st2));
    HIP_TRY(hipMemcpy(out, tr, (size_t)nblk * 64, hipMemcpyDeviceToHost));
    *nblk_out = nblk;
    (void)hipFree(A); (void)hipFree(Cd); (void)hipFree(C2); (void)hipFree(tr);
    return rc;
}

int pgp_test_read_gemm_trace(pgp_ctx* c, long long* out, int64_t words, int64_t* nwg) {
    if (!c || !out || !nwg || !c->gemm_trace) return -1;
    HIP_TRY(hipSetDevice(c->device));
    HIP_TRY(hipDeviceSynchronize());
    const long n = std::min<long>(c->gemm_trace_pos, words / 8);
    HIP_TRY(hipMemcpy(out, c->gemm_trace, (size_t)n * 64, hipMemcpyDeviceToHost));
    HIP_TRY(hipMemset(c->gemm_trace, 0, (size_t)c->gemm_trace_cap * 64));
    c->gemm_trace_pos = 0;
    *nwg = n;
    return PGP_OK;
}

int pgp_test_gemm_skip_wait(pgp_ctx* ctx, int tile, const double* A, const double* B, double* C, int n, int K, int skip_lo,
                            int skip_hi, int wait_ms, int* timed_out) {
    if (!ctx) return -1;
    pgp_ctx* c = ctx;
    HIP_TRY(hipSetDevice(c->device));
    DevScratch scr;
    double *Ad = nullptr, *Bd = nullptr, *Cd = nullptr;
    unsigned* fl = nullptr;
    const size_t an = (size_t)n * K * 8, cn = (size_t)n * n * 8;
    CHK(scr.alloc(&Ad, an)); CHK(scr.alloc(&Bd, an)); CHK(scr.alloc(&Cd, cn));
    CHK(scr.alloc(&fl, 16));
    HIP_TRY(hipMemcpy(Ad, A, an, hipMemcpyHostToDevice));
    HIP_TRY(hipMemcpy(Bd, B, an, hipMemcpyHostToDevice));
    HIP_TRY(hipMemcpy(Cd, C, cn, hipMemcpyHostToDevice));
    HIP_TRY(hipMemset(fl, 0, 16));
    GemmArgs g{};
    g.A = Ad; g.lda = n; g.B = Bd; g.ldb = n; g.C = Cd; g.ldc = n; g.M = n; g.N = n; g.K = K; g.alpha = -1.0; g.beta = 1.0;
    g.tri = 2; g.mask_diag = 1; g.batch = 1; g.tile = tile; g.dbg = c->gemm_dbg; g.skip_lo = skip_lo; g.skip_hi = skip_hi;
    if (wait_ms > 0) { g.wait_flag = fl; g.wait_target = 7u; g.wait_err = fl + 1; }
    int rc = gemm_f64_launch(g, c->st);
    if (rc == PGP_OK && wait_ms > 0) {
        std::this_thread::sleep_for(std::chrono::milliseconds(wait_ms));
        const unsigned seven = 7u;
        HIP_TRY(hipMemcpyAsync(fl, &seven, sizeof(seven), hipMemcpyHostToDevice, c->st2));
        HIP_TRY(hipStreamSynchronize(c->st2));
    }
    HIP_TRY(hipStreamSynchronize(c->st));
    unsigned flh[2] = {0u, 0u};
    HIP_TRY(hipMemcpy(flh, fl, sizeof(flh), hipMemcpyDeviceToHost));
    if (timed_out) *timed_out = (int)flh[1];
    if (rc == PGP_OK) HIP_TRY(hipMemcpy(C, Cd, cn, hipMemcpyDeviceToHost));
    return rc;
}

int pgp_test_gemm_shrink(pgp_ctx* ctx, const double* Y, int64_t ldy, int M, int K, int w, int nb, int dm, int zero_from,
                         double* C, int64_t ldc, int64_t sC) {
    if (!ctx) return -1;
    pgp_ctx* c = ctx;
    if (!Y || !C || M <= 0 || M % 128 || w % 128 || K % 16 || dm % 128 || nb < 1) return -2;
    HIP_TRY(hipSetDevice(c->device));
    DevScratch scr;
    double *yd, *cd;
    const size_t cbytes = (size_t)((nb - 1) * sC + ldc * w) * 8;
    CHK(scr.alloc(&yd, (size_t)ldy * K * 8)); CHK(scr.alloc(&cd, cbytes));
    HIP_TRY(hipMemcpy(yd, Y, (size_t)ldy * K * 8, hipMemcpyHostToDevice));
    HIP_TRY(hipMemcpy(cd, C, cbytes, hipMemcpyHostToDevice));
    GemmArgs g{};
    g.A = yd; g.lda = ldy; g.B = yd; g.ldb = ldy; g.C = cd; g.ldc = ldc; g.M = M; g.N = w; g.K = K;
    g.alpha = -1.0; g.beta = 1.0; g.tri = 1; g.mask_diag = 1; g.kmode = KM_FULL; g.tile = 128;
    g.batch = nb; g.sA = dm; g.sB = dm; g.sC = sC; g.batch_dm = dm; g.zero_from = zero_from;
    CHK(gemm_prof(c, PC_GEMM_TRAIL, g, c->st));
    HIP_TRY(hipStreamSynchronize(c->st));
    HIP_TRY(hipMemcpy(C, cd, cbytes, hipMemcpyDeviceToHost));
    return PGP_OK;
}

int pgp_test_gemm_zskip(pgp_ctx* ctx, int tile, int tri, int mask_diag, int zero_from, int zf_upper, double alpha, double beta,
                        const double* A, int64_t lda, const double* B, int64_t ldb, const double* Cin, double* C, int64_t ldc,
                        int M, int N, int K) {
    if (!ctx) return -1;
    pgp_ctx* c = ctx;
    if (!A || !B || !C || M <= 0 || N <= 0 || M % 128 || N % 128 || K % 16 || lda < M || ldb < N || ldc < M) return -2;
    if ((tile != 64 && tile != 128) || zero_from < 0 || zero_from % 128) return -2;
    HIP_TRY(hipSetDevice(c->device));
    DevScratch scr;
    double *Ad = nullptr, *Bd = nullptr, *Cd = nullptr, *Ci = nullptr;
    const size_t an = (size_t)lda * K * 8, bn = (size_t)ldb * K * 8, cn = (size_t)ldc * N * 8;
    CHK(scr.alloc(&Ad, an)); CHK(scr.alloc(&Bd, bn)); CHK(scr.alloc(&Cd, cn));
    HIP_TRY(hipMemcpy(Ad, A, an, hipMemcpyHostToDevice));
    HIP_TRY(hipMemcpy(Bd, B, bn, hipMemcpyHostToDevice));
    HIP_TRY(hipMemcpy(Cd, C, cn, hipMemcpyHostToDevice));
    if (Cin) { CHK(scr.alloc(&Ci, cn)); HIP_TRY(hipMemcpy(Ci, Cin, cn, hipMemcpyHostToDevice)); }
    GemmArgs g{};
    g.A = Ad; g.lda = lda; g.B = Bd; g.ldb = ldb; g.C = Cd; g.ldc = ldc; g.M = M; g.N = N; g.K = K; g.alpha = alpha; g.beta = beta;
    if (Ci) { g.Cin = Ci; g.ldcin = ldc; }
    g.tri = tri; g.mask_diag = mask_diag; g.kmode = KM_FULL; g.batch = 1; g.tile = tile; g.dbg = c->gemm_dbg;
    g.zero_from = zero_from; g.zf_upper = zf_upper;
    const int rc = gemm_f64_launch(g, c->st);
    HIP_TRY(hipStreamSynchronize(c->st));
    if (rc == PGP_OK) HIP_TRY(hipMemcpy(C, Cd, cn, hipMemcpyDeviceToHost));
    return rc;
}

}

namespace {
__device__ unsigned g_probe_claim[16];
__device__ unsigned g_probe_cnt[4];
__device__ long long g_probe_t[4];
__device__ unsigned g_probe_log[4 * 2048];
__global__ void holder_kernel(long long hold_ticks, int reserve) {
    extern __shared__ double hs[];
    __shared__ int leave;
    if (threadIdx.x == 0) {
        int mine = 0;
        if (reserve > 0) {
            const unsigned hw = __builtin_amdgcn_s_getreg((4 << 0) | (0 << 6) | (31 << 11));
            const unsigned xcc = __builtin_amdgcn_s_getreg((20 << 0) | (0 << 6) | (3 << 11)) & 15u;
            const unsigned key = 1u + ((hw >> 8) & 0xffu);
            const unsigned prev = atomicCAS(&g_probe_claim[xcc], 0u, key);
            mine = prev == 0u || prev == key;
        }
        leave = mine;
        atomicAdd(&g_probe_cnt[mine ? 1 : 0], 1u);
        if (blockIdx.x < 2048) {
            const unsigned hw = __builtin_amdgcn_s_getreg((4 << 0) | (0 << 6) | (31 << 11));
            const unsigned xcc = __builtin_amdgcn_s_getreg((20 << 0) | (0 << 6) | (3 << 11));
            g_probe_log[4 * blockIdx.x] = hw; g_probe_log[4 * blockIdx.x + 1] = xcc; g_probe_log[4 * blockIdx.x + 2] = mine;
            g_probe_log[4 * blockIdx.x + 3] = (unsigned)(wall_clock64() & 0xffffffffu);
        }
        if (blockIdx.x == 0) g_probe_t[0] = wall_clock64();
    }
    __syncthreads();
    if (leave) return;
    hs[threadIdx.x] = 1.0;
    const long long t0 = wall_clock64();
    while (wall_clock64() - t0 < hold_ticks) __builtin_amdgcn_s_sleep(20);
}
__global__ void probe_kernel() {
    extern __shared__ double ps[];
    if (threadIdx.x == 0) { g_probe_t[1] = wall_clock64(); ps[0] = 1.0; }
}
__global__ void probe_mark_kernel() { if (threadIdx.x == 0) g_probe_t[2] = wall_clock64(); }
}

extern "C" int pgp_test_slot_probe(pgp_ctx* c, int nwg, int lds_kb, int hold_us, int reserve, int probe_lds_kb, int delay_us,
                                   double* out4) {
    if (!c || !out4) return -1;
    HIP_TRY(hipSetDevice(c->device));
    unsigned zero16[16] = {0}; unsigned zero4[4] = {0}; long long zt[4] = {0, 0, 0, 0};
    HIP_TRY(hipMemcpyToSymbol(HIP_SYMBOL(g_probe_claim), zero16, sizeof(zero16)));
    HIP_TRY(hipMemcpyToSymbol(HIP_SYMBOL(g_probe_cnt), zero4, sizeof(zero4)));
    HIP_TRY(hipMemcpyToSymbol(HIP_SYMBOL(g_probe_t), zt, sizeof(zt)));
    (void)hipFuncSetAttribute((const void*)holder_kernel, hipFuncAttributeMaxDynamicSharedMemorySize, 160 * 1024);
    (void)hipFuncSetAttribute((const void*)probe_kernel, hipFuncAttributeMaxDynamicSharedMemorySize, 160 * 1024);
    HIP_TRY(hipDeviceSynchronize());
    hipLaunchKernelGGL(holder_kernel, dim3(nwg), dim3(256), (size_t)lds_kb * 1024, c->st, (long long)hold_us * 100, reserve);
    struct timespec ts = {0, (long)delay_us * 1000};
    nanosleep(&ts, nullptr);
    hipLaunchKernelGGL(probe_mark_kernel, dim3(1), dim3(64), 0, c->st2);
    hipLaunchKernelGGL(probe_kernel, dim3(1), dim3(256), (size_t)probe_lds_kb * 1024, c->st2);
    HIP_TRY(hipDeviceSynchronize());
    unsigned cnt[4]; long long t[4];
    HIP_TRY(hipMemcpyFromSymbol(cnt, HIP_SYMBOL(g_probe_cnt), sizeof(cnt)));
    HIP_TRY(hipMemcpyFromSymbol(t, HIP_SYMBOL(g_probe_t), sizeof(t)));
    out4[0] = (double)(t[1] - t[2]) / 100.0; out4[1] = cnt[0]; out4[2] = cnt[1]; out4[3] = (double)(t[1] - t[0]) / 100.0;
    if (getenv("PGP_PROBE_DUMP")) {
        static unsigned lg[4 * 2048];
        HIP_TRY(hipMemcpyFromSymbol(lg, HIP_SYMBOL(g_probe_log), sizeof(lg)));
        for (int i = 0; i < nwg && i < 2048; ++i)
            fprintf(stderr, "wg %4d hw %08x cu %2u sh %u se %u xcc %08x leave %u t %u\n", i, lg[4 * i], (lg[4 * i] >> 8) & 15u, (lg[4 * i] >> 12) & 1u,
                    (lg[4 * i] >> 13) & 7u, lg[4 * i + 1], lg[4 * i + 2], lg[4 * i + 3] - lg[3]);
    }
    return PGP_OK;
}

extern "C" int pgp_test_cumask_gemm(pgp_ctx* c, int M, int K, int reserve_per_xcd, int stride, int iters, double* out2) {
    if (!c || !out2) return -1;
    HIP_TRY(hipSetDevice(c->device));
    const int ncu = c->prop.multiProcessorCount;
    std::vector<uint32_t> mask((ncu + 31) / 32, 0u);
    int kept = 0;
    for (int i = 0; i < ncu; ++i) {
        const int within = stride == 8 ? i / 8 : i % (ncu / 8);
        const bool keep = within >= reserve_per_xcd;
        if (keep) { mask[i / 32] |= 1u << (i % 32); ++kept; }
    }
    hipStream_t ms = nullptr;
    HIP_TRY(hipExtStreamCreateWithCUMask(&ms, (uint32_t)mask.size(), mask.data()));
    DevScratch scr;
    double *A, *Cm;
    CHK(scr.alloc(&A, (size_t)M * K * 8)); CHK(scr.alloc(&Cm, (size_t)M * M * 8));
    HIP_TRY(hipMemset(A, 0, (size_t)M * K * 8)); HIP_TRY(hipMemset(Cm, 0, (size_t)M * M * 8));
    GemmArgs g{};
    g.A = A; g.lda = M; g.B = A; g.ldb = M; g.C = Cm; g.ldc = M; g.M = M; g.N = M; g.K = K;
    g.alpha = -1.0; g.beta = 1.0; g.tile = 128; g.batch = 1; g.dbg = c->gemm_dbg;
    hipEvent_t e0, e1;
    HIP_TRY(hipEventCreate(&e0)); HIP_TRY(hipEventCreate(&e1));
    hipStream_t sts[2] = {ms, c->st};
    for (int s = 0; s < 2; ++s) {
        for (int i = 0; i < 3; ++i) CHK(gemm_f64_launch(g, sts[s]));
        HIP_TRY(hipStreamSynchronize(sts[s]));
        HIP_TRY(hipEventRecord(e0, sts[s]));
        for (int i = 0; i < iters; ++i) CHK(gemm_f64_launch(g, sts[s]));
        HIP_TRY(hipEventRecord(e1, sts[s]));
        HIP_TRY(hipStreamSynchronize(sts[s]));
        float t = 0.f;
        HIP_TRY(hipEventElapsedTime(&t, e0, e1));
        out2[s] = t / iters;
    }
    (void)hipEventDestroy(e0); (void)hipEventDestroy(e1);
    (void)hipStreamDestroy(ms);
    return kept;
}

__global__ void pgp_probe_spin_kernel(unsigned* flag, long long wait_ticks, long long* out) {
    const long long t0 = (long long)wall_clock64();
    long long t = t0;
    unsigned seen = 0u;
    while ((t = (long long)wall_clock64()) - t0 < wait_ticks) {
        if (__hip_atomic_load(flag, __ATOMIC_RELAXED, __HIP_MEMORY_SCOPE_AGENT)) { seen = 1u; break; }
        __builtin_amdgcn_s_sleep(16);
    }
    if (threadIdx.x == 0) { out[0] = (long long)seen; out[1] = t - t0; }
}
__global__ void pgp_probe_set_kernel(unsigned* flag) { __hip_atomic_store(flag, 1u, __ATOMIC_RELAXED, __HIP_MEMORY_SCOPE_AGENT); }
extern "C" int pgp_test_stream_concurrency(pgp_ctx* c, int wait_us, double* out2) {
    if (!c || !out2) return -1;
    HIP_TRY(hipSetDevice(c->device));
    DevScratch scr;
    double* buf;
    CHK(scr.alloc(&buf, 64));
    HIP_TRY(hipMemset(buf, 0, 64));
    unsigned* flag = (unsigned*)buf;
    long long* res = (long long*)(buf + 2);
    hipLaunchKernelGGL(pgp_probe_spin_kernel, dim3(1), dim3(64), 0, c->st2, flag, (long long)wait_us * 100LL, res);
    hipLaunchKernelGGL(pgp_probe_set_kernel, dim3(1), dim3(1), 0, c->st, flag);
    HIP_TRY(hipStreamSynchronize(c->st2));
    HIP_TRY(hipStreamSynchronize(c->st));
    long long h[2] = {0, 0};
    HIP_TRY(hipMemcpy(h, res, sizeof(h), hipMemcpyDeviceToHost));
    out2[0] = (double)h[0]; out2[1] = (double)h[1] / 100.0;
    return PGP_OK;
}

namespace {
__global__ void laplace_lik_test_kernel(int lik, double sn2, const double* __restrict__ y, const double* __restrict__ f,
                                        double* __restrict__ out, int n) {
    const int i = blockIdx.x * blockDim.x + threadIdx.x;
    if (i >= n) return;
    double lp, d1, d2, d3;
    if (lik == PGP_LIK_GAUSS) gauss_laplace_derivs(y[i], f[i], sn2, &lp, &d1, &d2, &d3);
    else erf_laplace_derivs(y[i], f[i], &lp, &d1, &d2, &d3);
    out[i] = lp; out[n + i] = d1; out[2L * n + i] = d2; out[3L * n + i] = d3;
}
}

extern "C" int pgp_test_laplace_lik(pgp_ctx* c, int lik, double log_sn, const double* y, const double* f, int n, double* out) {
    if (!c || !y || !f || !out || n <= 0) return -1;
    if (lik != PGP_LIK_ERF && lik != PGP_LIK_GAUSS) return -2;
    HIP_TRY(hipSetDevice(c->device));
    DevScratch scr;
    double *yd, *fd, *od;
    CHK(scr.alloc(&yd, (size_t)n * 8)); CHK(scr.alloc(&fd, (size_t)n * 8)); CHK(scr.alloc(&od, (size_t)4 * n * 8));
    HIP_TRY(hipMemcpy(yd, y, (size_t)n * 8, hipMemcpyHostToDevice));
    HIP_TRY(hipMemcpy(fd, f, (size_t)n * 8, hipMemcpyHostToDevice));
    hipLaunchKernelGGL(laplace_lik_test_kernel, dim3((unsigned)((n + 255) / 256)), dim3(256), 0, c->st, lik, exp(2.0 * log_sn), yd, fd, od, n);
    HIP_TRY(hipStreamSynchronize(c->st));
    HIP_TRY(hipMemcpy(out, od, (size_t)4 * n * 8, hipMemcpyDeviceToHost));
    return PGP_OK;
}

namespace {
__global__ void laplace_ep_lik_test_kernel(const double* __restrict__ in, double* __restrict__ out, int n) {
    const int i = blockIdx.x * blockDim.x + threadIdx.x;
    if (i >= n) return;
    const double y = in[i], mu = in[n + i], s2 = in[2L * n + i], sn = in[3L * n + i];
    double lZ, dlZ, d2lZ;
    laplace_ep_moments(y, mu, s2, sn, &lZ, &dlZ, &d2lZ);
    out[i] = lZ; out[n + i] = dlZ; out[2L * n + i] = d2lZ; out[3L * n + i] = laplace_ep_dlZhyp(y, mu, s2, sn);
}
}

extern "C" int pgp_test_laplace_ep_lik(pgp_ctx* c, const double* y, const double* mu, const double* s2, const double* sn, int n,
                                       double* out) {
    if (!c || !y || !mu || !s2 || !sn || !out || n <= 0) return -1;
    HIP_TRY(hipSetDevice(c->device));
    DevScratch scr;
    double *id, *od;
    CHK(scr.alloc(&id, (size_t)4 * n * 8)); CHK(scr.alloc(&od, (size_t)4 * n * 8));
    const double* src[4] = {y, mu, s2, sn};
    for (int q = 0; q < 4; ++q) HIP_TRY(hipMemcpy(id + (size_t)q * n, src[q], (size_t)n * 8, hipMemcpyHostToDevice));
    hipLaunchKernelGGL(laplace_ep_lik_test_kernel, dim3((unsigned)((n + 255) / 256)), dim3(256), 0, c->st, id, od, n);
    HIP_TRY(hipGetLastError());
    HIP_TRY(hipStreamSynchronize(c->st));
    HIP_TRY(hipMemcpy(out, od, (size_t)4 * n * 8, hipMemcpyDeviceToHost));
    return PGP_OK;
}

extern "C" int pgp_test_hadamard(pgp_ctx* c, int kind, const double* hyp, int ncov, int para, int flags, const double* Binv,
                                 const double* alpha, const double* wv, double sn2, double* out) {
    if (!c) return -1;
    GateShared device_gate_hold(c);
    if (c->n <= 0) return -1;
    if (!hyp || !Binv || !alpha || !out) return -2;
    HIP_TRY(hipSetDevice(c->device));
    const long n = c->n, d = c->d, np = c->np;
    CovSpec cp;
    CHK(make_spec(c, kind, hyp, ncov, para, flags, -1, d, cp));
    if (cp.ncov != ncov) return -11;
    hipStream_t st = c->st;
    const double nan = std::nan("");
    std::vector<double> hB((size_t)np * np, nan), ha(np, nan), hw(np, nan);
    for (long r = 0; r < n; ++r)
        for (long q = r; q < n; ++q) hB[(size_t)r * np + q] = Binv[(size_t)r * n + q];
    for (long r = 0; r < n; ++r) { ha[r] = alpha[r]; if (wv) hw[r] = wv[r]; }
    PoolScratch tmp(c);
    double *XsT = nullptr, *scd = nullptr, *Bd = nullptr, *ad = nullptr, *wd = nullptr, *partial = nullptr, *prep = nullptr,
           *od = nullptr;
    CHK(tmp.alloc(&XsT, (size_t)c->dpad * np * sizeof(double)));
    CHK(tmp.alloc(&scd, (size_t)c->dpad * sizeof(double)));
    CHK(tmp.alloc(&Bd, (size_t)np * np * sizeof(double)));
    CHK(tmp.alloc(&ad, (size_t)np * sizeof(double)));
    if (wv) CHK(tmp.alloc(&wd, (size_t)np * sizeof(double)));
    CHK(tmp.alloc(&partial, (size_t)hadamard_partial_count(np, ncov) * sizeof(double)));
    CHK(tmp.alloc(&prep, (size_t)hadamard_prep_count(np) * sizeof(double)));
    CHK(tmp.alloc(&od, (size_t)(ncov + 1) * sizeof(double)));
    HIP_TRY(hipMemcpyAsync(Bd, hB.data(), hB.size() * sizeof(double), hipMemcpyHostToDevice, st));
    HIP_TRY(hipMemcpyAsync(ad, ha.data(), np * sizeof(double), hipMemcpyHostToDevice, st));
    if (wv) HIP_TRY(hipMemcpyAsync(wd, hw.data(), np * sizeof(double), hipMemcpyHostToDevice, st));
    CHK(upload_scaled(c, c->x_dev, n, d, cp.scale, XsT, np, c->dpad, scd));
    const bool gram = gram_assembly_applies(c, cp);
    if (gram) CHK(hadamard_prepare_launch(XsT, np, n, np, c->dpad, cp, prep, st, true));
    CHK(hadamard_reduce_launch(XsT, np, n, np, c->dpad, cp, ncov, sn2, Bd, np, ad, partial, od, st, wd, gram ? prep : nullptr));
    HIP_TRY(hipMemcpyAsync(out, od, (size_t)(ncov + 1) * sizeof(double), hipMemcpyDeviceToHost, st));
    HIP_TRY(hipStreamSynchronize(st));
    return PGP_OK;
}

extern "C" int pgp_test_yield_table(pgp_ctx* c, uint32_t* out4096) {
    if (!c || !out4096) return -1;
    if (!c->yield_flags) return -2;
    GateShared device_gate_hold(c);
    HIP_TRY(hipSetDevice(c->device));
    HIP_TRY(hipStreamSynchronize(c->st));
    if (c->st2) HIP_TRY(hipStreamSynchronize(c->st2));
    HIP_TRY(hipMemcpy(out4096, c->yield_flags, 4096 * sizeof(uint32_t), hipMemcpyDeviceToHost));
    return PGP_OK;
}
```

Before: 109.4 fits/s.

## Add ring-staged LDS-DMA pipeline to f64 GEMM tile loop

Adds a RING template path to the LDS-DMA GEMM tile kernels. It splits operand staging into finer pieces and issues them ahead of the MFMA steps, using counted vmcnt waits instead of full vmcnt(0) drains. The lazy C-input loads are also interleaved into the prologue. The path is enabled by default through a new tile_ring option and is threaded through the plain, pair, fold and 1264 launchers. In exchange it uses hand-written asm waits and a written-out prologue, which bring correctness risk and register pressure, and it adds a small LDS spare.

```diff
diff --git a/pygps_amd/_lib.py b/pygps_amd/_lib.py
--- a/pygps_amd/_lib.py
+++ b/pygps_amd/_lib.py
@@ -103,6 +103,8 @@
                                        _i64]),
     "pgp_test_gemm_zskip": (C.c_int, [_vp] + [C.c_int] * 5 + [C.c_double, C.c_double, _dp, _i64, _dp, _i64, _dp, _dp, _i64,
                                       C.c_int, C.c_int, C.c_int]),
+    "pgp_test_gemm_pair": (C.c_int, [_vp, C.c_double, C.c_double, _dp, _i64, _dp, _i64, _dp, _dp, _i64, C.c_int, C.c_int, C.c_int,
+                                     C.c_int]),
     "pgp_test_gemm_skip_wait": (C.c_int, [_vp, C.c_int, _dp, _dp, _dp, C.c_int, C.c_int, C.c_int, C.c_int, C.c_int,
                                           C.POINTER(C.c_int)]),
     "pgp_test_probit_hazard": (C.c_int, [_vp, _dp, _dp, C.c_int]),
diff --git a/pygps_amd/csrc/capi.hip b/pygps_amd/csrc/capi.hip
--- a/pygps_amd/csrc/capi.hip
+++ b/pygps_amd/csrc/capi.hip
@@ -175,6 +175,7 @@
     if (!strcmp(name, "trtri_small_tile_below")) { c->trtri_small_tile_below = value; return PGP_OK; }
     if (!strcmp(name, "xcd_order")) { c->xcd_order = value; return PGP_OK; }
     if (!strcmp(name, "gemm_dbg")) { if (value & ~(64 | 256 | 512)) return -2; c->gemm_dbg = value; return PGP_OK; }
+    if (!strcmp(name, "tile_ring")) { if (value < 0 || value > 1) return -2; c->tile_ring = value; return PGP_OK; }
     if (!strcmp(name, "lookahead")) { c->lookahead = value; return PGP_OK; }
     if (!strcmp(name, "leaf_first")) { c->leaf_first = value; return PGP_OK; }
     if (!strcmp(name, "leaf_pivot")) { if (value < 0 || value > 2) return -2; c->leaf_pivot = value; return PGP_OK; }
@@ -596,6 +597,7 @@
         g.yield_flags = c->yield_flags;
         if (g.yield_role != 2) g.yield_role = gemm_f64_uses_dma(g) ? 1 : 0;
     } else g.yield_role = 0;
+    g.ring = c->tile_ring && gemm_f64_uses_dma(g) ? 1 : 0;
     if (c->gemm_trace && gemm_f64_uses_dma128(g) && g.batch == 1) {
         const long mt = g.M / 128, nt = g.N / 128;
         const long nb = g.order ? g.norder : (g.tri == 2 ? mt * (mt + 1) / 2 : mt * nt);
diff --git a/pygps_amd/csrc/common.h b/pygps_amd/csrc/common.h
--- a/pygps_amd/csrc/common.h
+++ b/pygps_amd/csrc/common.h
@@ -42,6 +42,7 @@
     int norder;
     int order_z;
     int dbg;
+    int ring;
     double flops;
     const double* A2; long lda2; int a_split;
     double* C2; long ldc2; int c_split;
diff --git a/pygps_amd/csrc/ctx.h b/pygps_amd/csrc/ctx.h
--- a/pygps_amd/csrc/ctx.h
+++ b/pygps_amd/csrc/ctx.h
@@ -141,6 +141,7 @@
     int64_t pc_launch[PC_COUNT];
     std::map<std::vector<int>, std::pair<int*, int>> orders;
     int gemm_dbg = 64 | 256 | 512;
+    int tile_ring = 1;
     int xcd_order = 0;
     int nb_outer = 0;
     int trtri_small_tile_below = 2049;
diff --git a/pygps_amd/csrc/gemm_f64.hip b/pygps_amd/csrc/gemm_f64.hip
--- a/pygps_amd/csrc/gemm_f64.hip
+++ b/pygps_amd/csrc/gemm_f64.hip
@@ -52,7 +52,7 @@
     return true;
 }
 
-template <int TM, int TN, bool AKC, bool BKC, bool DMA = false, bool YIELD = false>
+template <int TM, int TN, bool AKC, bool BKC, bool DMA = false, bool YIELD = false, bool RING = false>
 __global__ __launch_bounds__(256, 2) void gemm_f64_kernel(GemmArgs g) {
     extern __shared__ __attribute__((aligned(16))) double smem[];
     if (g.trace) {
@@ -78,15 +78,15 @@
     }
     if (!YIELD && g.yield_role == 2) {
         pgp_yield_mark(g.yield_flags, +1);
-        gemm_tile_ns::gemm_tile<TM, TN, AKC, BKC, DMA, false>(g, ti, tj, bz, smem, (int)(blockIdx.x + gridDim.x * blockIdx.z));
+        gemm_tile_ns::gemm_tile<TM, TN, AKC, BKC, DMA, false, RING>(g, ti, tj, bz, smem, (int)(blockIdx.x + gridDim.x * blockIdx.z));
         __syncthreads();
         pgp_yield_mark(g.yield_flags, -1);
         return;
     }
-    gemm_tile_ns::gemm_tile<TM, TN, AKC, BKC, DMA, YIELD>(g, ti, tj, bz, smem, (int)(blockIdx.x + gridDim.x * blockIdx.z));
-}
-
-template <bool YIELD>
+    gemm_tile_ns::gemm_tile<TM, TN, AKC, BKC, DMA, YIELD, RING>(g, ti, tj, bz, smem, (int)(blockIdx.x + gridDim.x * blockIdx.z));
+}
+
+template <bool YIELD, bool RING = false>
 __global__ __launch_bounds__(256, 2) void gemm_f64_pair_kernel(GemmArgs a, GemmArgs b, int na) {
     extern __shared__ __attribute__((aligned(16))) double smem[];
     auto run = [&](const GemmArgs& g, int bid) {
@@ -97,38 +97,40 @@
         }
         int ti, tj;
         if (!decode_tile(g, bid, 128, 128, ti, tj)) return;
-        gemm_tile_ns::gemm_tile<128, 128, false, false, true, YIELD>(g, ti, tj, 0, smem, bid);
+        gemm_tile_ns::gemm_tile<128, 128, false, false, true, YIELD, RING>(g, ti, tj, 0, smem, bid);
     };
     if ((int)blockIdx.x < na) run(a, (int)blockIdx.x);
     else run(b, (int)blockIdx.x - na);
 }
 
-template <bool YIELD>
+template <bool YIELD, bool RING = false>
 __global__ __launch_bounds__(256, 2) void gemm_f64_fold_kernel(GemmArgs g) {
     extern __shared__ __attribute__((aligned(16))) double smem[];
     const int mt = g.M / 128, half = (mt + 1) / 2;
     const int r = (int)blockIdx.x % half, tj = (int)blockIdx.x / half;
     const int hi = mt - 1 - r;
     const long bz = blockIdx.z;
-    gemm_tile_ns::gemm_tile<128, 128, false, false, true, YIELD>(g, hi, tj, bz, smem, 0);
+    gemm_tile_ns::gemm_tile<128, 128, false, false, true, YIELD, RING>(g, hi, tj, bz, smem, 0);
     if (hi != r) {
         __syncthreads();
-        gemm_tile_ns::gemm_tile<128, 128, false, false, true, YIELD>(g, r, tj, bz, smem, 0);
-    }
-}
-
-template <int T, bool AKC, bool BKC, bool DMA = false, bool YIELD = false>
+        gemm_tile_ns::gemm_tile<128, 128, false, false, true, YIELD, RING>(g, r, tj, bz, smem, 0);
+    }
+}
+
+constexpr size_t DMA_SPARE = 16;
+
+template <int T, bool AKC, bool BKC, bool DMA = false, bool YIELD = false, bool RING = false>
 int launch_t(const GemmArgs& g, hipStream_t st) {
     constexpr int SK = BK + 2;
     constexpr int ASZ = AKC ? T * SK : BK * (T + 16);
     constexpr int BSZ = BKC ? T * SK : BK * (T + 16);
-    const size_t shm = 2 * (ASZ + BSZ) * sizeof(double);
+    const size_t shm = 2 * (ASZ + BSZ) * sizeof(double) + (DMA ? DMA_SPARE : 0);
     const int mt = g.M / T, nt = g.N / T;
     unsigned nblk = (g.tri == 2) ? (unsigned)((long)mt * (mt + 1) / 2) : (unsigned)(mt * nt);
     if (g.order) nblk = (unsigned)g.norder;
     dim3 grid(nblk, 1, (g.batch > 0 && !g.order_z) ? g.batch : 1);
-    func_max_dynamic_lds((const void*)gemm_f64_kernel<T, T, AKC, BKC, DMA, YIELD>, shm);
-    hipLaunchKernelGGL((gemm_f64_kernel<T, T, AKC, BKC, DMA, YIELD>), grid, dim3(256), shm, st, g);
+    func_max_dynamic_lds((const void*)gemm_f64_kernel<T, T, AKC, BKC, DMA, YIELD, RING>, shm);
+    hipLaunchKernelGGL((gemm_f64_kernel<T, T, AKC, BKC, DMA, YIELD, RING>), grid, dim3(256), shm, st, g);
     return hipGetLastError() == hipSuccess ? PGP_OK : PGP_ERR_HIP;
 }
 
@@ -136,13 +138,13 @@
 static bool dma1264_ok(const GemmArgs& g) {
     return g.tile == 1264 && dma_ok(g) && !g.tri && !g.order && g.batch <= 1 && !g.order_z && (g.N % 64) == 0 && (g.M % 128) == 0 && g.kmode == KM_FULL;
 }
-template <bool YIELD>
+template <bool YIELD, bool RING>
 int launch_1264(const GemmArgs& g, hipStream_t st) {
     constexpr int SA_ = 128 + 16;
-    const size_t shm = 2 * (BK * SA_ + (BK / 2) * SA_) * sizeof(double);
+    const size_t shm = 2 * (BK * SA_ + (BK / 2) * SA_) * sizeof(double) + DMA_SPARE;
     dim3 grid((unsigned)((g.M / 128) * (g.N / 64)), 1, 1);
-    func_max_dynamic_lds((const void*)gemm_f64_kernel<128, 64, false, false, true, YIELD>, shm);
-    hipLaunchKernelGGL((gemm_f64_kernel<128, 64, false, false, true, YIELD>), grid, dim3(256), shm, st, g);
+    func_max_dynamic_lds((const void*)gemm_f64_kernel<128, 64, false, false, true, YIELD, RING>, shm);
+    hipLaunchKernelGGL((gemm_f64_kernel<128, 64, false, false, true, YIELD, RING>), grid, dim3(256), shm, st, g);
     return hipGetLastError() == hipSuccess ? PGP_OK : PGP_ERR_HIP;
 }
 
@@ -172,29 +174,35 @@
     auto plain = [](const GemmArgs& g) {
         return g.M > 0 && g.N > 0 && g.tile != 64 && dma_ok(g) && g.batch <= 1 && !g.order_z && !g.wait_flag && g.yield_role != 2;
     };
-    return plain(a) && plain(b) && (a.yield_role == 1 && a.yield_flags) == (b.yield_role == 1 && b.yield_flags);
+    return plain(a) && plain(b) && (a.yield_role == 1 && a.yield_flags) == (b.yield_role == 1 && b.yield_flags) && !a.ring == !b.ring;
 }
 int gemm_f64_launch_pair(const GemmArgs& a, const GemmArgs& b, hipStream_t st) {
     if (!gemm_f64_pair_ok(a, b)) return -2;
     constexpr int SA_ = 128 + 16;
-    const size_t shm = 2 * (2 * BK * SA_) * sizeof(double);
+    const size_t shm = 2 * (2 * BK * SA_) * sizeof(double) + DMA_SPARE;
     const unsigned na = launch_blocks(a), nb = launch_blocks(b);
     const bool yield = a.yield_role == 1 && a.yield_flags;
-    func_max_dynamic_lds((const void*)(yield ? gemm_f64_pair_kernel<true> : gemm_f64_pair_kernel<false>), shm);
-    if (yield) hipLaunchKernelGGL(gemm_f64_pair_kernel<true>, dim3(na + nb), dim3(256), shm, st, a, b, (int)na);
-    else hipLaunchKernelGGL(gemm_f64_pair_kernel<false>, dim3(na + nb), dim3(256), shm, st, a, b, (int)na);
+    auto go = [&](auto kern) {
+        func_max_dynamic_lds((const void*)kern, shm);
+        hipLaunchKernelGGL(kern, dim3(na + nb), dim3(256), shm, st, a, b, (int)na);
+    };
+    if (a.ring) { if (yield) go(gemm_f64_pair_kernel<true, true>); else go(gemm_f64_pair_kernel<false, true>); }
+    else { if (yield) go(gemm_f64_pair_kernel<true, false>); else go(gemm_f64_pair_kernel<false, false>); }
     return hipGetLastError() == hipSuccess ? PGP_OK : PGP_ERR_HIP;
 }
 
 static int launch_fold(const GemmArgs& g, hipStream_t st) {
     constexpr int SA_ = 128 + 16;
-    const size_t shm = 2 * (2 * BK * SA_) * sizeof(double);
+    const size_t shm = 2 * (2 * BK * SA_) * sizeof(double) + DMA_SPARE;
     const int mt = g.M / 128, nt = g.N / 128;
     dim3 grid((unsigned)(((mt + 1) / 2) * nt), 1, g.batch > 0 ? g.batch : 1);
     const bool yield = g.yield_role == 1 && g.yield_flags;
-    func_max_dynamic_lds((const void*)(yield ? gemm_f64_fold_kernel<true> : gemm_f64_fold_kernel<false>), shm);
-    if (yield) hipLaunchKernelGGL(gemm_f64_fold_kernel<true>, grid, dim3(256), shm, st, g);
-    else hipLaunchKernelGGL(gemm_f64_fold_kernel<false>, grid, dim3(256), shm, st, g);
+    auto go = [&](auto kern) {
+        func_max_dynamic_lds((const void*)kern, shm);
+        hipLaunchKernelGGL(kern, grid, dim3(256), shm, st, g);
+    };
+    if (g.ring) { if (yield) go(gemm_f64_fold_kernel<true, true>); else go(gemm_f64_fold_kernel<false, true>); }
+    else { if (yield) go(gemm_f64_fold_kernel<true, false>); else go(gemm_f64_fold_kernel<false, false>); }
     return hipGetLastError() == hipSuccess ? PGP_OK : PGP_ERR_HIP;
 }
 
@@ -203,8 +211,14 @@
     if (g.tile == 64) return launch_l<64>(g, st);
     if (g.fold_rows && g.tile == 128 && dma_ok(g) && !g.tri && !g.order && !g.order_z && !g.wait_flag && g.yield_role != 2 && !g.trace)
         return launch_fold(g, st);
-    if (dma1264_ok(g)) return (g.yield_role == 1 && g.yield_flags) ? launch_1264<true>(g, st) : launch_1264<false>(g, st);
-    if (dma_ok(g)) return (g.yield_role == 1 && g.yield_flags) ? launch_t<128, false, false, true, true>(g, st)
-                                                               : launch_t<128, false, false, true>(g, st);
+    const bool yield = g.yield_role == 1 && g.yield_flags;
+    if (dma1264_ok(g)) {
+        if (g.ring) return yield ? launch_1264<true, true>(g, st) : launch_1264<false, true>(g, st);
+        return yield ? launch_1264<true, false>(g, st) : launch_1264<false, false>(g, st);
+    }
+    if (dma_ok(g)) {
+        if (g.ring) return yield ? launch_t<128, false, false, true, true, true>(g, st) : launch_t<128, false, false, true, false, true>(g, st);
+        return yield ? launch_t<128, false, false, true, true>(g, st) : launch_t<128, false, false, true>(g, st);
+    }
     return launch_l<128>(g, st);
 }
diff --git a/pygps_amd/csrc/gemm_tile.h b/pygps_amd/csrc/gemm_tile.h
--- a/pygps_amd/csrc/gemm_tile.h
+++ b/pygps_amd/csrc/gemm_tile.h
@@ -20,6 +20,20 @@
 }
 template <int V> struct IC { static constexpr int value = V; };
 
+template <int N>
+__device__ __forceinline__ void ring_wait() { asm volatile("s_waitcnt vmcnt(%0)" :: "n"(N) : "memory"); }
+template <int N>
+__device__ __forceinline__ void ring_wait_barrier() {
+    asm volatile("s_waitcnt vmcnt(%0) lgkmcnt(0)" :: "n"(N) : "memory");
+    __builtin_amdgcn_s_barrier();
+    asm volatile("" ::: "memory");
+}
+__device__ __forceinline__ void ring_load_f64(double& d, const double* p) {
+    asm volatile("global_load_dwordx2 %0, %1, off" : "=v"(d) : "v"(p) : "memory");
+}
+__device__ __forceinline__ void ring_landed(double& d) { asm volatile("" : "+v"(d)); }
+__device__ __forceinline__ void ring_landed(unsigned& d) { asm volatile("" : "+v"(d)); }
+
 __device__ __forceinline__ double swap_adjacent(double v) {
     const int lo = __builtin_amdgcn_update_dpp(0, __double2loint(v), 0xB1, 0xF, 0xF, false);
     const int hi = __builtin_amdgcn_update_dpp(0, __double2hiint(v), 0xB1, 0xF, 0xF, false);
@@ -33,8 +47,9 @@
     }
 }
 
-template <int TM, int TN, bool AKC, bool BKC, bool DMA = false, bool YIELD = false>
+template <int TM, int TN, bool AKC, bool BKC, bool DMA = false, bool YIELD = false, bool RING = false>
 __device__ __forceinline__ void gemm_tile(const GemmArgs& g, int ti, int tj, long bz, double* __restrict__ smem, int wg = 0) {
+    static_assert(!RING || DMA, "the staging ring is an LDS-DMA loop");
     static_assert(!DMA || (!AKC && !BKC && TM == 128 && (TN == 128 || TN == 64)), "LDS-DMA staging: M-contiguous operands, 128 x 128 or 128 x 64 tiles");
     constexpr bool BH = DMA && TN == 64;
     constexpr int SA = TM + 16, SB = BH ? TM + 16 : TN + 16, SK = BK + 2;
@@ -166,6 +181,24 @@
             for (int p = 0; p < 4; ++p) { da[p] += dstep_a; db[p] += dstep_b; }
         }
     };
+    constexpr int P = BH ? 3 : 4;
+    auto ring_piece = [&](auto bufc, auto halfc, auto jc) __attribute__((always_inline)) {
+        constexpr int O = decltype(bufc)::value * STAGE * 8, hf = decltype(halfc)::value, j = decltype(jc)::value;
+        if constexpr (DMA && BH) {
+            if constexpr (j == 0) { lds_dma_1k_s<O + (8 * hf) * SA * 8>(dvoff, da[2 * hf], lds_w); da[2 * hf] += dstep_a; }
+            if constexpr (j == 1) { lds_dma_1k_s<O + ASZ * 8 + (4 * hf) * SB * 8>(dvoff_b, db[hf], lds_w); db[hf] += dstep_b; }
+            if constexpr (j == 2) { lds_dma_1k_s<O + (8 * hf + 4) * SA * 8>(dvoff, da[2 * hf + 1], lds_w); da[2 * hf + 1] += dstep_a; }
+        } else if constexpr (DMA) {
+            if constexpr (j == 0) { lds_dma_1k_s<O + (8 * hf) * SA * 8>(dvoff, da[2 * hf], lds_w); da[2 * hf] += dstep_a; }
+            if constexpr (j == 1) { lds_dma_1k_s<O + ASZ * 8 + (8 * hf) * SB * 8>(dvoff, db[2 * hf], lds_w); db[2 * hf] += dstep_b; }
+            if constexpr (j == 2) { lds_dma_1k_s<O + (8 * hf + 4) * SA * 8>(dvoff, da[2 * hf + 1], lds_w); da[2 * hf + 1] += dstep_a; }
+            if constexpr (j == 3) { lds_dma_1k_s<O + ASZ * 8 + (8 * hf + 4) * SB * 8>(dvoff, db[2 * hf + 1], lds_w); db[2 * hf + 1] += dstep_b; }
+        }
+    };
+    auto ring_issue = [&](auto bufc, auto halfc) __attribute__((always_inline)) {
+        ring_piece(bufc, halfc, IC<0>{}); ring_piece(bufc, halfc, IC<1>{}); ring_piece(bufc, halfc, IC<2>{});
+        if constexpr (P == 4) ring_piece(bufc, halfc, IC<3>{});
+    };
     auto gload = [&](int) {
 #pragma unroll
         for (int p = 0; p < AV; ++p) { ra[p] = *(const double2_t*)pa[p]; pa[p] += astep; }
@@ -207,7 +240,28 @@
         }
     };
 
+    double cr[8];
+    const int ring_half = __builtin_amdgcn_readfirstlane(wave >> 1);
+    auto ring_cact = [&](int fold_step) __attribute__((always_inline)) { return !BH || ring_half == (fold_step >> 3); };
+    auto ring_cload = [&](int chunk) __attribute__((always_inline)) {
+        const int in = chunk / (FM / 2), hf = chunk % (FM / 2);
+#pragma unroll
+        for (int q = 0; q < 2; ++q) {
+            const double* cp = Cin + (long)(i0 + wm + (2 * hf + q) * 16 + l15) + (long)(j0 + wn + in * 16 + l4) * ldcin;
+#pragma unroll
+            for (int r = 0; r < 4; ++r) ring_load_f64(cr[4 * q + r], cp + (long)(4 * r) * ldcin);
+        }
+    };
     if (k0 < k1) {
+        if constexpr (RING) {
+            ring_issue(IC<0>{}, IC<0>{});
+            ring_issue(IC<0>{}, IC<1>{});
+            if (k0 + BK < k1) {
+                ring_issue(IC<1>{}, IC<0>{});
+                if (lazyc && ring_cact(1)) { ring_cload(0); ring_wait_barrier<2 * P + 8>(); }
+                else ring_wait_barrier<2 * P>();
+            } else ring_wait_barrier<P>();
+        } else {
         if constexpr (DMA) {
             dma_stage(IC<0>{});
             asm volatile("s_waitcnt vmcnt(0)" ::: "memory");
@@ -216,6 +270,7 @@
             sstore(0);
         }
         __syncthreads();
+        }
         double fa[2][FM], fb[2][FN];
         auto ldfrag = [&](int b, int ks, int slot) {
             const double* sa = smem + b * STAGE;
@@ -265,7 +320,100 @@
             __builtin_amdgcn_sched_barrier(0);
             mfmas((NS - 1) & 1);
         };
+        auto mfma1 = [&](int slot, auto ic) __attribute__((always_inline)) {
+            constexpr int i = decltype(ic)::value, in = i / FM, im = i % FM;
+            acc[im][in] = __builtin_amdgcn_mfma_f64_16x16x4f64(fb[slot][in], fa[slot][im], acc[im][in], 0, 0, 0);
+        };
+        auto mfmas_p = [&](int slot, bool go, auto bufc, auto halfc) __attribute__((always_inline)) {
+            auto one = [&](auto ic) __attribute__((always_inline)) {
+                constexpr int i = decltype(ic)::value;
+                mfma1(slot, ic);
+                if constexpr (i % 2 == 1 && i / 2 < P) {
+                    __builtin_amdgcn_sched_barrier(0);
+                    if (go) ring_piece(bufc, halfc, IC<i / 2>{});
+                    __builtin_amdgcn_sched_barrier(0);
+                }
+            };
+            one(IC<0>{}); one(IC<1>{}); one(IC<2>{}); one(IC<3>{}); one(IC<4>{}); one(IC<5>{}); one(IC<6>{}); one(IC<7>{});
+            if constexpr (FM * FN == 16) {
+                one(IC<8>{}); one(IC<9>{}); one(IC<10>{}); one(IC<11>{}); one(IC<12>{}); one(IC<13>{}); one(IC<14>{}); one(IC<15>{});
+            }
+        };
+        auto rstep = [&](int kt, auto bufc, auto pollc, int cp, int cmchunk, bool cmact) __attribute__((always_inline)) {
+            constexpr int buf = decltype(bufc)::value;
+            constexpr bool POLL = YIELD && decltype(pollc)::value != 0;
+            constexpr int Y = POLL ? 1 : 0;
+            const bool more = kt + BK < k1, more2 = kt + 2 * BK < k1;
+            unsigned yv = 0u;
+            if constexpr (POLL) asm volatile("global_load_dword %0, %1, %2 sc1" : "=v"(yv) : "v"(0u), "s"(yf) : "memory");
+            ldfrag(buf, 1, 1);
+            mfmas_p(0, more, IC<(buf ^ 1)>{}, IC<1>{});
+            if (more) {
+                if (cp != 0) ring_wait_barrier<2 * P + Y + 8>();
+                else ring_wait_barrier<2 * P + Y>();
+            } else ring_wait_barrier<0>();
+            const bool cm = cmchunk >= 0 && cmact;
+            if (cm) ring_cload(cmchunk);
+            ldfrag(buf, 2, 0);
+            __builtin_amdgcn_sched_barrier(0);
+            mfmas_p(1, more2, IC<buf>{}, IC<0>{});
+            ldfrag(buf, 3, 1);
+            mfmas(0);
+            if (more2) {
+                if (cm) ring_wait_barrier<2 * P + 8>();
+                else ring_wait_barrier<2 * P>();
+            } else if (more) ring_wait_barrier<P>();
+            else ring_wait_barrier<0>();
+            if constexpr (POLL) { ring_landed(yv); if (__builtin_amdgcn_readfirstlane(yv) != 0u) gemm_yield_wait(yf); }
+            if (more) ldfrag(buf ^ 1, 0, 0);
+            __builtin_amdgcn_sched_barrier(0);
+            mfmas(1);
+        };
         int kt = k0;
+        if constexpr (RING) {
+            if (lazyc) {
+                static_assert(FM == 4 && (FN == 4 || FN == 2), "lazy C: 64-row wave tiles, 64 or 32 columns");
+                auto lzstep = [&](auto stc) __attribute__((always_inline)) {
+                    constexpr int st = decltype(stc)::value;
+                    constexpr int chunk = (BH ? (st & 7) : st) >> 1, in = chunk / (FM / 2), hf = chunk % (FM / 2);
+                    if constexpr ((st & 1) != 0) {
+                        if (ring_cact(st)) {
+#pragma unroll
+                            for (int i = 0; i < 8; ++i) ring_landed(cr[i]);
+#pragma unroll
+                            for (int q = 0; q < 2; ++q)
+#pragma unroll
+                                for (int r = 0; r < 4; ++r) acc[2 * hf + q][in][r] = fma(ab, cr[4 * q + r], acc[2 * hf + q][in][r]);
+                        }
+                        rstep(kt, IC<1>{}, IC<0>{}, 0, st + 2 < LZ ? (BH ? ((st + 2) & 7) : (st + 2)) >> 1 : -1, ring_cact(st + 2));
+                    } else {
+                        const int cp = ring_cact(st + 1) ? 8 : 0;
+                        if constexpr ((st & 3) == 0) rstep(kt, IC<0>{}, IC<1>{}, cp, -1, false);
+                        else rstep(kt, IC<0>{}, IC<0>{}, cp, -1, false);
+                    }
+                    kt += BK;
+                };
+                static_assert(LZ == 16, "the prologue is written out");
+                lzstep(IC<0>{}); lzstep(IC<1>{}); lzstep(IC<2>{}); lzstep(IC<3>{}); lzstep(IC<4>{}); lzstep(IC<5>{}); lzstep(IC<6>{}); lzstep(IC<7>{});
+                lzstep(IC<8>{}); lzstep(IC<9>{}); lzstep(IC<10>{}); lzstep(IC<11>{}); lzstep(IC<12>{}); lzstep(IC<13>{}); lzstep(IC<14>{}); lzstep(IC<15>{});
+                if (g.trace) smem[2 * STAGE] = __longlong_as_double((long long)wall_clock64());
+            }
+            while (kt < k1) {
+                rstep(kt, IC<0>{}, IC<1>{}, 0, -1, false);
+                kt += BK;
+                if (kt >= k1) break;
+                rstep(kt, IC<1>{}, IC<0>{}, 0, -1, false);
+                kt += BK;
+                if constexpr (YIELD) {
+                    if (kt >= k1) break;
+                    rstep(kt, IC<0>{}, IC<0>{}, 0, -1, false);
+                    kt += BK;
+                    if (kt >= k1) break;
+                    rstep(kt, IC<1>{}, IC<0>{}, 0, -1, false);
+                    kt += BK;
+                }
+            }
+        } else {
         if constexpr (DMA) {
             if (lazyc) {
                 double4_t creg[2];
@@ -295,6 +443,7 @@
                     else kstep(kt, IC<0>{}, IC<0>{});
                     kt += BK;
                 }
+                if (g.trace) smem[2 * STAGE] = __longlong_as_double((long long)wall_clock64());
             }
         }
         while (kt < k1) {
@@ -312,10 +461,14 @@
                 kt += BK;
             }
         }
+        }
     }
 
     long long* const trc = g.trace ? g.trace + 8L * wg : nullptr;
-    if (trc) trc[2] = (long long)wall_clock64();
+    if (trc) {
+        trc[2] = (long long)wall_clock64();
+        if constexpr (DMA) trc[1] = lazyc ? __double_as_longlong(smem[2 * STAGE]) : 0ll;
+    }
     if (!diag && (g.dbg & 512) && !(ldc & 1) && !((unsigned long)C & 15ul)) {
         const bool odd = l15 & 1;
 #pragma unroll
diff --git a/pygps_amd/csrc/testhooks.h b/pygps_amd/csrc/testhooks.h
--- a/pygps_amd/csrc/testhooks.h
+++ b/pygps_amd/csrc/testhooks.h
@@ -13,6 +13,8 @@
 int pgp_test_gemm_zskip(pgp_ctx* ctx, int tile, int tri, int mask_diag, int zero_from, int zf_upper, double alpha, double beta,
                         const double* A, int64_t lda, const double* B, int64_t ldb, const double* Cin, double* C, int64_t ldc,
                         int M, int N, int K);
+int pgp_test_gemm_pair(pgp_ctx* ctx, double alpha, double beta, const double* A, int64_t lda, const double* B, int64_t ldb, double* Ca,
+                       double* Cb, int64_t ldc, int M, int N, int Ka, int Kb);
 int pgp_test_gemm_skip_wait(pgp_ctx* ctx, int tile, const double* A, const double* B, double* C, int n, int K, int skip_lo,
                             int skip_hi, int wait_ms, int* timed_out);
 int pgp_test_probit_hazard(pgp_ctx* ctx, const double* z, double* out, int n);
diff --git a/pygps_amd/csrc/testhooks.hip b/pygps_amd/csrc/testhooks.hip
--- a/pygps_amd/csrc/testhooks.hip
+++ b/pygps_amd/csrc/testhooks.hip
@@ -378,6 +378,8 @@
                   int64_t ldc, int M, int N, int K, int iters, double* ms_out) {
     if (!ctx) return -1;
     pgp_ctx* c = ctx;
+    const bool poll = getenv("PGP_TEST_GEMM_YIELD") != nullptr;
+    if (poll && !c->yield_flags) return -2;
     HIP_TRY(hipSetDevice(c->device));
     const size_t an = (size_t)lda * (a_kc ? M : K), bn = (size_t)ldb * (b_kc ? N : K), cn = (size_t)ldc * N;
     double *Ad, *Bd, *Cd;
@@ -388,8 +390,9 @@
     GemmArgs g{};
     g.A = Ad; g.lda = lda; g.a_kc = a_kc; g.B = Bd; g.ldb = ldb; g.b_kc = b_kc; g.C = Cd; g.ldc = ldc;
     g.M = M; g.N = N; g.K = K; g.alpha = alpha; g.beta = beta; g.tri = tri; g.tri_off = 0; g.mask_diag = mask_diag;
-    g.kmode = kmode; g.koff = koff; g.batch = 1; g.tile = tile; g.dbg = c->gemm_dbg;
+    g.kmode = kmode; g.koff = koff; g.batch = 1; g.tile = tile; g.dbg = c->gemm_dbg; g.ring = c->tile_ring != 0;
     if (getenv("PGP_TEST_GEMM_FOLD")) g.fold_rows = 1;
+    if (poll && gemm_f64_uses_dma(g)) { g.yield_flags = c->yield_flags; g.yield_role = 1; }
     hipStream_t ts = c->st;
     int rc = gemm_f64_launch(g, ts);
     HIP_TRY(hipStreamSynchronize(ts));
@@ -437,7 +440,7 @@
     HIP_TRY(hipMemset(Cd, 0, (size_t)M * M * 8)); HIP_TRY(hipMemset(C2, 0, (size_t)M * M * 8));
     GemmArgs g{};
     g.A = A; g.lda = M; g.B = A; g.ldb = M; g.C = Cd; g.ldc = M; g.M = M; g.N = M; g.K = K; g.alpha = -1.0; g.beta = 1.0;
-    g.tri = tri ? 2 : 0; g.mask_diag = tri ? 1 : 0; g.batch = 1; g.tile = 128; g.dbg = c->gemm_dbg;
+    g.tri = tri ? 2 : 0; g.mask_diag = tri ? 1 : 0; g.batch = 1; g.tile = 128; g.dbg = c->gemm_dbg; g.ring = c->tile_ring != 0;
     int rc = PGP_OK;
     for (int i = 0; i < warm && rc == PGP_OK; ++i) rc = gemm_f64_launch(g, c->st);
     HIP_TRY(hipStreamSynchronize(c->st));
@@ -481,7 +484,7 @@
     HIP_TRY(hipMemset(fl, 0, 16));
     GemmArgs g{};
     g.A = Ad; g.lda = n; g.B = Bd; g.ldb = n; g.C = Cd; g.ldc = n; g.M = n; g.N = n; g.K = K; g.alpha = -1.0; g.beta = 1.0;
-    g.tri = 2; g.mask_diag = 1; g.batch = 1; g.tile = tile; g.dbg = c->gemm_dbg; g.skip_lo = skip_lo; g.skip_hi = skip_hi;
+    g.tri = 2; g.mask_diag = 1; g.batch = 1; g.tile = tile; g.dbg = c->gemm_dbg; g.ring = c->tile_ring != 0; g.skip_lo = skip_lo; g.skip_hi = skip_hi;
     if (wait_ms > 0) { g.wait_flag = fl; g.wait_target = 7u; g.wait_err = fl + 1; }
     int rc = gemm_f64_launch(g, c->st);
     if (rc == PGP_OK && wait_ms > 0) {
@@ -539,11 +542,37 @@
     GemmArgs g{};
     g.A = Ad; g.lda = lda; g.B = Bd; g.ldb = ldb; g.C = Cd; g.ldc = ldc; g.M = M; g.N = N; g.K = K; g.alpha = alpha; g.beta = beta;
     if (Ci) { g.Cin = Ci; g.ldcin = ldc; }
-    g.tri = tri; g.mask_diag = mask_diag; g.kmode = KM_FULL; g.batch = 1; g.tile = tile; g.dbg = c->gemm_dbg;
+    g.tri = tri; g.mask_diag = mask_diag; g.kmode = KM_FULL; g.batch = 1; g.tile = tile; g.dbg = c->gemm_dbg; g.ring = c->tile_ring != 0;
     g.zero_from = zero_from; g.zf_upper = zf_upper;
     const int rc = gemm_f64_launch(g, c->st);
     HIP_TRY(hipStreamSynchronize(c->st));
     if (rc == PGP_OK) HIP_TRY(hipMemcpy(C, Cd, cn, hipMemcpyDeviceToHost));
+    return rc;
+}
+
+int pgp_test_gemm_pair(pgp_ctx* ctx, double alpha, double beta, const double* A, int64_t lda, const double* B, int64_t ldb, double* Ca,
+                       double* Cb, int64_t ldc, int M, int N, int Ka, int Kb) {
+    if (!ctx) return -1;
+    pgp_ctx* c = ctx;
+    const int K = std::max(Ka, Kb);
+    if (!A || !B || !Ca || !Cb || M <= 0 || N <= 0 || M % 128 || N % 128 || Ka <= 0 || Kb <= 0 || Ka % 16 || Kb % 16 || lda < M || ldb < N || ldc < M) return -2;
+    HIP_TRY(hipSetDevice(c->device));
+    DevScratch scr;
+    double *Ad = nullptr, *Bd = nullptr, *Cad = nullptr, *Cbd = nullptr;
+    const size_t an = (size_t)lda * K * 8, bn = (size_t)ldb * K * 8, cn = (size_t)ldc * N * 8;
+    CHK(scr.alloc(&Ad, an)); CHK(scr.alloc(&Bd, bn)); CHK(scr.alloc(&Cad, cn)); CHK(scr.alloc(&Cbd, cn));
+    HIP_TRY(hipMemcpy(Ad, A, an, hipMemcpyHostToDevice));
+    HIP_TRY(hipMemcpy(Bd, B, bn, hipMemcpyHostToDevice));
+    HIP_TRY(hipMemcpy(Cad, Ca, cn, hipMemcpyHostToDevice));
+    HIP_TRY(hipMemcpy(Cbd, Cb, cn, hipMemcpyHostToDevice));
+    GemmArgs g{};
+    g.A = Ad; g.lda = lda; g.B = Bd; g.ldb = ldb; g.C = Cad; g.ldc = ldc; g.M = M; g.N = N; g.K = Ka; g.alpha = alpha; g.beta = beta;
+    g.kmode = KM_FULL; g.batch = 1; g.tile = 128; g.dbg = c->gemm_dbg; g.ring = c->tile_ring != 0;
+    GemmArgs h = g;
+    h.C = Cbd; h.K = Kb;
+    const int rc = gemm_f64_launch_pair(g, h, c->st);
+    HIP_TRY(hipStreamSynchronize(c->st));
+    if (rc == PGP_OK) { HIP_TRY(hipMemcpy(Ca, Cad, cn, hipMemcpyDeviceToHost)); HIP_TRY(hipMemcpy(Cb, Cbd, cn, hipMemcpyDeviceToHost)); }
     return rc;
 }
 
@@ -639,7 +668,7 @@
     HIP_TRY(hipMemset(A, 0, (size_t)M * K * 8)); HIP_TRY(hipMemset(Cm, 0, (size_t)M * M * 8));
     GemmArgs g{};
     g.A = A; g.lda = M; g.B = A; g.ldb = M; g.C = Cm; g.ldc = M; g.M = M; g.N = M; g.K = K;
-    g.alpha = -1.0; g.beta = 1.0; g.tile = 128; g.batch = 1; g.dbg = c->gemm_dbg;
+    g.alpha = -1.0; g.beta = 1.0; g.tile = 128; g.batch = 1; g.dbg = c->gemm_dbg; g.ring = c->tile_ring != 0;
     hipEvent_t e0, e1;
     HIP_TRY(hipEventCreate(&e0)); HIP_TRY(hipEventCreate(&e1));
     hipStream_t sts[2] = {ms, c->st};
```

Result: faster. 111.0 fits/s, median of 6 (+1.5%).
